# stormalex/minimap2_chaindp

Hardware: AMD Instinct MI355X
Metric: chained anchors/sec (whole node) (higher is better)
Workload: dtype int32

## Files before the change

### minimap2_chaindp_amd/chaindp.py

```python
import collections
import ctypes as C
import os

import numpy as np

from .params import ChainParams, PostOpt

_HERE = os.path.dirname(os.path.abspath(__file__))
LIB_PATH = os.environ.get("CHAINDP_LIB") or os.path.join(_HERE, "csrc", "libchaindp_hip.so")

SEED_DTYPE = np.dtype([("x", "<u8"), ("y", "<u8"), ("p", "<i4"), ("f", "<i4")])

ABI_SYMBOLS = (
    "chaindp_device_count", "chaindp_create", "chaindp_destroy", "chaindp_last_error", "chaindp_chain_batch",
    "chaindp_upload", "chaindp_run", "chaindp_sync", "chaindp_download", "chaindp_compact",
    "chaindp_upload_gather", "chaindp_compact_offsets", "chaindp_download_seeds", "chaindp_host_alloc",
    "chaindp_host_free", "chaindp_run_device", "chaindp_set_profiling", "chaindp_get_kernel_ms",
    "chaindp_get_stats", "chaindp_set_ring", "chaindp_run_full", "chaindp_set_variant", "chaindp_upload_gather_ex", "chaindp_scatter_seeds", "chaindp_backtrack",
    "chaindp_index_create", "chaindp_index_destroy", "chaindp_collect_seeds", "chaindp_download_mini_pos", "chaindp_download_anchors", "chaindp_collect_seeds_gather", "chaindp_scatter_mini_pos",
    "chaindp_gen_regs", "chaindp_est_err",
    "chaindp_pipe_create", "chaindp_pipe_destroy", "chaindp_pipe_submit", "chaindp_pipe_wait", "chaindp_pipe_release",
    "chaindp_pipe_last_error", "chaindp_map_batch",
    "chaindp_chain_post", "chaindp_map_reads", "chaindp_post_logf_selftest", "chaindp_post_logf_patches",
)

REG_DTYPE = np.dtype([(k, "<i4") for k in ("id", "cnt", "rid", "score", "qs", "qe", "rs", "re", "parent", "subsc", "as", "mlen", "blen", "n_sub", "score0")]
                     + [("bits", "<u4"), ("hash", "<u4"), ("div", "<f4"), ("reserved", "<u4", (2,))])


class ChainDPError(RuntimeError):
    pass


_lib = None


def lib():
    global _lib
    if _lib is None:
        if not os.path.exists(LIB_PATH):
            raise ChainDPError(f"{LIB_PATH} is missing: build it with __graft_entry__.build() "
                               "(make -C minimap2_chaindp_amd/csrc); there is no fallback path")
        L = C.CDLL(LIB_PATH)
        P = C.POINTER(ChainParams)
        vp, i64, i32 = C.c_void_p, C.c_int64, C.c_int
        L.chaindp_device_count.restype = i32
        L.chaindp_create.restype = vp
        L.chaindp_create.argtypes = [i32, i64, i64]
        L.chaindp_destroy.argtypes = [vp]
        L.chaindp_last_error.restype = C.c_char_p
        L.chaindp_last_error.argtypes = [vp]
        L.chaindp_chain_batch.argtypes = [vp, P, i64, vp, vp, vp, vp, vp, vp]
        L.chaindp_upload.argtypes = [vp, i64, vp, vp, vp]
        L.chaindp_run.argtypes = [vp, P]
        L.chaindp_run_full.argtypes = [vp, P]
        L.chaindp_sync.argtypes = [vp]
        L.chaindp_download.argtypes = [vp, vp, vp, vp]
        L.chaindp_compact.argtypes = [vp, P, vp, vp]
        L.chaindp_upload_gather.argtypes = [vp, i64, vp, vp, vp]
        L.chaindp_compact_offsets.argtypes = [vp, P, vp]
        L.chaindp_download_seeds.argtypes = [vp, i64, i64, vp]
        L.chaindp_host_alloc.restype = vp
        L.chaindp_host_alloc.argtypes = [C.c_size_t]
        L.chaindp_host_free.argtypes = [vp]
        L.chaindp_run_device.argtypes = [vp, P, i64, i64, vp, vp, vp, vp, vp, vp, vp]
        L.chaindp_set_profiling.argtypes = [vp, i32]
        L.chaindp_get_kernel_ms.argtypes = [vp, vp, vp, i32]
        L.chaindp_get_stats.argtypes = [vp, vp]
        L.chaindp_set_ring.argtypes = [vp, i32]
        L.chaindp_set_variant.argtypes = [vp, i32]
        L.chaindp_backtrack.argtypes = [vp, P, i32, vp, vp, vp, vp]
        L.chaindp_gen_regs.argtypes = [vp, vp, vp, vp]
        L.chaindp_est_err.argtypes = [vp, vp, vp, vp, vp, i32, vp, vp, vp]
        L.chaindp_index_create.restype = vp
        L.chaindp_index_create.argtypes = [i32, vp, C.c_size_t, vp, C.c_size_t, vp, C.c_size_t, vp, C.c_size_t]
        L.chaindp_index_destroy.restype = None
        L.chaindp_index_destroy.argtypes = [vp]
        L.chaindp_collect_seeds.argtypes = [vp, vp, i32, i32, i64, vp, vp, vp, vp, vp, vp, vp, vp]
        L.chaindp_download_mini_pos.argtypes = [vp, vp]
        L.chaindp_collect_seeds_gather.argtypes = [vp, vp, i32, i32, i64, vp, vp, vp, vp, vp, vp, vp, vp]
        L.chaindp_scatter_mini_pos.argtypes = [vp, i64, vp]
        L.chaindp_upload_gather_ex.argtypes = [vp, i64, vp, vp, vp, i32]
        L.chaindp_scatter_seeds.argtypes = [vp, i64, vp]
        L.chaindp_device_count.argtypes = []
        L.chaindp_download_anchors.argtypes = [vp, vp]
        L.chaindp_map_batch.argtypes = [vp, vp, i32, i32, P, i32, i64, vp, vp, vp, vp, vp, vp, vp, i64, vp, vp]
        PO = C.POINTER(PostOpt)
        L.chaindp_chain_post.argtypes = [vp, PO, vp, vp, vp, i32, vp, vp, vp, vp, i64, vp, vp]
        L.chaindp_map_reads.argtypes = [vp, vp, i32, i32, P, i32, PO, i64, vp, vp, vp, vp, vp, vp, i32, vp, vp, i64, vp, vp]
        L.chaindp_post_logf_selftest.restype = i64
        L.chaindp_post_logf_selftest.argtypes = [vp, i32]
        L.chaindp_post_logf_patches.restype = i64
        L.chaindp_post_logf_patches.argtypes = [vp, vp, i64]
        L.chaindp_pipe_create.restype = vp
        L.chaindp_pipe_create.argtypes = [i32, i32, i64, i64]
        L.chaindp_pipe_destroy.restype = None
        L.chaindp_pipe_destroy.argtypes = [vp]
        L.chaindp_pipe_submit.argtypes = [vp, P, i64, vp, vp, vp, i64]
        L.chaindp_pipe_wait.argtypes = [vp, vp]
        L.chaindp_pipe_release.argtypes = [vp]
        L.chaindp_pipe_last_error.restype = C.c_char_p
        L.chaindp_pipe_last_error.argtypes = [vp]
        _lib = L
    return _lib


def post_logf_patches():
    L = lib()
    n = int(L.chaindp_post_logf_patches(None, None, 0))
    k, v = np.zeros(max(n, 1), np.uint32), np.zeros(max(n, 1), np.float32)
    L.chaindp_post_logf_patches(_ptr(k), _ptr(v), n)
    return k[:n], v[:n]


def device_count():
    return lib().chaindp_device_count()


def _ptr(a):
    return None if a is None else a.ctypes.data


class Device:

    def __init__(self, device=0, max_anchors=1 << 24, max_reads=1 << 20, ring=None):
        self._lib = lib()
        if self._lib.chaindp_device_count() <= 0:
            raise ChainDPError("no HIP device visible: the chaining DP runs only on the GPU (no CPU fallback)")
        self._ctx = self._lib.chaindp_create(device, max_anchors, max_reads)
        if not self._ctx:
            raise ChainDPError(self._lib.chaindp_last_error(None).decode())
        self.device = device
        self.max_anchors, self.max_reads = max_anchors, max_reads
        self._n_reads = self._total = 0
        self._indexes = []
        if ring is not None:
            self._check(self._lib.chaindp_set_ring(self._ctx, ring))

    def close(self):
        if self._ctx:
            for h in self._indexes:
                self._lib.chaindp_index_destroy(h)
            self._indexes = []
            self._lib.chaindp_destroy(self._ctx)
            self._ctx = None

    def __enter__(self):
        return self

    def __exit__(self, *exc):
        self.close()

    def __del__(self):
        try:
            self.close()
        except Exception:
            pass

    def _check(self, rc):
        if rc != 0:
            raise ChainDPError(f"chaindp error {rc}: {self._lib.chaindp_last_error(self._ctx).decode()}")

    @staticmethod
    def _prep(off, anchors, n_segs):
        off = np.ascontiguousarray(off, np.int64)
        anchors = np.ascontiguousarray(anchors, np.uint64).reshape(-1, 2)
        if len(off) < 1 or off[0] != 0 or int(off[-1]) != anchors.shape[0]:
            raise ValueError("off must start at 0 and end at the number of anchors")
        ns = None if n_segs is None else np.ascontiguousarray(n_segs, np.int32)
        if ns is not None and len(ns) != len(off) - 1:
            raise ValueError("n_segs must have one entry per read")
        return off, anchors, ns

    def chain_batch(self, par, off, anchors, n_segs=None, want_v=True):
        off, anchors, ns = self._prep(off, anchors, n_segs)
        tot = anchors.shape[0]
        f, p = np.empty(tot, np.int32), np.empty(tot, np.int32)
        v = np.empty(tot, np.int32) if want_v else None
        self._check(self._lib.chaindp_chain_batch(self._ctx, C.byref(par), len(off) - 1, _ptr(off), _ptr(anchors), _ptr(ns),
                                                  _ptr(f), _ptr(p), _ptr(v)))
        self._n_reads, self._total = len(off) - 1, tot
        return f, p, v

    def upload(self, off, anchors, n_segs=None):
        off, anchors, ns = self._prep(off, anchors, n_segs)
        self._check(self._lib.chaindp_upload(self._ctx, len(off) - 1, _ptr(off), _ptr(anchors), _ptr(ns)))
        self._n_reads, self._total = len(off) - 1, anchors.shape[0]

    def run(self, par):
        self._check(self._lib.chaindp_run(self._ctx, C.byref(par)))

    def run_full(self, par):
        self._check(self._lib.chaindp_run_full(self._ctx, C.byref(par)))

    def sync(self):
        self._check(self._lib.chaindp_sync(self._ctx))

    def download(self, want_v=True):
        f, p = np.empty(self._total, np.int32), np.empty(self._total, np.int32)
        v = np.empty(self._total, np.int32) if want_v else None
        self._check(self._lib.chaindp_download(self._ctx, _ptr(f), _ptr(p), _ptr(v)))
        return f, p, v

    def compact(self, par):
        soff = np.zeros(self._n_reads + 1, np.int64)
        seeds = np.zeros(max(self._total, 1), SEED_DTYPE)
        self._check(self._lib.chaindp_compact(self._ctx, C.byref(par), _ptr(soff), _ptr(seeds)))
        return soff, seeds[:int(soff[-1])]

    def backtrack(self, par, min_cnt=3):
        coff = np.zeros(self._n_reads + 1, np.int64)
        boff = np.zeros(self._n_reads + 1, np.int64)
        cap = max(self._total, 1)
        u = np.zeros(cap, np.uint64)
        b = np.zeros((cap, 2), np.uint64)
        self._check(self._lib.chaindp_backtrack(self._ctx, C.byref(par), min_cnt, _ptr(coff), _ptr(u), _ptr(boff), _ptr(b)))
        return coff, u[:int(coff[-1])], boff, b[:int(boff[-1])]

    def gen_regs(self, hash_, qlen, n_chains):
        hash_ = np.ascontiguousarray(hash_, np.uint32)
        qlen = np.ascontiguousarray(qlen, np.int32)
        regs = np.zeros(max(int(n_chains), 1), REG_DTYPE)
        self._check(self._lib.chaindp_gen_regs(self._ctx, _ptr(hash_), _ptr(qlen), _ptr(regs)))
        return regs[:int(n_chains)]

    def est_err(self, regs_off, regs, qlen, ref_len, mini_pos_off=None, mini_pos=None):
        regs_off = np.ascontiguousarray(regs_off, np.int64)
        regs = np.ascontiguousarray(regs, REG_DTYPE).copy()
        qlen = np.ascontiguousarray(qlen, np.int32)
        ref_len = np.ascontiguousarray(ref_len, np.int32)
        mt = np.zeros((max(len(regs), 1), 2), np.int32)
        mpo = None if mini_pos_off is None else np.ascontiguousarray(mini_pos_off, np.int64)
        mp = None if mini_pos is None else np.ascontiguousarray(mini_pos, np.uint64)
        self._check(self._lib.chaindp_est_err(self._ctx, _ptr(regs_off), _ptr(regs) if len(regs) else None, _ptr(qlen), _ptr(ref_len) if len(ref_len) else None,
                                              len(ref_len), None if mpo is None else _ptr(mpo), None if mp is None or not len(mp) else _ptr(mp), _ptr(mt)))
        return regs, mt[:len(regs), 0].copy(), mt[:len(regs), 1].copy()

    def load_index(self, img):
        blobs = [np.ascontiguousarray(b, np.uint8) for b in img]
        h = self._lib.chaindp_index_create(self.device, *sum(([_ptr(b) if b.size else None, int(b.size)] for b in blobs), []))
        if not h:
            raise ChainDPError((self._lib.chaindp_last_error(None) or b"").decode())
        self._indexes.append(h)
        return h

    def collect_seeds(self, index, flag, max_occ, mini_off, mini, bid, qlen, n_segs=None):
        mini_off = np.ascontiguousarray(mini_off, np.int64)
        n_reads = len(mini_off) - 1
        mini = np.ascontiguousarray(mini, np.uint64).reshape(-1, 2)
        bid = np.ascontiguousarray(bid, np.uint32); qlen = np.ascontiguousarray(qlen, np.int32)
        off = np.zeros(n_reads + 1, np.int64); mpo = np.zeros(n_reads + 1, np.int64); rep = np.zeros(max(n_reads, 1), np.int32)
        ns = None if n_segs is None else np.ascontiguousarray(n_segs, np.int32)
        self._check(self._lib.chaindp_collect_seeds(self._ctx, index, int(flag), int(max_occ), n_reads, _ptr(mini_off), _ptr(mini), _ptr(bid),
                                                    _ptr(qlen), _ptr(ns), _ptr(off), _ptr(rep), _ptr(mpo)))
        self._n_reads, self._total = n_reads, int(off[-1])
        a = np.zeros((max(self._total, 1), 2), np.uint64)
        self._check(self._lib.chaindp_download_anchors(self._ctx, _ptr(a)))
        mp = np.zeros(max(int(mpo[-1]), 1), np.uint64)
        self._check(self._lib.chaindp_download_mini_pos(self._ctx, _ptr(mp)))
        return off, a[:self._total], rep[:n_reads], mpo, mp[:int(mpo[-1])]

    def map_batch(self, index, flag, max_occ, par, min_cnt, mini_off, mini, bid, qlen, hash_, regs_cap=None):
        mini_off = np.ascontiguousarray(mini_off, np.int64)
        n_reads = len(mini_off) - 1
        mini = np.ascontiguousarray(mini, np.uint64).reshape(-1, 2)
        bid = np.ascontiguousarray(bid, np.uint32); qlen = np.ascontiguousarray(qlen, np.int32); hash_ = np.ascontiguousarray(hash_, np.uint32)
        cap = int(regs_cap) if regs_cap is not None else max(len(mini) // 4, 1024)
        roff = np.zeros(n_reads + 1, np.int64); rep = np.zeros(max(n_reads, 1), np.int32)
        regs = np.zeros(max(cap, 1), REG_DTYPE)
        na = C.c_int64(0)
        rc = self._lib.chaindp_map_batch(self._ctx, index, int(flag), int(max_occ), C.byref(par), int(min_cnt), n_reads, _ptr(mini_off), _ptr(mini),
                                         _ptr(bid), _ptr(qlen), _ptr(hash_), _ptr(roff), _ptr(regs), cap, _ptr(rep), C.byref(na))
        if rc == -2 and int(roff[-1]) > cap:
            regs = self.gen_regs(hash_, qlen, int(roff[-1]))
        else:
            self._check(rc)
        self._n_reads, self._total = n_reads, int(na.value)
        return roff, regs[:int(roff[-1])], rep[:n_reads], int(na.value)

    def chain_post(self, opt, ref_len, qlen=None, rep_len=None, mini_pos_off=None, mini_pos=None, regs_cap=None, want_anchors=False):
        n_reads = self._n_reads
        ref_len = np.ascontiguousarray(ref_len, np.int32)
        ql = None if qlen is None else np.ascontiguousarray(qlen, np.int32)
        rl = None if rep_len is None else np.ascontiguousarray(rep_len, np.int32)
        mpo = None if mini_pos_off is None else np.ascontiguousarray(mini_pos_off, np.int64)
        mp = None if mini_pos is None else np.ascontiguousarray(mini_pos, np.uint64)
        cap = int(regs_cap) if regs_cap is not None else max(self._total, 1)
        roff = np.zeros(n_reads + 1, np.int64)
        regs = np.zeros(max(cap, 1), REG_DTYPE)
        aoff = np.zeros(n_reads + 1, np.int64) if want_anchors else None
        a = np.zeros((max(self._total, 1), 2), np.uint64) if want_anchors else None
        self._check(self._lib.chaindp_chain_post(self._ctx, C.byref(opt), _ptr(ql), _ptr(rl), _ptr(ref_len) if len(ref_len) else None, len(ref_len),
                                                 _ptr(mpo), None if mp is None or not len(mp) else _ptr(mp), _ptr(roff), _ptr(regs), cap,
                                                 _ptr(aoff), _ptr(a)))
        regs = regs[:int(roff[-1])]
        return (roff, regs, aoff, a[:int(aoff[-1])]) if want_anchors else (roff, regs)

    def map_reads(self, index, flag, max_occ, par, min_cnt, opt, mini_off, mini, bid, qlen, hash_, ref_len, regs_cap=None):
        mini_off = np.ascontiguousarray(mini_off, np.int64)
        n_reads = len(mini_off) - 1
        mini = np.ascontiguousarray(mini, np.uint64).reshape(-1, 2)
        bid = np.ascontiguousarray(bid, np.uint32); qlen = np.ascontiguousarray(qlen, np.int32); hash_ = np.ascontiguousarray(hash_, np.uint32)
        ref_len = np.ascontiguousarray(ref_len, np.int32)
        cap = int(regs_cap) if regs_cap is not None else max(len(mini) // 4, 1024)
        roff = np.zeros(n_reads + 1, np.int64); rep = np.zeros(max(n_reads, 1), np.int32)
        regs = np.zeros(max(cap, 1), REG_DTYPE)
        na = C.c_int64(0)
        rc = self._lib.chaindp_map_reads(self._ctx, index, int(flag), int(max_occ), C.byref(par), int(min_cnt), C.byref(opt), n_reads, _ptr(mini_off),
                                         _ptr(mini), _ptr(bid), _ptr(qlen), _ptr(hash_), _ptr(ref_len) if len(ref_len) else None, len(ref_len),
                                         _ptr(roff), _ptr(regs), cap, _ptr(rep), C.byref(na))
        self._n_reads, self._total = n_reads, int(na.value)
        if rc == -2 and int(roff[-1]) > cap:
            roff, regs = self.chain_post(opt, ref_len, regs_cap=int(roff[-1]))
        else:
            self._check(rc)
        return roff, regs[:int(roff[-1])], rep[:n_reads], int(na.value)

    def post_logf_selftest(self, kmax=1 << 24):
        n = self._lib.chaindp_post_logf_selftest(self._ctx, int(kmax))
        if n < 0:
            self._check(int(n))
        return int(n)

    def run_device(self, par, n_reads, total, d_off, d_a, d_n_segs, d_f, d_p, d_v, stream=0):
        self._check(self._lib.chaindp_run_device(self._ctx, C.byref(par), n_reads, total, d_off, d_a, d_n_segs or None,
                                                 d_f, d_p, d_v, stream or None))

    def set_ring(self, ring):
        self._check(self._lib.chaindp_set_ring(self._ctx, ring))

    def set_variant(self, force_general):
        self._check(self._lib.chaindp_set_variant(self._ctx, int(force_general)))

    def set_profiling(self, on=True):
        self._check(self._lib.chaindp_set_profiling(self._ctx, int(bool(on))))

    def kernel_ms(self, reset=False):
        ms = (C.c_double * 4)()
        n = (C.c_int64 * 4)()
        self._check(self._lib.chaindp_get_kernel_ms(self._ctx, ms, n, int(reset)))
        return {k: (ms[i], n[i]) for i, k in enumerate(("prepass", "chain_dp", "compact", "backtrack"))}

    def leftover_units(self):
        self._lib.chaindp_debug_leftover.restype = C.c_int64
        self._lib.chaindp_debug_leftover.argtypes = [C.c_void_p]
        return int(self._lib.chaindp_debug_leftover(self._ctx))

    def deep_units(self):
        self._lib.chaindp_debug_deep_units.restype = C.c_int64
        self._lib.chaindp_debug_deep_units.argtypes = [C.c_void_p]
        return int(self._lib.chaindp_debug_deep_units(self._ctx))

    def set_quad(self, on=True):
        self._lib.chaindp_debug_set_quad.restype = C.c_int
        self._lib.chaindp_debug_set_quad.argtypes = [C.c_void_p, C.c_int]
        self._check(self._lib.chaindp_debug_set_quad(self._ctx, int(bool(on))))

    def quad_took(self):
        self._lib.chaindp_debug_quad_took.restype = C.c_int
        self._lib.chaindp_debug_quad_took.argtypes = [C.c_void_p]
        return int(self._lib.chaindp_debug_quad_took(self._ctx)) == 1

    def set_twin_handover(self, mode=0):
        self._lib.chaindp_debug_set_twin_handover.restype = C.c_int
        self._lib.chaindp_debug_set_twin_handover.argtypes = [C.c_void_p, C.c_int]
        self._check(self._lib.chaindp_debug_set_twin_handover(self._ctx, int(mode)))

    def set_deep_handover(self, on=True):
        self._lib.chaindp_debug_set_deep_handover.restype = C.c_int
        self._lib.chaindp_debug_set_deep_handover.argtypes = [C.c_void_p, C.c_int]
        self._check(self._lib.chaindp_debug_set_deep_handover(self._ctx, on if on in (2, 3, 4) else int(bool(on))))

    def stats(self):
        st = (C.c_int64 * 4)()
        self._check(self._lib.chaindp_get_stats(self._ctx, st))
        return dict(units=st[0], singletons=st[1], anchors=st[2], reads=st[3])


class PinnedArray:

    def __init__(self, shape, dtype):
        self._lib = lib()
        dtype = np.dtype(dtype)
        n = int(np.prod(shape)) * dtype.itemsize
        self._ptr = self._lib.chaindp_host_alloc(max(n, 1))
        if not self._ptr:
            raise ChainDPError("chaindp_host_alloc failed (no GPU runtime or out of pinned memory)")
        self.array = np.ctypeslib.as_array((C.c_uint8 * max(n, 1)).from_address(self._ptr))[:n].view(dtype).reshape(shape)

    def free(self):
        if self._ptr:
            self.array = None
            self._lib.chaindp_host_free(self._ptr)
            self._ptr = None

    def __del__(self):
        try:
            self.free()
        except Exception:
            pass


class _PipeResult(C.Structure):
    _fields_ = [("tag", C.c_int64), ("n_reads", C.c_int64), ("n_anchors", C.c_int64), ("n_seeds", C.c_int64),
                ("seeds_off", C.c_void_p), ("seeds", C.c_void_p)]


class Pipe:

    def __init__(self, device=0, depth=3, max_anchors=1 << 24, max_reads=1 << 20):
        self._lib = lib()
        if self._lib.chaindp_device_count() <= 0:
            raise ChainDPError("no HIP device visible: the chaining DP runs only on the GPU (no CPU fallback)")
        self._p = self._lib.chaindp_pipe_create(device, depth, max_anchors, max_reads)
        if not self._p:
            raise ChainDPError((self._lib.chaindp_pipe_last_error(None) or b"").decode())
        self.depth = depth
        self._keep = collections.deque()

    def close(self):
        if self._p:
            self._lib.chaindp_pipe_destroy(self._p)
            self._p = None

    def __enter__(self):
        return self

    def __exit__(self, *exc):
        self.close()

    def _check(self, rc):
        if rc != 0:
            raise ChainDPError(f"chaindp pipe error {rc}: {self._lib.chaindp_pipe_last_error(self._p).decode()}")

    def submit(self, par, off, anchors, n_segs=None, tag=0):
        off, anchors, ns = Device._prep(off, anchors, n_segs)
        rc = self._lib.chaindp_pipe_submit(self._p, C.byref(par), len(off) - 1, _ptr(off), _ptr(anchors), _ptr(ns), tag)
        if rc == -5:
            return False
        self._check(rc)
        self._keep.append((off, anchors, ns))
        return True

    def wait(self, copy=True):
        r = _PipeResult()
        self._check(self._lib.chaindp_pipe_wait(self._p, C.byref(r)))
        soff = np.ctypeslib.as_array((C.c_int64 * (r.n_reads + 1)).from_address(r.seeds_off))
        seeds = np.ctypeslib.as_array((C.c_uint8 * max(r.n_seeds * 24, 1)).from_address(r.seeds))[:r.n_seeds * 24].view(SEED_DTYPE)
        if copy:
            soff, seeds = soff.copy(), seeds.copy()
        if self._keep:
            self._keep.popleft()
        return r.tag, soff, seeds

    def release(self):
        self._check(self._lib.chaindp_pipe_release(self._p))
```

### minimap2_chaindp_amd/csrc/chaindp_abi.cpp

```cpp
#include <hip/hip_runtime.h>
#include <stdint.h>
#include <stdio.h>
#include <stdlib.h>
#include <string.h>
#include <math.h>
#include <mutex>
#include <string>
#include <vector>
#include "../../include/chaindp.h"
#include "chaindp_kernels.h"

using chaindp::Params;
using chaindp::Unit;

static thread_local std::string g_create_error;

struct EventSet { hipEvent_t e[3]; int n; int slot0; };

struct chaindp_ctx {
	int device = -1;
	hipStream_t stream = nullptr;
	int64_t cap_anchors = 0, cap_reads = 0;
	int ring = 128;
	int64_t n_reads = 0, total = 0, n_seeds = 0;
	bool has_n_segs = false, ran = false, compact_ready = false;
	bool singles_pending = false;
	chaindp_params_t ran_par{};
	int64_t *d_off = nullptr;
	void *d_a = nullptr;
	int32_t *d_n_segs = nullptr;
	int32_t *d_f = nullptr, *d_p = nullptr, *d_v = nullptr;
	unsigned long long *d_tg = nullptr;
	uint32_t epoch = 0;
	unsigned long long *d_sumq = nullptr;
	Unit *d_units = nullptr;
	chaindp::UnitAux *d_unit_aux = nullptr;
	Unit *d_left = nullptr;
	unsigned long long *d_left_cnt = nullptr;
	Unit *d_deep = nullptr;
	int deep_route = 0;
	int deep_eager = 0;
	bool deep_handover = true;
	bool use_quad = false;
	int twin_force_left = 0;
	int variant = 0;
	unsigned long long *d_counters = nullptr;
	chaindp::PrepassScratch pre = {nullptr, nullptr, nullptr, nullptr, nullptr};
	chaindp::CompactScratch cmp = {nullptr, nullptr, nullptr, nullptr, nullptr, nullptr};
	chaindp::BottomScratch bot = {};
	bool bot_ready = false, seed_ready = false;
	std::vector<void*> bot_allocs;
	uint16_t *d_lut = nullptr;
	void **d_ptrs = nullptr;
	size_t ptr_cap = 0;
	size_t lut_bytes = 0;
	bool use_lut = true;
	int32_t *d_first_child = nullptr;
	unsigned int *d_twin_queue = nullptr;
	int64_t *d_seeds_off = nullptr;
	void *d_seeds = nullptr;
	chaindp::SeedScratch seed = {nullptr, nullptr, nullptr, nullptr, nullptr, nullptr, nullptr};
	void *d_mini = nullptr;
	int64_t *d_mini_off = nullptr, *d_mp_off = nullptr;
	uint32_t *d_bid = nullptr;
	int32_t *d_qlen = nullptr, *d_rep_len = nullptr;
	unsigned long long *d_mini_pos = nullptr;
	int64_t seed_cap_mini = 0, n_mini_pos = 0;
	int seed_max_n = -1, seed_max_n2 = -1;
	int seed_lab_cap = 0;
	void *d_regs = nullptr, *d_reg_counts = nullptr, *d_ref_len = nullptr, *d_mp_up = nullptr;
	size_t regs_cap = 0, reg_counts_cap = 0, ref_len_cap = 0, mp_up_cap = 0;
	uint32_t *d_rhash = nullptr;
	int32_t *d_rqlen = nullptr;
	int64_t *d_regs_off = nullptr, *d_mp_off_up = nullptr;
	unsigned long long *d_sum_k = nullptr;
	int64_t bot_n_reads = -1, bot_n_chains = 0, bot_n_b = 0;
	bool mp_resident = false;
	bool regs_resident = false;
	void *d_post_stage = nullptr, *d_post_out = nullptr, *d_post_sq = nullptr, *d_post_scratch = nullptr;
	size_t post_stage_cap = 0, post_out_cap = 0, post_sq_cap = 0, post_scratch_cap = 0;
	unsigned long long *d_post_off = nullptr, *d_post_tile = nullptr;
	int32_t *d_post_qlen = nullptr, *d_post_rep = nullptr, *d_post_err = nullptr;
	uint32_t *d_logf_k = nullptr;
	float *d_logf_v = nullptr;
	int n_logf = -1;
	bool prof = false;
	std::vector<EventSet> pending;
	double ms[4] = {0, 0, 0, 0};
	int64_t launches[4] = {0, 0, 0, 0};
	int64_t stats[4] = {0, 0, 0, 0};
	std::string err;
};

#define HIP_TRY(ctx, call)                                                                         \
	do {                                                                                           \
		hipError_t e_ = (call);                                                                    \
		if (e_ != hipSuccess) {                                                                    \
			(ctx)->err = std::string(#call) + ": " + hipGetErrorString(e_);                        \
			return CHAINDP_ERR_HIP;                                                                \
		}                                                                                          \
	} while (0)

static Params to_params(const chaindp_params_t *p)
{
	Params q;
	q.max_dist_x = p->max_dist_x; q.max_dist_y = p->max_dist_y; q.bw = p->bw; q.max_skip = p->max_skip;
	q.min_sc = p->min_sc; q.is_cdna = p->is_cdna; q.n_segs = p->n_segs;
	return q;
}

static int check_params(chaindp_ctx *ctx, const chaindp_params_t *par)
{
	if (!par) { ctx->err = "params is NULL"; return CHAINDP_ERR_ARG; }
	if (par->max_dist_x < 0 || par->max_dist_y < 0 || par->bw < 0) {
		ctx->err = "max_dist_x, max_dist_y and bw must be >= 0";
		return CHAINDP_ERR_ARG;
	}
	return CHAINDP_OK;
}

extern "C" int chaindp_device_count(void)
{
	int n = 0;
	if (hipGetDeviceCount(&n) != hipSuccess) return 0;
	return n;
}

extern "C" const char *chaindp_last_error(const chaindp_ctx_t *ctx)
{
	return ctx ? ctx->err.c_str() : g_create_error.c_str();
}

extern "C" void chaindp_destroy(chaindp_ctx_t *ctx)
{
	if (!ctx) return;
	if (ctx->device >= 0) (void)hipSetDevice(ctx->device);
	if (ctx->stream) (void)hipStreamSynchronize(ctx->stream);
	for (auto &es : ctx->pending) for (int k = 0; k < es.n; ++k) (void)hipEventDestroy(es.e[k]);
	void *bufs[] = {ctx->d_twin_queue, ctx->d_off, ctx->d_a, ctx->d_n_segs, ctx->d_f, ctx->d_p, ctx->d_v, ctx->d_tg, ctx->d_sumq, ctx->d_units,
	                ctx->d_counters, ctx->d_unit_aux, ctx->d_left, ctx->d_left_cnt, ctx->d_deep, ctx->pre.start_mask, ctx->pre.single_mask, ctx->pre.emit_mask, ctx->pre.block_cnt, ctx->pre.tile_tmp, ctx->pre.units_tmp, ctx->pre.hist, ctx->pre.block_reads, ctx->d_lut, ctx->d_ptrs, ctx->cmp.flags, ctx->cmp.block_cnt, ctx->cmp.tile_tmp, ctx->cmp.n_seeds, ctx->cmp.sub, ctx->d_first_child, ctx->d_seeds_off, ctx->d_seeds};
	for (void *b : bufs) if (b) (void)hipFree(b);
	for (void *b : ctx->bot_allocs) if (b) (void)hipFree(b);
	void *sbufs[] = {ctx->seed.kept, ctx->seed.used, ctx->seed.src, ctx->seed.mstate, ctx->seed.tile_tmp, ctx->seed.totals, ctx->seed.stacks,
	                 ctx->d_mini, ctx->d_mini_off, ctx->d_mp_off, ctx->d_bid, ctx->d_qlen, ctx->d_rep_len, ctx->d_mini_pos};
	for (void *b : sbufs) if (b) (void)hipFree(b);
	if (ctx->stream) (void)hipStreamDestroy(ctx->stream);
	delete ctx;
}

extern "C" chaindp_ctx_t *chaindp_create(int device, int64_t max_anchors, int64_t max_reads)
{
	int n_dev = 0;
	if (hipGetDeviceCount(&n_dev) != hipSuccess || n_dev <= 0) { g_create_error = "no HIP device visible"; return nullptr; }
	if (device < 0 || device >= n_dev || max_anchors < 0 || max_reads < 0 || max_anchors > 0x7fffffff || max_reads > 0x7fffffff) {
		g_create_error = "bad device index or capacity (at most 2^31-1 anchors and reads per batch)";
		return nullptr;
	}
	chaindp_ctx *ctx = new chaindp_ctx();
	ctx->device = device;
	ctx->cap_anchors = max_anchors > 0 ? max_anchors : 1;
	ctx->cap_reads = max_reads > 0 ? max_reads : 1;
	const size_t na = (size_t)ctx->cap_anchors, nr = (size_t)ctx->cap_reads;
	hipError_t e = hipSetDevice(device);
	if (e == hipSuccess) e = hipStreamCreateWithFlags(&ctx->stream, hipStreamNonBlocking);
	if (e == hipSuccess) e = hipMalloc((void**)&ctx->d_off, (nr + 1) * 8);
	if (e == hipSuccess) e = hipMalloc(&ctx->d_a, na * 16);
	if (e == hipSuccess) e = hipMalloc((void**)&ctx->d_n_segs, nr * 4);
	if (e == hipSuccess) e = hipMalloc((void**)&ctx->d_f, na * 4);
	if (e == hipSuccess) e = hipMalloc((void**)&ctx->d_twin_queue, 8 * 64 * sizeof(unsigned int));
	if (e == hipSuccess) e = hipMalloc((void**)&ctx->d_p, na * 4);
	if (e == hipSuccess) e = hipMalloc((void**)&ctx->d_v, na * 4);
	if (e == hipSuccess) e = hipMalloc((void**)&ctx->d_tg, na * 8);
	if (e == hipSuccess) e = hipMemset(ctx->d_tg, 0, na * 8);
	if (e == hipSuccess) e = hipMalloc((void**)&ctx->d_sumq, nr * 8);
	if (e == hipSuccess) e = hipMalloc((void**)&ctx->d_units, (na / 2 + 1) * sizeof(Unit));
	if (e == hipSuccess) e = hipMalloc((void**)&ctx->d_unit_aux, (na / 2 + 1) * sizeof(chaindp::UnitAux));
	if (e == hipSuccess) e = hipMalloc((void**)&ctx->d_counters, 2 * sizeof(unsigned long long));
	if (e == hipSuccess) e = hipMalloc((void**)&ctx->d_left, (na / 2 + 1) * sizeof(Unit));
	if (e == hipSuccess) e = hipMalloc((void**)&ctx->d_left_cnt, 4 * sizeof(unsigned long long));
	if (e == hipSuccess) e = hipMalloc((void**)&ctx->d_deep, (na / 64 + 2) * sizeof(Unit));
	size_t flags_bytes0 = 0, cblocks_bytes0 = 0;
	chaindp::compact_scratch_bytes(ctx->cap_anchors, &flags_bytes0, &cblocks_bytes0);
	if (e == hipSuccess) e = hipMalloc((void**)&ctx->d_first_child, na * 4);
	if (e == hipSuccess) e = hipMalloc((void**)&ctx->cmp.flags, flags_bytes0);
	size_t mask_bytes = 0, blocks_bytes = 0;
	chaindp::prepass_scratch_bytes(ctx->cap_anchors, &mask_bytes, &blocks_bytes);
	if (e == hipSuccess) e = hipMalloc((void**)&ctx->pre.start_mask, mask_bytes);
	if (e == hipSuccess) e = hipMalloc((void**)&ctx->pre.single_mask, mask_bytes);
	if (e == hipSuccess) e = hipMalloc((void**)&ctx->pre.emit_mask, mask_bytes);
	ctx->cmp.single_mask = ctx->pre.single_mask; ctx->cmp.emit_mask = ctx->pre.emit_mask;
	if (e == hipSuccess) e = hipMalloc((void**)&ctx->pre.block_cnt, blocks_bytes);
	if (e == hipSuccess) e = hipMalloc((void**)&ctx->pre.tile_tmp, blocks_bytes);
	if (e == hipSuccess) e = hipMalloc((void**)&ctx->pre.units_tmp, (na / 2 + 1) * sizeof(Unit));
	if (e == hipSuccess) e = hipMalloc((void**)&ctx->pre.hist, (2 * 128 + 2) * sizeof(unsigned int));
	ctx->pre.key_range = ctx->pre.hist ? ctx->pre.hist + 2 * 128 : nullptr;
	if (e == hipSuccess) e = hipMalloc((void**)&ctx->pre.block_reads, blocks_bytes);
	ctx->cmp.block_reads = ctx->pre.block_reads;
	ctx->use_quad = getenv("CHAINDP_QUAD") != nullptr;
	ctx->deep_handover = getenv("CHAINDP_NO_DEEP_HANDOVER") == nullptr;
	if (const char *v = getenv("CHAINDP_TWIN_FORCE_LEFT")) ctx->twin_force_left = atoi(v) == 2 ? 2 : 1;
	if (e != hipSuccess) {
		g_create_error = std::string("chaindp_create: ") + hipGetErrorString(e);
		chaindp_destroy(ctx);
		return nullptr;
	}
	return ctx;
}

extern "C" int chaindp_set_ring(chaindp_ctx_t *ctx, int ring)
{
	if (!ctx) return CHAINDP_ERR_ARG;
	if (ring != 128 && ring != 256 && ring != 512) { ctx->err = "ring must be 128, 256 or 512"; return CHAINDP_ERR_ARG; }
	ctx->ring = ring;
	return CHAINDP_OK;
}

extern "C" int chaindp_set_variant(chaindp_ctx_t *ctx, int force_general)
{
	if (!ctx) return CHAINDP_ERR_ARG;
	if (force_general < 0 || force_general > 2) { ctx->err = "variant must be 0 (two units per wave + the rest), 1 (general) or 2 (one unit per wave)"; return CHAINDP_ERR_ARG; }
	ctx->use_lut = force_general != 1;
	ctx->variant = force_general;
	return CHAINDP_OK;
}

extern "C" int chaindp_set_profiling(chaindp_ctx_t *ctx, int on)
{
	if (!ctx) return CHAINDP_ERR_ARG;
	ctx->prof = on != 0;
	return CHAINDP_OK;
}

static int run_on_stream(chaindp_ctx *ctx, const chaindp_params_t *par, int64_t n_reads, int64_t total,
                         const int64_t *d_off, const void *d_a, const int32_t *d_n_segs,
                         int32_t *d_f, int32_t *d_p, int32_t *d_v, hipStream_t st)
{
	int rc = check_params(ctx, par);
	if (rc) return rc;
	if (n_reads < 0 || total < 0) { ctx->err = "negative batch size"; return CHAINDP_ERR_ARG; }
	if (n_reads > ctx->cap_reads || total > ctx->cap_anchors) {
		ctx->err = "batch exceeds the capacity the context was created with";
		return CHAINDP_ERR_CAPACITY;
	}
	HIP_TRY(ctx, hipSetDevice(ctx->device));
	const Params q = to_params(par);
	EventSet es; es.n = 0; es.slot0 = 0;
	if (ctx->prof) {
		for (int k = 0; k < 3; ++k) HIP_TRY(ctx, hipEventCreate(&es.e[k]));
		es.n = 3;
	}
	if (ctx->prof) HIP_TRY(ctx, hipEventRecord(es.e[0], st));
	HIP_TRY(ctx, chaindp::launch_prepass(st, q, n_reads, total, d_off, d_a, ctx->d_sumq, ctx->d_units, ctx->d_counters, ctx->pre, ctx->d_unit_aux, d_n_segs, ctx->d_left_cnt));
	if (ctx->prof) HIP_TRY(ctx, hipEventRecord(es.e[1], st));
	uint16_t *lut = nullptr;
	int lut_stride = 0;
	if (ctx->use_lut && !q.is_cdna && q.bw <= CHAINDP_LUT_MAX_BW && n_reads > 0) {
		lut_stride = (q.bw + 1 + 7) & ~7;
		const size_t need = (size_t)n_reads * lut_stride * sizeof(uint16_t);
		if (need > ctx->lut_bytes) {
			HIP_TRY(ctx, hipStreamSynchronize(st));
			if (ctx->d_lut) HIP_TRY(ctx, hipFree(ctx->d_lut));
			ctx->d_lut = nullptr; ctx->lut_bytes = 0;
			HIP_TRY(ctx, hipMalloc((void**)&ctx->d_lut, need));
			ctx->lut_bytes = need;
		}
		lut = ctx->d_lut;
		HIP_TRY(ctx, chaindp::launch_lut(st, q, n_reads, d_off, ctx->d_sumq, lut_stride, lut));
	}
	if (++ctx->epoch == 0) {
		HIP_TRY(ctx, hipMemsetAsync(ctx->d_tg, 0, (size_t)ctx->cap_anchors * 8, st));
		ctx->epoch = 1;
	}
	Unit *const deep = ctx->deep_handover ? ctx->d_deep : nullptr;
	unsigned int *const deep_cnt = (unsigned int*)(ctx->d_left_cnt + 1);
	if (ctx->variant == 0 && lut) {
		unsigned int *const route = (unsigned int*)(ctx->d_left_cnt + 3);
		Params qt = q;
		if (d_n_segs) qt.n_segs = 1;
		if (ctx->use_quad)
			HIP_TRY(ctx, chaindp::launch_chain_quad(st, qt, total / 2, d_a, lut, lut_stride, ctx->d_units, ctx->d_unit_aux, ctx->d_counters, ctx->pre.key_range,
			                                        d_f, d_p, d_v, ctx->d_first_child, ctx->cmp.flags, ctx->d_left, (unsigned int*)ctx->d_left_cnt,
			                                        (unsigned int*)ctx->d_left_cnt + 1, route, ctx->twin_force_left, total));
		HIP_TRY(ctx, chaindp::launch_chain_twin(st, qt, total / 2, d_off, d_a, ctx->d_sumq, lut, lut_stride, ctx->d_units, ctx->d_counters,
		                                        d_f, d_p, d_v, ctx->d_first_child, ctx->cmp.flags, ctx->d_left, (unsigned int*)ctx->d_left_cnt,
		                                        ctx->twin_force_left, total, ctx->d_unit_aux, route, ctx->d_twin_queue));
		const int64_t left_grid = total / 2 < 32768 ? total / 2 : 32768;
		HIP_TRY(ctx, chaindp::launch_chain(st, ctx->ring, q, left_grid, d_off, d_a, d_n_segs, ctx->d_sumq, lut, lut_stride, ctx->d_left,
		                                   ctx->d_left_cnt, d_f, d_p, d_v, ctx->d_tg, ctx->epoch, ctx->d_first_child, ctx->cmp.flags,
		                                   ctx->d_units, ctx->d_counters, deep, deep_cnt, ctx->pre.hist + CHAINDP_LONG_UNIT_CLASS, ctx->deep_eager, ctx->deep_route));
	} else
		HIP_TRY(ctx, chaindp::launch_chain(st, ctx->ring, q, total / 2, d_off, d_a, d_n_segs, ctx->d_sumq, lut, lut_stride, ctx->d_units,
		                                   ctx->d_counters, d_f, d_p, d_v, ctx->d_tg, ctx->epoch, ctx->d_first_child, ctx->cmp.flags,
		                                   nullptr, nullptr, deep, deep_cnt, ctx->pre.hist + CHAINDP_LONG_UNIT_CLASS, ctx->deep_eager, ctx->deep_route));
	if (deep && lut) {
		HIP_TRY(ctx, chaindp::launch_chain_dense(st, q, total / 64 + 1, d_off, d_a, lut, lut_stride, ctx->d_deep, ctx->d_left_cnt + 1,
		                                         d_f, d_p, d_v, ctx->d_first_child, ctx->cmp.flags, ctx->pre.hist + CHAINDP_LONG_UNIT_CLASS, ctx->deep_route,
		                                           (unsigned int*)(ctx->d_left_cnt + 3) + 1));
		HIP_TRY(ctx, chaindp::launch_chain_dense16(st, q, total / 64 + 1, d_off, d_a, lut, lut_stride, ctx->d_deep, ctx->d_left_cnt + 1,
		                                           d_f, d_p, d_v, ctx->d_first_child, ctx->cmp.flags, ctx->pre.hist + CHAINDP_LONG_UNIT_CLASS, ctx->deep_route,
		                                           (unsigned int*)(ctx->d_left_cnt + 3) + 1));
		HIP_TRY(ctx, chaindp::launch_chain_dense1(st, q, total / 64 + 1, d_off, d_a, lut, lut_stride, ctx->d_deep, ctx->d_left_cnt + 1,
		                                          ctx->pre.hist + CHAINDP_LONG_UNIT_CLASS, ctx->deep_route, (unsigned int*)(ctx->d_left_cnt + 2), d_f, d_p, d_v, ctx->d_first_child, ctx->cmp.flags));
	}
	if (ctx->prof) { HIP_TRY(ctx, hipEventRecord(es.e[2], st)); ctx->pending.push_back(es); }
	ctx->stats[2] = total; ctx->stats[3] = n_reads;
	return CHAINDP_OK;
}

extern "C" int chaindp_upload(chaindp_ctx_t *ctx, int64_t n_reads, const int64_t *off, const chaindp_anchor_t *a,
                              const int32_t *n_segs_per_read)
{
	if (!ctx) return CHAINDP_ERR_ARG;
	if (n_reads < 0 || !off || (n_reads > 0 && off[0] != 0)) { ctx->err = "bad offsets"; return CHAINDP_ERR_ARG; }
	const int64_t total = n_reads > 0 ? off[n_reads] : 0;
	if (total < 0 || (total > 0 && !a)) { ctx->err = "bad anchors"; return CHAINDP_ERR_ARG; }
	if (n_reads > ctx->cap_reads || total > ctx->cap_anchors) {
		ctx->err = "batch exceeds the capacity the context was created with";
		return CHAINDP_ERR_CAPACITY;
	}
	HIP_TRY(ctx, hipSetDevice(ctx->device));
	HIP_TRY(ctx, hipMemcpyAsync(ctx->d_off, off, (size_t)(n_reads + 1) * 8, hipMemcpyHostToDevice, ctx->stream));
	if (total) HIP_TRY(ctx, hipMemcpyAsync(ctx->d_a, a, (size_t)total * 16, hipMemcpyHostToDevice, ctx->stream));
	ctx->has_n_segs = n_segs_per_read != nullptr;
	if (n_segs_per_read && n_reads)
		HIP_TRY(ctx, hipMemcpyAsync(ctx->d_n_segs, n_segs_per_read, (size_t)n_reads * 4, hipMemcpyHostToDevice, ctx->stream));
	HIP_TRY(ctx, hipStreamSynchronize(ctx->stream));
	ctx->n_reads = n_reads; ctx->total = total; ctx->ran = false; ctx->bot_n_reads = -1; ctx->mp_resident = false;
	return CHAINDP_OK;
}

extern "C" int chaindp_run(chaindp_ctx_t *ctx, const chaindp_params_t *par)
{
	if (!ctx) return CHAINDP_ERR_ARG;
	int rc = run_on_stream(ctx, par, ctx->n_reads, ctx->total, ctx->d_off, ctx->d_a, ctx->has_n_segs ? ctx->d_n_segs : nullptr,
	                       ctx->d_f, ctx->d_p, ctx->d_v, ctx->stream);
	if (rc == CHAINDP_OK) { ctx->ran = true; ctx->singles_pending = true; ctx->ran_par = *par; }
	return rc;
}

extern "C" int chaindp_run_device(chaindp_ctx_t *ctx, const chaindp_params_t *par, int64_t n_reads, int64_t total_anchors,
                                  const void *d_off, const void *d_a, const void *d_n_segs,
                                  void *d_f, void *d_p, void *d_v, void *stream)
{
	if (!ctx) return CHAINDP_ERR_ARG;
	if (!d_off || (total_anchors > 0 && (!d_a || !d_f || !d_p || !d_v))) { ctx->err = "NULL device pointer"; return CHAINDP_ERR_ARG; }
	hipStream_t st = stream ? (hipStream_t)stream : ctx->stream;
	const int rc = run_on_stream(ctx, par, n_reads, total_anchors, (const int64_t*)d_off, d_a, (const int32_t*)d_n_segs,
	                             (int32_t*)d_f, (int32_t*)d_p, (int32_t*)d_v, st);
	if (rc != CHAINDP_OK) return rc;
	HIP_TRY(ctx, chaindp::launch_fill_singles(st, to_params(par), total_anchors, d_a, ctx->pre, (int32_t*)d_f, (int32_t*)d_p, (int32_t*)d_v, ctx->cmp.flags));
	return CHAINDP_OK;
}

extern "C" int chaindp_sync(chaindp_ctx_t *ctx)
{
	if (!ctx) return CHAINDP_ERR_ARG;
	HIP_TRY(ctx, hipSetDevice(ctx->device));
	HIP_TRY(ctx, hipStreamSynchronize(ctx->stream));
	return CHAINDP_OK;
}

extern "C" int chaindp_download(chaindp_ctx_t *ctx, int32_t *f, int32_t *p, int32_t *v)
{
	if (!ctx) return CHAINDP_ERR_ARG;
	if (!ctx->ran) { ctx->err = "chaindp_download before chaindp_run"; return CHAINDP_ERR_ARG; }
	HIP_TRY(ctx, hipSetDevice(ctx->device));
	const size_t bytes = (size_t)ctx->total * 4;
	if (ctx->singles_pending) {
		HIP_TRY(ctx, chaindp::launch_fill_singles(ctx->stream, to_params(&ctx->ran_par), ctx->total, ctx->d_a, ctx->pre, ctx->d_f, ctx->d_p, ctx->d_v, ctx->cmp.flags));
		ctx->singles_pending = false;
	}
	if (bytes) {
		if (f) HIP_TRY(ctx, hipMemcpyAsync(f, ctx->d_f, bytes, hipMemcpyDeviceToHost, ctx->stream));
		if (p) HIP_TRY(ctx, hipMemcpyAsync(p, ctx->d_p, bytes, hipMemcpyDeviceToHost, ctx->stream));
		if (v) HIP_TRY(ctx, hipMemcpyAsync(v, ctx->d_v, bytes, hipMemcpyDeviceToHost, ctx->stream));
	}
	HIP_TRY(ctx, hipStreamSynchronize(ctx->stream));
	return CHAINDP_OK;
}

extern "C" int chaindp_chain_batch(chaindp_ctx_t *ctx, const chaindp_params_t *par, int64_t n_reads, const int64_t *off,
                                   const chaindp_anchor_t *a, const int32_t *n_segs_per_read,
                                   int32_t *f, int32_t *p, int32_t *v)
{
	if (!ctx) return CHAINDP_ERR_ARG;
	int rc = check_params(ctx, par);
	if (rc) return rc;
	if ((rc = chaindp_upload(ctx, n_reads, off, a, n_segs_per_read)) != CHAINDP_OK) return rc;
	if ((rc = chaindp_run(ctx, par)) != CHAINDP_OK) return rc;
	return chaindp_download(ctx, f, p, v);
}

static int compact_launch(chaindp_ctx *ctx, const chaindp_params_t *par)
{
	int rc = check_params(ctx, par);
	if (rc) return rc;
	if (!ctx->ran) { ctx->err = "compaction before chaindp_run"; return CHAINDP_ERR_ARG; }
	HIP_TRY(ctx, hipSetDevice(ctx->device));
	if (!ctx->compact_ready) {
		const size_t na = (size_t)ctx->cap_anchors, nr = (size_t)ctx->cap_reads;
		size_t flags_bytes = 0, blocks_bytes = 0;
		chaindp::compact_scratch_bytes(ctx->cap_anchors, &flags_bytes, &blocks_bytes);
		void *nb[6] = {nullptr, nullptr, nullptr, nullptr, nullptr, nullptr};
		const size_t sz[6] = {(nr + 1) * 8, ctx->d_seeds ? 0 : na * sizeof(chaindp_seed_t) + 16, blocks_bytes, blocks_bytes, 8, blocks_bytes * 32};
		hipError_t e = hipSuccess;
		for (int k = 0; k < 6 && e == hipSuccess; ++k) if (sz[k]) e = hipMalloc(&nb[k], sz[k]);
		if (e != hipSuccess) {
			for (void *b : nb) if (b) (void)hipFree(b);
			ctx->err = std::string("compaction buffers: ") + hipGetErrorString(e);
			return CHAINDP_ERR_HIP;
		}
		ctx->d_seeds_off = (int64_t*)nb[0];
		if (nb[1]) ctx->d_seeds = nb[1];
		ctx->cmp.block_cnt = (unsigned long long*)nb[2]; ctx->cmp.tile_tmp = (unsigned long long*)nb[3];
		ctx->cmp.n_seeds = (unsigned long long*)nb[4]; ctx->cmp.sub = (uint32_t*)nb[5];
		ctx->compact_ready = true;
	}
	EventSet es; es.n = 0; es.slot0 = 2;
	if (ctx->prof) {
		for (int k = 0; k < 2; ++k) HIP_TRY(ctx, hipEventCreate(&es.e[k]));
		es.n = 2;
		HIP_TRY(ctx, hipEventRecord(es.e[0], ctx->stream));
	}
	HIP_TRY(ctx, chaindp::launch_compact(ctx->stream, to_params(par), ctx->n_reads, ctx->total, ctx->d_off, ctx->d_a, ctx->d_f, ctx->d_p,
	                                     ctx->d_v, ctx->d_first_child, ctx->d_seeds_off, ctx->d_seeds, ctx->cmp));
	if (ctx->prof) { HIP_TRY(ctx, hipEventRecord(es.e[1], ctx->stream)); ctx->pending.push_back(es); }
	return CHAINDP_OK;
}

static int compact_on_device(chaindp_ctx *ctx, const chaindp_params_t *par, int64_t *seeds_off)
{
	if (!seeds_off) { ctx->err = "NULL output"; return CHAINDP_ERR_ARG; }
	int rc = compact_launch(ctx, par);
	if (rc) return rc;
	HIP_TRY(ctx, hipMemcpyAsync(seeds_off, ctx->d_seeds_off, (size_t)(ctx->n_reads + 1) * 8, hipMemcpyDeviceToHost, ctx->stream));
	HIP_TRY(ctx, hipStreamSynchronize(ctx->stream));
	ctx->n_seeds = seeds_off[ctx->n_reads];
	return CHAINDP_OK;
}

template <typename T>
static hipError_t bot_alloc(chaindp_ctx *ctx, T *&p, size_t bytes)
{
	void *q = nullptr;
	hipError_t e = hipMalloc(&q, bytes ? bytes : 8);
	if (e == hipSuccess) { ctx->bot_allocs.push_back(q); p = (T*)q; }
	return e;
}

extern "C" int chaindp_backtrack(chaindp_ctx_t *ctx, const chaindp_params_t *par, int min_cnt,
                                 int64_t *chains_off, uint64_t *u, int64_t *b_off, chaindp_anchor_t *b)
{
	if (!ctx) return CHAINDP_ERR_ARG;
	int rc = check_params(ctx, par);
	if (rc) return rc;
	if (!ctx->ran || !ctx->d_seeds) { ctx->err = "chaindp_backtrack needs a completed run and compaction"; return CHAINDP_ERR_ARG; }
	if (!chains_off || !b_off) { ctx->err = "NULL output"; return CHAINDP_ERR_ARG; }
	ctx->regs_resident = false;
	HIP_TRY(ctx, hipSetDevice(ctx->device));
	unsigned long long n_seeds = 0;
	HIP_TRY(ctx, hipMemcpyAsync(&n_seeds, ctx->cmp.n_seeds, 8, hipMemcpyDeviceToHost, ctx->stream));
	HIP_TRY(ctx, hipStreamSynchronize(ctx->stream));
	const int64_t m = ctx->total > 0 && ctx->n_reads > 0 ? (int64_t)(uint32_t)n_seeds : 0;
	ctx->n_seeds = m;
	if (!ctx->bot_ready) {
		const size_t M = (size_t)ctx->cap_anchors, R = (size_t)ctx->cap_reads, NB = M / 1024 + 2;
		chaindp::BottomScratch &s = ctx->bot;
		const size_t first = ctx->bot_allocs.size();
		hipError_t e = hipSuccess;
#define BOT_ALLOC(field, bytes) if (e == hipSuccess) e = bot_alloc(ctx, s.field, (bytes))
		BOT_ALLOC(has, M);
		BOT_ALLOC(owner, M * 4); BOT_ALLOC(end_rec, M * 4); BOT_ALLOC(ccnt, M * 4); BOT_ALLOC(kpos, M * 4); BOT_ALLOC(bpos, M * 4);
		BOT_ALLOC(c_src, M * 4); BOT_ALLOC(c_dst, M * 4);
		BOT_ALLOC(key, M * 8); BOT_ALLOC(skey, M * 8); BOT_ALLOC(cu, M * 8); BOT_ALLOC(u_tmp, M * 8); BOT_ALLOC(u_out, M * 8);
		BOT_ALLOC(b_tmp, M * 16); BOT_ALLOC(b_out, M * 16); BOT_ALLOC(w, M * 16);
		BOT_ALLOC(stacks, (M / 64 + 2 * R + 4) * 12);
		BOT_ALLOC(block_cnt, (NB > R + 2 ? NB : R + 2) * 8); BOT_ALLOC(tile_tmp, (NB > R + 2 ? NB : R + 2) * 8);
		BOT_ALLOC(read_tot, (R + 2) * 8); BOT_ALLOC(total, 8);
		BOT_ALLOC(ends_off, (R + 2) * 8); BOT_ALLOC(chains_off, (R + 2) * 8); BOT_ALLOC(b_off, (R + 2) * 8);
#undef BOT_ALLOC
		if (e != hipSuccess) {
			for (size_t k = first; k < ctx->bot_allocs.size(); ++k) if (ctx->bot_allocs[k]) (void)hipFree(ctx->bot_allocs[k]);
			ctx->bot_allocs.resize(first);
			ctx->bot = chaindp::BottomScratch{};
			ctx->err = std::string("backtrack buffers: ") + hipGetErrorString(e);
			return CHAINDP_ERR_HIP;
		}
		ctx->bot_ready = true;
	}
	EventSet es; es.n = 0; es.slot0 = 3;
	if (ctx->prof) {
		for (int k = 0; k < 2; ++k) HIP_TRY(ctx, hipEventCreate(&es.e[k]));
		es.n = 2;
		HIP_TRY(ctx, hipEventRecord(es.e[0], ctx->stream));
	}
	HIP_TRY(ctx, chaindp::launch_backtrack(ctx->stream, min_cnt, par->min_sc, ctx->n_reads, ctx->cap_anchors, ctx->d_seeds_off, ctx->d_seeds,
	                                       ctx->cmp.n_seeds, ctx->bot, m));
	if (ctx->prof) { HIP_TRY(ctx, hipEventRecord(es.e[1], ctx->stream)); ctx->pending.push_back(es); }
	const size_t ob = (size_t)(ctx->n_reads > 0 ? ctx->n_reads + 1 : 1) * 8;
	HIP_TRY(ctx, hipMemcpyAsync(chains_off, ctx->bot.chains_off, ob, hipMemcpyDeviceToHost, ctx->stream));
	HIP_TRY(ctx, hipMemcpyAsync(b_off, ctx->bot.b_off, ob, hipMemcpyDeviceToHost, ctx->stream));
	HIP_TRY(ctx, hipStreamSynchronize(ctx->stream));
	const int64_t n_c = ctx->n_reads > 0 ? chains_off[ctx->n_reads] : 0, n_b = ctx->n_reads > 0 ? b_off[ctx->n_reads] : 0;
	ctx->bot_n_reads = ctx->n_reads; ctx->bot_n_chains = n_c; ctx->bot_n_b = n_b;
	if (u && n_c > 0) HIP_TRY(ctx, hipMemcpyAsync(u, ctx->bot.u_out, (size_t)n_c * 8, hipMemcpyDeviceToHost, ctx->stream));
	if (b && n_b > 0) HIP_TRY(ctx, hipMemcpyAsync(b, ctx->bot.b_out, (size_t)n_b * 16, hipMemcpyDeviceToHost, ctx->stream));
	HIP_TRY(ctx, hipStreamSynchronize(ctx->stream));
	return CHAINDP_OK;
}

static hipError_t regs_grow(chaindp_ctx *ctx, void *&p, size_t &cap, size_t need)
{
	if (need <= cap && p) return hipSuccess;
	void *q = nullptr;
	hipError_t e = hipMalloc(&q, need ? need + need / 4 : 8);
	if (e != hipSuccess) return e;
	for (void *&old : ctx->bot_allocs) if (old == p && p) { (void)hipFree(p); old = nullptr; }
	ctx->bot_allocs.push_back(q);
	p = q; cap = need + need / 4;
	return hipSuccess;
}

static int regs_per_read_buffers(chaindp_ctx *ctx)
{
	if (ctx->d_rhash) return CHAINDP_OK;
	const size_t R = (size_t)ctx->cap_reads + 2;
	HIP_TRY(ctx, bot_alloc(ctx, ctx->d_rhash, R * 4)); HIP_TRY(ctx, bot_alloc(ctx, ctx->d_rqlen, R * 4));
	HIP_TRY(ctx, bot_alloc(ctx, ctx->d_regs_off, R * 8)); HIP_TRY(ctx, bot_alloc(ctx, ctx->d_mp_off_up, R * 8));
	HIP_TRY(ctx, bot_alloc(ctx, ctx->d_sum_k, R * 8));
	return CHAINDP_OK;
}

static int gen_regs_impl(chaindp_ctx *ctx, const uint32_t *hash, const int32_t *qlen, chaindp_reg_t *regs, bool download)
{
	if (!ctx) return CHAINDP_ERR_ARG;
	if (ctx->bot_n_reads < 0 || ctx->bot_n_reads != ctx->n_reads || !ctx->bot.has) { ctx->err = "chaindp_gen_regs needs the chains of a chaindp_backtrack on this batch"; return CHAINDP_ERR_ARG; }
	const int64_t R = ctx->bot_n_reads, n_c = ctx->bot_n_chains;
	if (R > 0 && (!hash || !qlen)) { ctx->err = "NULL hash or qlen"; return CHAINDP_ERR_ARG; }
	if (download && n_c > 0 && !regs) { ctx->err = "NULL output"; return CHAINDP_ERR_ARG; }
	ctx->regs_resident = false;
	if (R == 0 || n_c == 0) { ctx->regs_resident = true; return CHAINDP_OK; }
	HIP_TRY(ctx, hipSetDevice(ctx->device));
	int rc = regs_per_read_buffers(ctx);
	if (rc) return rc;
	HIP_TRY(ctx, regs_grow(ctx, ctx->d_regs, ctx->regs_cap, (size_t)n_c * sizeof(chaindp_reg_t)));
	hipStream_t st = ctx->stream;
	HIP_TRY(ctx, hipMemcpyAsync(ctx->d_rhash, hash, (size_t)R * 4, hipMemcpyHostToDevice, st));
	HIP_TRY(ctx, hipMemcpyAsync(ctx->d_rqlen, qlen, (size_t)R * 4, hipMemcpyHostToDevice, st));
	HIP_TRY(ctx, chaindp::launch_gen_regs(st, R, ctx->bot.chains_off, ctx->bot.b_off, ctx->bot.u_out, ctx->bot.b_out, ctx->d_rhash, ctx->d_rqlen,
	                                      ctx->bot.w, ctx->bot.stacks, ctx->d_regs));
	if (download) HIP_TRY(ctx, hipMemcpyAsync(regs, ctx->d_regs, (size_t)n_c * sizeof(chaindp_reg_t), hipMemcpyDeviceToHost, st));
	HIP_TRY(ctx, hipStreamSynchronize(st));
	ctx->regs_resident = true;
	return CHAINDP_OK;
}

extern "C" int chaindp_gen_regs(chaindp_ctx_t *ctx, const uint32_t *hash, const int32_t *qlen, chaindp_reg_t *regs)
{
	return gen_regs_impl(ctx, hash, qlen, regs, true);
}

extern "C" int chaindp_est_err(chaindp_ctx_t *ctx, const int64_t *regs_off, chaindp_reg_t *regs, const int32_t *qlen,
                               const int32_t *ref_len, int32_t n_ref, const int64_t *mini_pos_off, const uint64_t *mini_pos,
                               int32_t *match_tot)
{
	if (!ctx) return CHAINDP_ERR_ARG;
	if (ctx->bot_n_reads < 0 || ctx->bot_n_reads != ctx->n_reads || !ctx->bot.has) { ctx->err = "chaindp_est_err needs the chains of a chaindp_backtrack on this batch"; return CHAINDP_ERR_ARG; }
	const int64_t R = ctx->bot_n_reads;
	if (R == 0) return CHAINDP_OK;
	if (!regs_off || !qlen || (n_ref > 0 && !ref_len) || n_ref < 0) { ctx->err = "NULL argument"; return CHAINDP_ERR_ARG; }
	if (regs_off[0] != 0) { ctx->err = "regs_off must start at 0"; return CHAINDP_ERR_ARG; }
	for (int64_t r = 0; r < R; ++r) if (regs_off[r + 1] < regs_off[r]) { ctx->err = "regs_off must not decrease"; return CHAINDP_ERR_ARG; }
	const int64_t n_regs = regs_off[R];
	if (n_regs == 0) return CHAINDP_OK;
	if (!regs) { ctx->err = "NULL regs"; return CHAINDP_ERR_ARG; }
	const bool resident = mini_pos == nullptr && mini_pos_off == nullptr;
	if (resident && (!ctx->mp_resident || !ctx->d_mp_off)) { ctx->err = "no resident mini_pos: pass the arrays, or collect the seeds with chaindp_collect_seeds"; return CHAINDP_ERR_ARG; }
	if (!resident && !mini_pos_off) { ctx->err = "mini_pos without offsets"; return CHAINDP_ERR_ARG; }
	for (int64_t g = 0; g < n_regs; ++g) if (regs[g].cnt < 0 || regs[g].as < 0) { ctx->err = "hit with a negative count or offset"; return CHAINDP_ERR_ARG; }
	HIP_TRY(ctx, hipSetDevice(ctx->device));
	int rc = regs_per_read_buffers(ctx);
	if (rc) return rc;
	hipStream_t st = ctx->stream;
	ctx->regs_resident = false;
	{
		std::vector<int64_t> boff((size_t)R + 1);
		HIP_TRY(ctx, hipMemcpyAsync(boff.data(), ctx->bot.b_off, (size_t)(R + 1) * 8, hipMemcpyDeviceToHost, st));
		HIP_TRY(ctx, hipStreamSynchronize(st));
		for (int64_t r = 0; r < R; ++r)
			for (int64_t g = regs_off[r]; g < regs_off[r + 1]; ++g)
				if ((int64_t)regs[g].as + regs[g].cnt > boff[r + 1] - boff[r]) { ctx->err = "hit reaches beyond its read's chain anchors"; return CHAINDP_ERR_ARG; }
	}
	HIP_TRY(ctx, regs_grow(ctx, ctx->d_regs, ctx->regs_cap, (size_t)n_regs * sizeof(chaindp_reg_t)));
	HIP_TRY(ctx, regs_grow(ctx, ctx->d_reg_counts, ctx->reg_counts_cap, (size_t)n_regs * 8));
	HIP_TRY(ctx, regs_grow(ctx, ctx->d_ref_len, ctx->ref_len_cap, (size_t)(n_ref > 0 ? n_ref : 1) * 4));
	const int64_t *d_mpo = ctx->d_mp_off;
	const unsigned long long *d_mp = ctx->d_mini_pos;
	if (!resident) {
		const int64_t n_mp = mini_pos_off[R];
		if (n_mp < 0 || (n_mp > 0 && !mini_pos)) { ctx->err = "mini_pos announced but absent"; return CHAINDP_ERR_ARG; }
		HIP_TRY(ctx, regs_grow(ctx, ctx->d_mp_up, ctx->mp_up_cap, (size_t)(n_mp > 0 ? n_mp : 1) * 8));
		HIP_TRY(ctx, hipMemcpyAsync(ctx->d_mp_off_up, mini_pos_off, (size_t)(R + 1) * 8, hipMemcpyHostToDevice, st));
		if (n_mp > 0) HIP_TRY(ctx, hipMemcpyAsync(ctx->d_mp_up, mini_pos, (size_t)n_mp * 8, hipMemcpyHostToDevice, st));
		d_mpo = ctx->d_mp_off_up; d_mp = (const unsigned long long*)ctx->d_mp_up;
	}
	HIP_TRY(ctx, hipMemcpyAsync(ctx->d_regs_off, regs_off, (size_t)(R + 1) * 8, hipMemcpyHostToDevice, st));
	HIP_TRY(ctx, hipMemcpyAsync(ctx->d_rqlen, qlen, (size_t)R * 4, hipMemcpyHostToDevice, st));
	if (n_ref > 0) HIP_TRY(ctx, hipMemcpyAsync(ctx->d_ref_len, ref_len, (size_t)n_ref * 4, hipMemcpyHostToDevice, st));
	HIP_TRY(ctx, hipMemcpyAsync(ctx->d_regs, regs, (size_t)n_regs * sizeof(chaindp_reg_t), hipMemcpyHostToDevice, st));
	HIP_TRY(ctx, chaindp::launch_est_err(st, R, n_regs, ctx->d_regs_off, ctx->bot.b_off, ctx->bot.b_out, ctx->d_rqlen, (const int32_t*)ctx->d_ref_len, n_ref,
	                                     d_mpo, d_mp, ctx->d_sum_k, ctx->d_regs, (int32_t*)ctx->d_reg_counts));
	HIP_TRY(ctx, hipMemcpyAsync(regs, ctx->d_regs, (size_t)n_regs * sizeof(chaindp_reg_t), hipMemcpyDeviceToHost, st));
	if (match_tot) HIP_TRY(ctx, hipMemcpyAsync(match_tot, ctx->d_reg_counts, (size_t)n_regs * 8, hipMemcpyDeviceToHost, st));
	HIP_TRY(ctx, hipStreamSynchronize(st));
	return CHAINDP_OK;
}

extern "C" int64_t chaindp_debug_leftover(chaindp_ctx_t *ctx)
{
	if (!ctx || !ctx->d_left_cnt) return -1;
	unsigned long long c = 0, cnt = 0;
	if (hipSetDevice(ctx->device) != hipSuccess || hipStreamSynchronize(ctx->stream) != hipSuccess ||
	    hipMemcpy(&c, ctx->d_left_cnt, sizeof(c), hipMemcpyDeviceToHost) != hipSuccess ||
	    hipMemcpy(&cnt, ctx->d_counters, sizeof(cnt), hipMemcpyDeviceToHost) != hipSuccess) return -1;
	return (uint32_t)c == 0xffffffffu ? (int64_t)(uint32_t)cnt : (int64_t)(uint32_t)c;
}

extern "C" int chaindp_debug_set_quad(chaindp_ctx_t *ctx, int on)
{
	if (!ctx) return CHAINDP_ERR_ARG;
	ctx->use_quad = on != 0;
	return CHAINDP_OK;
}

extern "C" int chaindp_debug_quad_took(chaindp_ctx_t *ctx)
{
	if (!ctx || !ctx->d_left_cnt) return -1;
	unsigned long long r = 0;
	if (hipSetDevice(ctx->device) != hipSuccess || hipStreamSynchronize(ctx->stream) != hipSuccess ||
	    hipMemcpy(&r, ctx->d_left_cnt + 3, sizeof(r), hipMemcpyDeviceToHost) != hipSuccess) return -1;
	return (uint32_t)r != 0;
}

extern "C" int chaindp_debug_set_twin_handover(chaindp_ctx_t *ctx, int mode)
{
	if (!ctx || mode < 0 || mode > 2) return CHAINDP_ERR_ARG;
	ctx->twin_force_left = mode;
	return CHAINDP_OK;
}

extern "C" int chaindp_debug_set_deep_handover(chaindp_ctx_t *ctx, int on)
{
	if (!ctx) return CHAINDP_ERR_ARG;
	ctx->deep_handover = on != 0;
	ctx->deep_eager = on >= 2;
	ctx->deep_route = on == 2 ? 1 : on == 3 ? 2 : on == 4 ? 3 : 0;
	return CHAINDP_OK;
}

extern "C" int64_t chaindp_debug_deep_units(chaindp_ctx_t *ctx)
{
	if (!ctx || !ctx->d_left_cnt) return -1;
	unsigned long long c = 0;
	if (hipSetDevice(ctx->device) != hipSuccess || hipStreamSynchronize(ctx->stream) != hipSuccess ||
	    hipMemcpy(&c, ctx->d_left_cnt + 1, sizeof(c), hipMemcpyDeviceToHost) != hipSuccess) return -1;
	return (int64_t)(uint32_t)c;
}

extern "C" int chaindp_debug_poison(chaindp_ctx_t *ctx, int which, int byte, size_t bytes)
{
	if (!ctx || which < 0 || (size_t)which >= ctx->bot_allocs.size()) return CHAINDP_ERR_ARG;
	HIP_TRY(ctx, hipSetDevice(ctx->device));
	HIP_TRY(ctx, hipMemset(ctx->bot_allocs[which], byte, bytes));
	return CHAINDP_OK;
}

extern "C" int chaindp_debug_bottom(chaindp_ctx_t *ctx, int which, void *dst, size_t bytes)
{
	if (!ctx || !ctx->bot.has) return CHAINDP_ERR_ARG;
	const void *src = nullptr;
	switch (which) {
	case 0: src = ctx->bot.has; break;
	case 1: src = ctx->bot.owner; break;
	case 2: src = ctx->bot.skey; break;
	case 3: src = ctx->bot.ccnt; break;
	case 4: src = ctx->bot.key; break;
	case 5: src = ctx->bot.end_rec; break;
	case 6: src = ctx->bot.ends_off; break;
	default: return CHAINDP_ERR_ARG;
	}
	HIP_TRY(ctx, hipSetDevice(ctx->device));
	HIP_TRY(ctx, hipMemcpy(dst, src, bytes, hipMemcpyDeviceToHost));
	return CHAINDP_OK;
}

extern "C" int chaindp_run_full(chaindp_ctx_t *ctx, const chaindp_params_t *par)
{
	if (!ctx) return CHAINDP_ERR_ARG;
	int rc = chaindp_run(ctx, par);
	if (rc) return rc;
	return compact_launch(ctx, par);
}

extern "C" int chaindp_compact_offsets(chaindp_ctx_t *ctx, const chaindp_params_t *par, int64_t *seeds_off)
{
	if (!ctx) return CHAINDP_ERR_ARG;
	return compact_on_device(ctx, par, seeds_off);
}

extern "C" int chaindp_download_seeds(chaindp_ctx_t *ctx, int64_t first_seed, int64_t n_seeds, chaindp_seed_t *dst)
{
	if (!ctx) return CHAINDP_ERR_ARG;
	if (first_seed < 0 || n_seeds < 0 || first_seed + n_seeds > ctx->n_seeds || (n_seeds > 0 && !dst)) {
		ctx->err = "seed range outside the last compaction";
		return CHAINDP_ERR_ARG;
	}
	if (n_seeds == 0) return CHAINDP_OK;
	HIP_TRY(ctx, hipSetDevice(ctx->device));
	HIP_TRY(ctx, hipMemcpyAsync(dst, (const chaindp_seed_t*)ctx->d_seeds + first_seed, (size_t)n_seeds * sizeof(chaindp_seed_t),
	                            hipMemcpyDeviceToHost, ctx->stream));
	return CHAINDP_OK;
}

extern "C" int chaindp_compact(chaindp_ctx_t *ctx, const chaindp_params_t *par, int64_t *seeds_off, chaindp_seed_t *seeds)
{
	if (!ctx) return CHAINDP_ERR_ARG;
	if (ctx->total > 0 && !seeds) { ctx->err = "NULL output"; return CHAINDP_ERR_ARG; }
	int rc = compact_on_device(ctx, par, seeds_off);
	if (rc) return rc;
	if ((rc = chaindp_download_seeds(ctx, 0, ctx->n_seeds, seeds)) != CHAINDP_OK) return rc;
	return chaindp_sync(ctx);
}

static int stage_pointers(chaindp_ctx *ctx, const void *const *ptrs, int64_t n)
{
	if ((size_t)n > ctx->ptr_cap) {
		HIP_TRY(ctx, hipStreamSynchronize(ctx->stream));
		if (ctx->d_ptrs) HIP_TRY(ctx, hipFree(ctx->d_ptrs));
		ctx->d_ptrs = nullptr; ctx->ptr_cap = 0;
		const size_t cap = (size_t)n + (size_t)n / 2 + 64;
		HIP_TRY(ctx, hipMalloc((void**)&ctx->d_ptrs, cap * sizeof(void*)));
		ctx->ptr_cap = cap;
	}
	if (n) HIP_TRY(ctx, hipMemcpyAsync(ctx->d_ptrs, ptrs, (size_t)n * sizeof(void*), hipMemcpyHostToDevice, ctx->stream));
	return CHAINDP_OK;
}

extern "C" int chaindp_upload_gather_ex(chaindp_ctx_t *ctx, int64_t n_reads, const int64_t *off,
                                        const chaindp_anchor_t *const *read_anchors, const int32_t *n_segs_per_read, int pinned)
{
	if (!ctx) return CHAINDP_ERR_ARG;
	if (!pinned) return chaindp_upload_gather(ctx, n_reads, off, read_anchors, n_segs_per_read);
	if (n_reads < 0 || !off || (n_reads > 0 && (off[0] != 0 || !read_anchors))) { ctx->err = "bad offsets"; return CHAINDP_ERR_ARG; }
	const int64_t total = n_reads > 0 ? off[n_reads] : 0;
	if (n_reads > ctx->cap_reads || total > ctx->cap_anchors) {
		ctx->err = "batch exceeds the capacity the context was created with";
		return CHAINDP_ERR_CAPACITY;
	}
	for (int64_t r = 0; r < n_reads; ++r)
		if (off[r + 1] < off[r] || (off[r + 1] > off[r] && !read_anchors[r])) { ctx->err = "bad read in gather list"; return CHAINDP_ERR_ARG; }
	HIP_TRY(ctx, hipSetDevice(ctx->device));
	HIP_TRY(ctx, hipMemcpyAsync(ctx->d_off, off, (size_t)(n_reads + 1) * 8, hipMemcpyHostToDevice, ctx->stream));
	int rc = stage_pointers(ctx, (const void *const *)read_anchors, n_reads);
	if (rc) return rc;
	HIP_TRY(ctx, chaindp::launch_gather_reads(ctx->stream, n_reads, ctx->d_off, (const void *const *)ctx->d_ptrs, ctx->d_a));
	ctx->has_n_segs = n_segs_per_read != nullptr;
	if (n_segs_per_read && n_reads)
		HIP_TRY(ctx, hipMemcpyAsync(ctx->d_n_segs, n_segs_per_read, (size_t)n_reads * 4, hipMemcpyHostToDevice, ctx->stream));
	HIP_TRY(ctx, hipStreamSynchronize(ctx->stream));
	ctx->n_reads = n_reads; ctx->total = total; ctx->ran = false; ctx->bot_n_reads = -1; ctx->mp_resident = false;
	return CHAINDP_OK;
}

extern "C" int chaindp_scatter_seeds(chaindp_ctx_t *ctx, int64_t n_reads, chaindp_seed_t *const *dst)
{
	if (!ctx) return CHAINDP_ERR_ARG;
	if (n_reads != ctx->n_reads || (n_reads > 0 && !dst) || !ctx->d_seeds) { ctx->err = "scatter does not match the last compaction"; return CHAINDP_ERR_ARG; }
	for (int64_t r = 0; r < n_reads; ++r) if ((uintptr_t)dst[r] & 15u) { ctx->err = "scatter destinations must be 16-byte aligned"; return CHAINDP_ERR_ARG; }
	HIP_TRY(ctx, hipSetDevice(ctx->device));
	int rc = stage_pointers(ctx, (const void *const *)dst, n_reads);
	if (rc) return rc;
	HIP_TRY(ctx, chaindp::launch_scatter_seeds(ctx->stream, n_reads, ctx->d_seeds_off, (void *const *)ctx->d_ptrs, ctx->d_seeds));
	return CHAINDP_OK;
}

extern "C" int chaindp_upload_gather(chaindp_ctx_t *ctx, int64_t n_reads, const int64_t *off,
                                     const chaindp_anchor_t *const *read_anchors, const int32_t *n_segs_per_read)
{
	if (!ctx) return CHAINDP_ERR_ARG;
	if (n_reads < 0 || !off || (n_reads > 0 && (off[0] != 0 || !read_anchors))) { ctx->err = "bad offsets"; return CHAINDP_ERR_ARG; }
	const int64_t total = n_reads > 0 ? off[n_reads] : 0;
	if (n_reads > ctx->cap_reads || total > ctx->cap_anchors) {
		ctx->err = "batch exceeds the capacity the context was created with";
		return CHAINDP_ERR_CAPACITY;
	}
	HIP_TRY(ctx, hipSetDevice(ctx->device));
	HIP_TRY(ctx, hipMemcpyAsync(ctx->d_off, off, (size_t)(n_reads + 1) * 8, hipMemcpyHostToDevice, ctx->stream));
	for (int64_t r = 0; r < n_reads; ++r) {
		const int64_t n = off[r + 1] - off[r];
		if (n < 0 || (n > 0 && !read_anchors[r])) { ctx->err = "bad read in gather list"; return CHAINDP_ERR_ARG; }
		if (n) HIP_TRY(ctx, hipMemcpyAsync((chaindp_anchor_t*)ctx->d_a + off[r], read_anchors[r], (size_t)n * 16, hipMemcpyHostToDevice, ctx->stream));
	}
	ctx->has_n_segs = n_segs_per_read != nullptr;
	if (n_segs_per_read && n_reads)
		HIP_TRY(ctx, hipMemcpyAsync(ctx->d_n_segs, n_segs_per_read, (size_t)n_reads * 4, hipMemcpyHostToDevice, ctx->stream));
	HIP_TRY(ctx, hipStreamSynchronize(ctx->stream));
	ctx->n_reads = n_reads; ctx->total = total; ctx->ran = false; ctx->bot_n_reads = -1; ctx->mp_resident = false;
	return CHAINDP_OK;
}

extern "C" void *chaindp_host_alloc(size_t bytes)
{
	void *p = nullptr;
	if (hipHostMalloc(&p, bytes ? bytes : 1, hipHostMallocDefault) != hipSuccess) return nullptr;
	return p;
}

extern "C" void chaindp_host_free(void *p)
{
	if (p) (void)hipHostFree(p);
}

extern "C" int chaindp_get_kernel_ms(chaindp_ctx_t *ctx, double ms[4], int64_t launches[4], int reset)
{
	if (!ctx) return CHAINDP_ERR_ARG;
	HIP_TRY(ctx, hipSetDevice(ctx->device));
	for (auto &es : ctx->pending) {
		HIP_TRY(ctx, hipEventSynchronize(es.e[es.n - 1]));
		for (int k = 0; k + 1 < es.n; ++k) {
			float t = 0;
			HIP_TRY(ctx, hipEventElapsedTime(&t, es.e[k], es.e[k + 1]));
			ctx->ms[es.slot0 + k] += (double)t;
			ctx->launches[es.slot0 + k] += 1;
		}
		for (int k = 0; k < es.n; ++k) (void)hipEventDestroy(es.e[k]);
	}
	ctx->pending.clear();
	for (int k = 0; k < 4; ++k) { if (ms) ms[k] = ctx->ms[k]; if (launches) launches[k] = ctx->launches[k]; }
	if (reset) for (int k = 0; k < 4; ++k) { ctx->ms[k] = 0; ctx->launches[k] = 0; }
	return CHAINDP_OK;
}

extern "C" int chaindp_get_stats(chaindp_ctx_t *ctx, int64_t st[4])
{
	if (!ctx || !st) return CHAINDP_ERR_ARG;
	HIP_TRY(ctx, hipSetDevice(ctx->device));
	unsigned long long c = 0;
	HIP_TRY(ctx, hipStreamSynchronize(ctx->stream));
	HIP_TRY(ctx, hipMemcpy(&c, ctx->d_counters, sizeof(c), hipMemcpyDeviceToHost));
	ctx->stats[0] = (int64_t)(c & 0xffffffffull); ctx->stats[1] = (int64_t)(c >> 32);
	for (int k = 0; k < 4; ++k) st[k] = ctx->stats[k];
	return CHAINDP_OK;
}


struct chaindp_index {
	int device = -1;
	uint8_t *blob[4] = {nullptr, nullptr, nullptr, nullptr};
	size_t bytes[4] = {0, 0, 0, 0};
	int b_bits = 0;
};

extern "C" chaindp_index_t *chaindp_index_create(int device, const void *B, size_t nB, const void *H, size_t nH,
                                                 const void *V, size_t nV, const void *P, size_t nP)
{
	g_create_error.clear();
	if (!B || nB < 16 || !H || !V) { g_create_error = "chaindp_index_create: the image needs its B, H and V blobs"; return nullptr; }
	if (hipSetDevice(device) != hipSuccess) { g_create_error = "chaindp_index_create: no such HIP device (there is no CPU fallback)"; return nullptr; }
	chaindp_index *ix = new chaindp_index();
	ix->device = device;
	const void *src[4] = {B, H, V, P};
	const size_t nb[4] = {nB, nH, nV, nP};
	for (int k = 0; k < 4; ++k) {
		ix->bytes[k] = nb[k];
		const size_t alloc = (nb[k] + 63) & ~(size_t)63;
		if (hipMalloc((void**)&ix->blob[k], alloc ? alloc : 64) != hipSuccess ||
		    hipMemset(ix->blob[k], 0, alloc ? alloc : 64) != hipSuccess ||
		    (nb[k] && hipMemcpy(ix->blob[k], src[k], nb[k], hipMemcpyHostToDevice) != hipSuccess)) {
			g_create_error = "chaindp_index_create: out of device memory";
			chaindp_index_destroy(ix);
			return nullptr;
		}
	}
	size_t entries = nB / 16;
	while ((size_t)2 << ix->b_bits <= entries) ++ix->b_bits;
	return ix;
}

extern "C" void chaindp_index_destroy(chaindp_index_t *ix)
{
	if (!ix) return;
	if (ix->device >= 0) (void)hipSetDevice(ix->device);
	for (int k = 0; k < 4; ++k) if (ix->blob[k]) (void)hipFree(ix->blob[k]);
	delete ix;
}

static int seed_reserve(chaindp_ctx *ctx, int64_t n_mini)
{
	if (!ctx->seed_ready) {
		const size_t nr = (size_t)ctx->cap_reads;
		void **slot[7] = {(void**)&ctx->d_mini_off, (void**)&ctx->d_mp_off, (void**)&ctx->d_bid, (void**)&ctx->d_qlen, (void**)&ctx->d_rep_len,
		                  (void**)&ctx->seed.totals, (void**)&ctx->seed.stacks};
		const size_t stack_bytes = ((size_t)ctx->cap_anchors / 64 + 2 * nr + 4) * 12, tied_bytes = ((size_t)ctx->cap_anchors / 64 + nr + 8) * 4;
		const size_t sz[7] = {(nr + 1) * 8, (nr + 1) * 8, (nr + 1) * 4, (nr + 1) * 4, (nr + 1) * 4, 32, stack_bytes + tied_bytes};
		void *nb[7] = {nullptr, nullptr, nullptr, nullptr, nullptr, nullptr, nullptr};
		hipError_t e = hipSuccess;
		for (int k = 0; k < 7 && e == hipSuccess; ++k) e = hipMalloc(&nb[k], sz[k]);
		if (e != hipSuccess) {
			for (void *q : nb) if (q) (void)hipFree(q);
			ctx->err = std::string("seed collection buffers: ") + hipGetErrorString(e);
			return CHAINDP_ERR_HIP;
		}
		for (int k = 0; k < 7; ++k) *slot[k] = nb[k];
		ctx->seed.tied = (uint32_t*)((char*)ctx->seed.stacks + stack_bytes);
		ctx->seed_ready = true;
	}
	if (n_mini > ctx->seed_cap_mini) {
		HIP_TRY(ctx, hipStreamSynchronize(ctx->stream));
		void **grow[] = {(void**)&ctx->seed.kept, (void**)&ctx->seed.used, (void**)&ctx->seed.src, (void**)&ctx->seed.mstate,
		                 (void**)&ctx->seed.tile_tmp, (void**)&ctx->d_mini, (void**)&ctx->d_mini_pos};
		for (void **g : grow) if (*g) { HIP_TRY(ctx, hipFree(*g)); *g = nullptr; }
		ctx->seed_cap_mini = 0;
		const size_t n = (size_t)n_mini + (size_t)n_mini / 4 + 1024;
		HIP_TRY(ctx, hipMalloc((void**)&ctx->seed.kept, n * 8));
		HIP_TRY(ctx, hipMalloc((void**)&ctx->seed.used, n * 8));
		HIP_TRY(ctx, hipMalloc((void**)&ctx->seed.src, n * 8));
		HIP_TRY(ctx, hipMalloc((void**)&ctx->seed.mstate, n * 8));
		HIP_TRY(ctx, hipMalloc((void**)&ctx->seed.tile_tmp, (n / 1024 + 2) * 8));
		HIP_TRY(ctx, hipMalloc((void**)&ctx->d_mini, n * 16));
		HIP_TRY(ctx, hipMalloc((void**)&ctx->d_mini_pos, n * 8));
		ctx->seed_cap_mini = (int64_t)n;
	}
	return CHAINDP_OK;
}

static int collect_seeds_impl(chaindp_ctx *ctx, const chaindp_index_t *ix, int flag, int max_occ, int64_t n_reads,
                              const int64_t *mini_off, const chaindp_anchor_t *mini, const chaindp_anchor_t *const *read_mini,
                              const uint32_t *bid, const int32_t *qlen,
                              const int32_t *n_segs_per_read, int64_t *off, int32_t *rep_len, int64_t *mini_pos_off)
{
	if (!ctx) return CHAINDP_ERR_ARG;
	if (!ix || ix->device != ctx->device) { ctx->err = "index image missing or on another device"; return CHAINDP_ERR_ARG; }
	if (n_reads < 0 || !mini_off || (n_reads > 0 && (mini_off[0] != 0 || !bid || !qlen))) { ctx->err = "bad minimizer offsets"; return CHAINDP_ERR_ARG; }
	const int64_t n_mini = n_reads > 0 ? mini_off[n_reads] : 0;
	if (n_mini < 0 || (n_mini > 0 && !mini && !read_mini)) { ctx->err = "bad minimizers"; return CHAINDP_ERR_ARG; }
	if (n_reads > ctx->cap_reads) { ctx->err = "batch exceeds the capacity the context was created with"; return CHAINDP_ERR_CAPACITY; }
	HIP_TRY(ctx, hipSetDevice(ctx->device));
	int rc = seed_reserve(ctx, n_mini);
	if (rc) return rc;
	hipStream_t st = ctx->stream;
	HIP_TRY(ctx, hipMemcpyAsync(ctx->d_mini_off, mini_off, (size_t)(n_reads + 1) * 8, hipMemcpyHostToDevice, st));
	if (n_mini && read_mini) {
		rc = stage_pointers(ctx, (const void *const *)read_mini, n_reads);
		if (rc) return rc;
		HIP_TRY(ctx, chaindp::launch_gather_reads(st, n_reads, ctx->d_mini_off, (const void *const *)ctx->d_ptrs, ctx->d_mini));
	} else if (n_mini) HIP_TRY(ctx, hipMemcpyAsync(ctx->d_mini, mini, (size_t)n_mini * 16, hipMemcpyHostToDevice, st));
	if (n_reads) {
		HIP_TRY(ctx, hipMemcpyAsync(ctx->d_bid, bid, (size_t)n_reads * 4, hipMemcpyHostToDevice, st));
		HIP_TRY(ctx, hipMemcpyAsync(ctx->d_qlen, qlen, (size_t)n_reads * 4, hipMemcpyHostToDevice, st));
	}
	ctx->has_n_segs = n_segs_per_read != nullptr;
	if (n_segs_per_read && n_reads) HIP_TRY(ctx, hipMemcpyAsync(ctx->d_n_segs, n_segs_per_read, (size_t)n_reads * 4, hipMemcpyHostToDevice, st));
	chaindp::SeedIndex dix;
	dix.B = ix->blob[0]; dix.H = ix->blob[1]; dix.V = ix->blob[2]; dix.P = ix->blob[3];
	dix.nB = ix->bytes[0]; dix.nH = ix->bytes[1]; dix.nV = ix->bytes[2]; dix.nP = ix->bytes[3];
	dix.b_bits = ix->b_bits;
	HIP_TRY(ctx, chaindp::launch_seed_collect(st, dix, flag, max_occ, n_reads, n_mini, ctx->d_mini_off, ctx->d_mini, ctx->d_bid, ctx->seed,
	                                          ctx->d_off, ctx->d_mp_off, ctx->d_rep_len));
	unsigned long long totals[2] = {0, 0};
	HIP_TRY(ctx, hipMemcpyAsync(totals, ctx->seed.totals, 16, hipMemcpyDeviceToHost, st));
	HIP_TRY(ctx, hipStreamSynchronize(st));
	if ((int64_t)totals[0] > ctx->cap_anchors) {
		ctx->n_reads = 0; ctx->total = 0; ctx->ran = false; ctx->bot_n_reads = -1; ctx->mp_resident = false;
		ctx->err = "the batch's seeds exceed the anchor capacity the context was created with";
		return CHAINDP_ERR_CAPACITY;
	}
	if (!ctx->d_seeds) HIP_TRY(ctx, hipMalloc(&ctx->d_seeds, (size_t)ctx->cap_anchors * sizeof(chaindp_seed_t) + 16));
	if (ctx->seed_max_n < 0) {
		int lds_limit = 0;
		HIP_TRY(ctx, hipDeviceGetAttribute(&lds_limit, hipDeviceAttributeMaxSharedMemoryPerBlock, ctx->device));
		int m = 8192, m2 = 65024, cap = (lds_limit - 8192) & ~15;
		if (const char *v = getenv("CHAINDP_SEED_MAX_N")) { m = atoi(v) < m ? atoi(v) : m; if (const char *c = strchr(v, ',')) m2 = atoi(c + 1); }
		if (const char *v = getenv("CHAINDP_SEED_LAB_CAP")) cap = atoi(v) < cap ? atoi(v) & ~15 : cap;
		if (m < 64) m = 64;
		if (cap < 256) cap = 256;
		while (m > 0 && chaindp::seed_sort_lds_bytes(m, 32, 8) > (size_t)lds_limit) m -= 512;
		while (m2 > m && chaindp::seed_sort_lds_bytes(m2, 4, 2) > (size_t)lds_limit) m2 -= 64;
		ctx->seed_lab_cap = cap;
		ctx->seed_max_n = m; ctx->seed_max_n2 = m2;
	}
	HIP_TRY(ctx, chaindp::launch_seed_expand_sort(st, dix, flag, n_reads, n_mini, ctx->d_mini_off, ctx->d_mini, ctx->d_bid, ctx->d_qlen, ctx->seed,
	                                              ctx->d_seeds, ctx->d_a, ctx->d_off, ctx->d_mini_pos, ctx->seed_max_n, ctx->seed_max_n2,
	                                              ctx->seed_lab_cap, (int64_t)totals[0]));
	if (off) HIP_TRY(ctx, hipMemcpyAsync(off, ctx->d_off, (size_t)(n_reads + 1) * 8, hipMemcpyDeviceToHost, st));
	if (mini_pos_off) HIP_TRY(ctx, hipMemcpyAsync(mini_pos_off, ctx->d_mp_off, (size_t)(n_reads + 1) * 8, hipMemcpyDeviceToHost, st));
	if (rep_len && n_reads) HIP_TRY(ctx, hipMemcpyAsync(rep_len, ctx->d_rep_len, (size_t)n_reads * 4, hipMemcpyDeviceToHost, st));
	HIP_TRY(ctx, hipStreamSynchronize(st));
	ctx->n_reads = n_reads; ctx->total = (int64_t)totals[0]; ctx->n_mini_pos = (int64_t)totals[1]; ctx->ran = false; ctx->bot_n_reads = -1; ctx->mp_resident = true;
	return CHAINDP_OK;
}

extern "C" int chaindp_collect_seeds(chaindp_ctx_t *ctx, const chaindp_index_t *ix, int flag, int max_occ, int64_t n_reads,
                                     const int64_t *mini_off, const chaindp_anchor_t *mini, const uint32_t *bid, const int32_t *qlen,
                                     const int32_t *n_segs_per_read, int64_t *off, int32_t *rep_len, int64_t *mini_pos_off)
{
	return collect_seeds_impl(ctx, ix, flag, max_occ, n_reads, mini_off, mini, nullptr, bid, qlen, n_segs_per_read, off, rep_len, mini_pos_off);
}

extern "C" int chaindp_collect_seeds_gather(chaindp_ctx_t *ctx, const chaindp_index_t *ix, int flag, int max_occ, int64_t n_reads,
                                            const int64_t *mini_off, const chaindp_anchor_t *const *read_mini, const uint32_t *bid,
                                            const int32_t *qlen, const int32_t *n_segs_per_read, int64_t *off, int32_t *rep_len,
                                            int64_t *mini_pos_off)
{
	if (ctx && n_reads > 0 && !read_mini) { ctx->err = "bad minimizers"; return CHAINDP_ERR_ARG; }
	return collect_seeds_impl(ctx, ix, flag, max_occ, n_reads, mini_off, nullptr, read_mini, bid, qlen, n_segs_per_read, off, rep_len, mini_pos_off);
}

extern "C" int chaindp_map_batch(chaindp_ctx_t *ctx, const chaindp_index_t *ix, int flag, int max_occ, const chaindp_params_t *par, int min_cnt,
                                 int64_t n_reads, const int64_t *mini_off, const chaindp_anchor_t *mini, const uint32_t *bid, const int32_t *qlen,
                                 const uint32_t *hash, int64_t *regs_off, chaindp_reg_t *regs, int64_t regs_cap, int32_t *rep_len, int64_t *n_anchors)
{
	if (!ctx) return CHAINDP_ERR_ARG;
	int rc = check_params(ctx, par);
	if (rc) return rc;
	if (!regs_off || regs_cap < 0 || (regs_cap > 0 && !regs) || (n_reads > 0 && !hash)) { ctx->err = "NULL output or hash"; return CHAINDP_ERR_ARG; }
	if ((rc = collect_seeds_impl(ctx, ix, flag, max_occ, n_reads, mini_off, mini, nullptr, bid, qlen, nullptr, nullptr, rep_len, nullptr)) != CHAINDP_OK) return rc;
	if (n_anchors) *n_anchors = ctx->total;
	if ((rc = chaindp_run_full(ctx, par)) != CHAINDP_OK) return rc;
	std::vector<int64_t> b_off((size_t)(n_reads > 0 ? n_reads + 1 : 1));
	if ((rc = chaindp_backtrack(ctx, par, min_cnt, regs_off, nullptr, b_off.data(), nullptr)) != CHAINDP_OK) return rc;
	const int64_t n_c = n_reads > 0 ? regs_off[n_reads] : 0;
	if (n_c > regs_cap) { ctx->err = "more hits than regs has room for (regs_off is valid; chaindp_gen_regs with a larger buffer returns them)"; return CHAINDP_ERR_CAPACITY; }
	return chaindp_gen_regs(ctx, hash, qlen, regs);
}

extern "C" int chaindp_scatter_mini_pos(chaindp_ctx_t *ctx, int64_t n_reads, uint64_t *const *dst)
{
	if (!ctx) return CHAINDP_ERR_ARG;
	if (n_reads != ctx->n_reads || (n_reads > 0 && !dst) || !ctx->d_mp_off) { ctx->err = "scatter does not match the last seed collection"; return CHAINDP_ERR_ARG; }
	for (int64_t r = 0; r < n_reads; ++r) if ((uintptr_t)dst[r] & 15u) { ctx->err = "scatter destinations must be 16-byte aligned"; return CHAINDP_ERR_ARG; }
	HIP_TRY(ctx, hipSetDevice(ctx->device));
	int rc = stage_pointers(ctx, (const void *const *)dst, n_reads);
	if (rc) return rc;
	HIP_TRY(ctx, chaindp::launch_scatter_words(ctx->stream, n_reads, ctx->d_mp_off, (void *const *)ctx->d_ptrs, ctx->d_mini_pos));
	return CHAINDP_OK;
}

extern "C" int chaindp_download_mini_pos(chaindp_ctx_t *ctx, uint64_t *mini_pos)
{
	if (!ctx || (ctx->n_mini_pos > 0 && !mini_pos)) return CHAINDP_ERR_ARG;
	HIP_TRY(ctx, hipSetDevice(ctx->device));
	if (ctx->n_mini_pos) HIP_TRY(ctx, hipMemcpyAsync(mini_pos, ctx->d_mini_pos, (size_t)ctx->n_mini_pos * 8, hipMemcpyDeviceToHost, ctx->stream));
	HIP_TRY(ctx, hipStreamSynchronize(ctx->stream));
	return CHAINDP_OK;
}

extern "C" int chaindp_download_anchors(chaindp_ctx_t *ctx, chaindp_anchor_t *a)
{
	if (!ctx || (ctx->total > 0 && !a)) return CHAINDP_ERR_ARG;
	HIP_TRY(ctx, hipSetDevice(ctx->device));
	if (ctx->total) HIP_TRY(ctx, hipMemcpyAsync(a, ctx->d_a, (size_t)ctx->total * 16, hipMemcpyDeviceToHost, ctx->stream));
	HIP_TRY(ctx, hipStreamSynchronize(ctx->stream));
	return CHAINDP_OK;
}


struct PipeSlot {
	chaindp_ctx *ctx = nullptr;
	int64_t *h_seeds_off = nullptr;
	chaindp_seed_t *h_seeds = nullptr;
	unsigned long long *h_n_seeds = nullptr;
	hipEvent_t done = nullptr;
	hipEvent_t up = nullptr;
	int64_t tag = 0, n_reads = 0, total = 0;
	int state = 0;
};

struct chaindp_pipe {
	int device = -1, depth = 0;
	hipStream_t s_up = nullptr, s_down = nullptr;
	std::vector<PipeSlot> slots;
	int head = 0, tail = 0, inflight = 0;
	std::string err;
};

extern "C" const char *chaindp_pipe_last_error(const chaindp_pipe_t *pipe)
{
	return pipe ? pipe->err.c_str() : g_create_error.c_str();
}

extern "C" void chaindp_pipe_destroy(chaindp_pipe_t *pipe)
{
	if (!pipe) return;
	if (pipe->device >= 0) (void)hipSetDevice(pipe->device);
	for (auto &sl : pipe->slots) {
		if (sl.ctx && sl.ctx->stream) (void)hipStreamSynchronize(sl.ctx->stream);
		if (sl.done) (void)hipEventDestroy(sl.done);
		if (sl.up) (void)hipEventDestroy(sl.up);
		if (sl.h_seeds_off) (void)hipHostFree(sl.h_seeds_off);
		if (sl.h_seeds) (void)hipHostFree(sl.h_seeds);
		if (sl.h_n_seeds) (void)hipHostFree(sl.h_n_seeds);
		if (sl.ctx) chaindp_destroy(sl.ctx);
	}
	if (pipe->s_up) { (void)hipStreamSynchronize(pipe->s_up); (void)hipStreamDestroy(pipe->s_up); }
	if (pipe->s_down) { (void)hipStreamSynchronize(pipe->s_down); (void)hipStreamDestroy(pipe->s_down); }
	delete pipe;
}

extern "C" chaindp_pipe_t *chaindp_pipe_create(int device, int depth, int64_t max_anchors, int64_t max_reads)
{
	g_create_error.clear();
	if (depth < 1 || depth > 8) { g_create_error = "chaindp_pipe_create: depth must be 1..8"; return nullptr; }
	chaindp_pipe *pipe = new chaindp_pipe();
	pipe->device = device; pipe->depth = depth;
	pipe->slots.resize((size_t)depth);
	if (hipSetDevice(device) != hipSuccess || hipStreamCreateWithFlags(&pipe->s_up, hipStreamNonBlocking) != hipSuccess ||
	    hipStreamCreateWithFlags(&pipe->s_down, hipStreamNonBlocking) != hipSuccess) {
		g_create_error = "chaindp_pipe_create: no usable HIP device (there is no CPU fallback)";
		chaindp_pipe_destroy(pipe);
		return nullptr;
	}
	for (auto &sl : pipe->slots) {
		sl.ctx = chaindp_create(device, max_anchors, max_reads);
		if (!sl.ctx) { chaindp_pipe_destroy(pipe); return nullptr; }
		const size_t na = (size_t)sl.ctx->cap_anchors, nr = (size_t)sl.ctx->cap_reads;
		hipError_t e = hipHostMalloc((void**)&sl.h_seeds_off, (nr + 1) * 8, hipHostMallocDefault);
		if (e == hipSuccess) e = hipHostMalloc((void**)&sl.h_seeds, na * sizeof(chaindp_seed_t) + 16, hipHostMallocDefault);
		if (e == hipSuccess) e = hipHostMalloc((void**)&sl.h_n_seeds, 64, hipHostMallocDefault);
		if (e == hipSuccess) e = hipEventCreateWithFlags(&sl.done, hipEventDisableTiming);
		if (e == hipSuccess) e = hipEventCreateWithFlags(&sl.up, hipEventDisableTiming);
		if (e != hipSuccess) {
			g_create_error = std::string("chaindp_pipe_create: ") + hipGetErrorString(e);
			chaindp_pipe_destroy(pipe);
			return nullptr;
		}
	}
	return pipe;
}

#define PIPE_TRY(pipe, call)                                                                       \
	do {                                                                                           \
		hipError_t e_ = (call);                                                                    \
		if (e_ != hipSuccess) {                                                                    \
			(pipe)->err = std::string(#call) + ": " + hipGetErrorString(e_);                       \
			return CHAINDP_ERR_HIP;                                                                \
		}                                                                                          \
	} while (0)

extern "C" int chaindp_pipe_submit(chaindp_pipe_t *pipe, const chaindp_params_t *par, int64_t n_reads, const int64_t *off,
                                   const chaindp_anchor_t *a, const int32_t *n_segs_per_read, int64_t tag)
{
	if (!pipe) return CHAINDP_ERR_ARG;
	if (pipe->inflight == pipe->depth) { pipe->err = "every slot of the pipe is in flight: wait for the oldest batch first"; return CHAINDP_ERR_BUSY; }
	PipeSlot &sl = pipe->slots[(size_t)pipe->head];
	chaindp_ctx *ctx = sl.ctx;
	int rc = check_params(ctx, par);
	if (rc) { pipe->err = ctx->err; return rc; }
	if (n_reads < 0 || !off || (n_reads > 0 && off[0] != 0)) { pipe->err = "bad offsets"; return CHAINDP_ERR_ARG; }
	const int64_t total = n_reads > 0 ? off[n_reads] : 0;
	if (total < 0 || (total > 0 && !a)) { pipe->err = "bad anchors"; return CHAINDP_ERR_ARG; }
	if (n_reads > ctx->cap_reads || total > ctx->cap_anchors) { pipe->err = "batch exceeds the capacity the pipe was created with"; return CHAINDP_ERR_CAPACITY; }
	PIPE_TRY(pipe, hipSetDevice(pipe->device));
	hipStream_t st = ctx->stream;
	PIPE_TRY(pipe, hipMemcpyAsync(ctx->d_off, off, (size_t)(n_reads + 1) * 8, hipMemcpyHostToDevice, pipe->s_up));
	if (total) PIPE_TRY(pipe, hipMemcpyAsync(ctx->d_a, a, (size_t)total * 16, hipMemcpyHostToDevice, pipe->s_up));
	ctx->has_n_segs = n_segs_per_read != nullptr;
	if (n_segs_per_read && n_reads) PIPE_TRY(pipe, hipMemcpyAsync(ctx->d_n_segs, n_segs_per_read, (size_t)n_reads * 4, hipMemcpyHostToDevice, pipe->s_up));
	PIPE_TRY(pipe, hipEventRecord(sl.up, pipe->s_up));
	PIPE_TRY(pipe, hipStreamWaitEvent(st, sl.up, 0));
	ctx->n_reads = n_reads; ctx->total = total; ctx->ran = false; ctx->bot_n_reads = -1; ctx->mp_resident = false;
	rc = chaindp_run_full(ctx, par);
	if (rc) { pipe->err = ctx->err; return rc; }
	PIPE_TRY(pipe, hipMemcpyAsync(sl.h_seeds_off, ctx->d_seeds_off, (size_t)(n_reads + 1) * 8, hipMemcpyDeviceToHost, st));
	PIPE_TRY(pipe, hipMemcpyAsync(sl.h_n_seeds, ctx->cmp.n_seeds, 8, hipMemcpyDeviceToHost, st));
	PIPE_TRY(pipe, hipEventRecord(sl.done, st));
	sl.tag = tag; sl.n_reads = n_reads; sl.total = total; sl.state = 1;
	pipe->head = (pipe->head + 1) % pipe->depth;
	++pipe->inflight;
	return CHAINDP_OK;
}

extern "C" int chaindp_pipe_wait(chaindp_pipe_t *pipe, chaindp_pipe_result_t *res)
{
	if (!pipe || !res) return CHAINDP_ERR_ARG;
	PipeSlot &sl = pipe->slots[(size_t)pipe->tail];
	if (pipe->inflight == 0 || sl.state != 1) { pipe->err = sl.state == 2 ? "release the batch waited for first" : "nothing in flight"; return CHAINDP_ERR_BUSY; }
	PIPE_TRY(pipe, hipSetDevice(pipe->device));
	PIPE_TRY(pipe, hipEventSynchronize(sl.done));
	const int64_t m = sl.total > 0 && sl.n_reads > 0 ? (int64_t)(uint32_t)*sl.h_n_seeds : 0;
	sl.ctx->n_seeds = m;
	if (m > 0) {
		static const int copy_blocks = getenv("CHAINDP_PIPE_COPY_BLOCKS") ? atoi(getenv("CHAINDP_PIPE_COPY_BLOCKS")) : 64;
		if (copy_blocks > 0) PIPE_TRY(pipe, chaindp::launch_copy_out(pipe->s_down, sl.h_seeds, sl.ctx->d_seeds, (size_t)m * sizeof(chaindp_seed_t), copy_blocks));
		else PIPE_TRY(pipe, hipMemcpyAsync(sl.h_seeds, sl.ctx->d_seeds, (size_t)m * sizeof(chaindp_seed_t), hipMemcpyDeviceToHost, pipe->s_down));
		PIPE_TRY(pipe, hipStreamSynchronize(pipe->s_down));
	}
	if (sl.n_reads == 0) sl.h_seeds_off[0] = 0;
	res->tag = sl.tag; res->n_reads = sl.n_reads; res->n_anchors = sl.total; res->n_seeds = m;
	res->seeds_off = sl.h_seeds_off; res->seeds = sl.h_seeds;
	sl.state = 2;
	return CHAINDP_OK;
}

extern "C" int chaindp_pipe_release(chaindp_pipe_t *pipe)
{
	if (!pipe) return CHAINDP_ERR_ARG;
	PipeSlot &sl = pipe->slots[(size_t)pipe->tail];
	if (sl.state != 2) { pipe->err = "no waited batch to release"; return CHAINDP_ERR_ARG; }
	sl.state = 0;
	pipe->tail = (pipe->tail + 1) % pipe->depth;
	--pipe->inflight;
	return CHAINDP_OK;
}


static std::once_flag g_logf_once;
static std::vector<uint32_t> g_logf_k;
static std::vector<float> g_logf_v;
static float (*volatile g_host_logf)(float) = logf;
static double (*volatile g_host_log)(double) = log;

static void build_logf_patches()
{
	std::call_once(g_logf_once, [] {
		float (*lf)(float) = g_host_logf;
		double (*ld)(double) = g_host_log;
		for (uint32_t k = 1; k <= (uint32_t)POST_LOGF_MAX; ++k) {
			const float h = lf((float)k), c = (float)ld((double)k);
			if (memcmp(&h, &c, 4) != 0) { g_logf_k.push_back(k); g_logf_v.push_back(h); }
		}
	});
}

extern "C" int64_t chaindp_post_logf_patches(uint32_t *k, float *v, int64_t cap)
{
	build_logf_patches();
	const int64_t n = (int64_t)g_logf_k.size();
	for (int64_t i = 0; i < n && i < cap; ++i) { if (k) k[i] = g_logf_k[(size_t)i]; if (v) v[i] = g_logf_v[(size_t)i]; }
	return n;
}

static int post_logf_upload(chaindp_ctx *ctx)
{
	if (ctx->n_logf >= 0) return CHAINDP_OK;
	build_logf_patches();
	const size_t n = g_logf_k.size();
	HIP_TRY(ctx, bot_alloc(ctx, ctx->d_logf_k, (n ? n : 1) * 4));
	HIP_TRY(ctx, bot_alloc(ctx, ctx->d_logf_v, (n ? n : 1) * 4));
	if (n) {
		HIP_TRY(ctx, hipMemcpy(ctx->d_logf_k, g_logf_k.data(), n * 4, hipMemcpyHostToDevice));
		HIP_TRY(ctx, hipMemcpy(ctx->d_logf_v, g_logf_v.data(), n * 4, hipMemcpyHostToDevice));
	}
	ctx->n_logf = (int)n;
	return CHAINDP_OK;
}

extern "C" int64_t chaindp_post_logf_selftest(chaindp_ctx_t *ctx, int32_t kmax)
{
	if (!ctx) return CHAINDP_ERR_ARG;
	if (kmax < 1 || kmax > POST_LOGF_MAX) { ctx->err = "kmax must lie in [1, 2^24]"; return CHAINDP_ERR_ARG; }
	HIP_TRY(ctx, hipSetDevice(ctx->device));
	int rc = post_logf_upload(ctx);
	if (rc) return rc;
	float *d_out = nullptr;
	HIP_TRY(ctx, hipMalloc(&d_out, (size_t)kmax * 8));
	int32_t *d_term = (int32_t*)(d_out + kmax);
	std::vector<float> dev((size_t)kmax);
	std::vector<int32_t> term((size_t)kmax);
	hipError_t e = chaindp::launch_post_logf_probe(ctx->stream, kmax, ctx->d_logf_k, ctx->d_logf_v, ctx->n_logf, d_out, d_term);
	if (e == hipSuccess) e = hipMemcpyAsync(dev.data(), d_out, (size_t)kmax * 4, hipMemcpyDeviceToHost, ctx->stream);
	if (e == hipSuccess) e = hipMemcpyAsync(term.data(), d_term, (size_t)kmax * 4, hipMemcpyDeviceToHost, ctx->stream);
	if (e == hipSuccess) e = hipStreamSynchronize(ctx->stream);
	(void)hipFree(d_out);
	if (e != hipSuccess) { ctx->err = std::string("logf self-test: ") + hipGetErrorString(e); return CHAINDP_ERR_HIP; }
	float (*lf)(float) = g_host_logf;
	int64_t bad = 0;
	for (int32_t k = 1; k <= kmax; ++k) {
		const float h = lf((float)k);
		const int t = (int)(4.343f * h + .499f);
		bad += memcmp(&h, &dev[(size_t)k - 1], 4) != 0 || t != term[(size_t)k - 1];
	}
	return bad;
}

static chaindp::PostOpt to_post_opt(const chaindp_post_opt_t *o)
{
	chaindp::PostOpt p;
	p.flag = o->flag; p.mask_level = o->mask_level; p.pri_ratio = o->pri_ratio; p.best_n = o->best_n; p.min_diff = o->min_diff;
	p.sub_diff = o->sub_diff; p.max_join_long = o->max_join_long; p.max_join_short = o->max_join_short;
	p.min_join_flank_sc = o->min_join_flank_sc; p.min_cnt = o->min_cnt; p.min_chain_score = o->min_chain_score; p.match_sc = o->match_sc;
	p.is_sr = o->is_sr;
	return p;
}

extern "C" int chaindp_chain_post(chaindp_ctx_t *ctx, const chaindp_post_opt_t *opt, const int32_t *qlen, const int32_t *rep_len,
                                  const int32_t *ref_len, int32_t n_ref, const int64_t *mini_pos_off, const uint64_t *mini_pos,
                                  int64_t *regs_off, chaindp_reg_t *regs, int64_t regs_cap, int64_t *a_off, chaindp_anchor_t *a)
{
	if (!ctx) return CHAINDP_ERR_ARG;
	if (!opt || !regs_off || regs_cap < 0 || (regs_cap > 0 && !regs) || n_ref < 0 || (n_ref > 0 && !ref_len) || (a && !a_off)) {
		ctx->err = "NULL argument"; return CHAINDP_ERR_ARG;
	}
	if (ctx->bot_n_reads < 0 || ctx->bot_n_reads != ctx->n_reads || !ctx->bot.has || !ctx->regs_resident) {
		ctx->err = "chaindp_chain_post needs the hits of a chaindp_gen_regs on this batch (a chaindp_est_err since has replaced them)";
		return CHAINDP_ERR_ARG;
	}
	const int64_t R = ctx->bot_n_reads, n_c = ctx->bot_n_chains, n_b = ctx->bot_n_b;
	const bool do_mapq = !(opt->flag & CHAINDP_F_CIGAR), do_err = !opt->is_sr;
	hipStream_t st = ctx->stream;
	HIP_TRY(ctx, hipSetDevice(ctx->device));
	if (ctx->ran_par.n_segs > 1 && !ctx->has_n_segs) { ctx->err = "chaindp_chain_post takes single-segment reads only (n_segs > 1)"; return CHAINDP_ERR_ARG; }
	if (ctx->has_n_segs && R > 0) {
		std::vector<int32_t> ns((size_t)R);
		HIP_TRY(ctx, hipMemcpyAsync(ns.data(), ctx->d_n_segs, (size_t)R * 4, hipMemcpyDeviceToHost, st));
		HIP_TRY(ctx, hipStreamSynchronize(st));
		for (int32_t v : ns) if (v > 1) { ctx->err = "chaindp_chain_post takes single-segment reads only (n_segs > 1)"; return CHAINDP_ERR_ARG; }
	}
	if (R == 0) { regs_off[0] = 0; if (a_off) a_off[0] = 0; return CHAINDP_OK; }
	if (n_c == 0) {
		for (int64_t r = 0; r <= R; ++r) regs_off[r] = 0;
		if (a_off) for (int64_t r = 0; r <= R; ++r) a_off[r] = 0;
		return CHAINDP_OK;
	}
	const bool mp_given = mini_pos != nullptr || mini_pos_off != nullptr;
	if (do_err && !mp_given && (!ctx->mp_resident || !ctx->d_mp_off)) { ctx->err = "no resident mini_pos: pass the arrays, or collect the seeds with chaindp_collect_seeds"; return CHAINDP_ERR_ARG; }
	if (do_err && mp_given && !mini_pos_off) { ctx->err = "mini_pos without offsets"; return CHAINDP_ERR_ARG; }
	if (do_mapq && !rep_len && !ctx->mp_resident) { ctx->err = "no resident rep_len: pass it, or collect the seeds with chaindp_collect_seeds"; return CHAINDP_ERR_ARG; }
	int rc = regs_per_read_buffers(ctx);
	if (rc) return rc;
	if ((rc = post_logf_upload(ctx)) != CHAINDP_OK) return rc;
	const size_t RB = (size_t)ctx->cap_reads + 2;
	if (!ctx->d_post_off) {
		HIP_TRY(ctx, bot_alloc(ctx, ctx->d_post_off, RB * 8)); HIP_TRY(ctx, bot_alloc(ctx, ctx->d_post_tile, (RB / 1024 + 2) * 8));
		HIP_TRY(ctx, bot_alloc(ctx, ctx->d_post_qlen, RB * 4)); HIP_TRY(ctx, bot_alloc(ctx, ctx->d_post_rep, RB * 4));
		HIP_TRY(ctx, bot_alloc(ctx, ctx->d_post_err, 4));
	}
	HIP_TRY(ctx, regs_grow(ctx, ctx->d_post_stage, ctx->post_stage_cap, (size_t)n_c * sizeof(chaindp_reg_t)));
	HIP_TRY(ctx, regs_grow(ctx, ctx->d_post_out, ctx->post_out_cap, (size_t)n_c * sizeof(chaindp_reg_t)));
	HIP_TRY(ctx, regs_grow(ctx, ctx->d_post_sq, ctx->post_sq_cap, (size_t)(n_b > 0 ? n_b : 1) * 16));
	HIP_TRY(ctx, regs_grow(ctx, ctx->d_post_scratch, ctx->post_scratch_cap, (size_t)n_c * POST_SCRATCH_INTS * 4));
	const int32_t *d_qlen = ctx->d_rqlen;
	if (qlen) { HIP_TRY(ctx, hipMemcpyAsync(ctx->d_post_qlen, qlen, (size_t)R * 4, hipMemcpyHostToDevice, st)); d_qlen = ctx->d_post_qlen; }
	const int32_t *d_rep = ctx->d_rep_len;
	if (rep_len) { HIP_TRY(ctx, hipMemcpyAsync(ctx->d_post_rep, rep_len, (size_t)R * 4, hipMemcpyHostToDevice, st)); d_rep = ctx->d_post_rep; }
	HIP_TRY(ctx, hipMemsetAsync(ctx->d_post_err, 0, 4, st));
	const chaindp::PostOpt po = to_post_opt(opt);
	HIP_TRY(ctx, chaindp::launch_post_read(st, R, ctx->bot.chains_off, ctx->bot.b_off, ctx->bot.b_out, ctx->d_regs, d_qlen, po,
	                                       (int32_t*)ctx->d_post_scratch, ctx->d_post_stage, ctx->d_post_sq, ctx->d_post_off));
	HIP_TRY(ctx, chaindp::launch_scan_u64(st, R, ctx->d_post_off, ctx->d_post_tile, ctx->d_post_off + R));
	HIP_TRY(ctx, chaindp::launch_post_scatter(st, R, ctx->bot.chains_off, ctx->d_post_off, ctx->d_post_stage, ctx->d_post_out));
	HIP_TRY(ctx, hipMemcpyAsync(regs_off, ctx->d_post_off, (size_t)(R + 1) * 8, hipMemcpyDeviceToHost, st));
	HIP_TRY(ctx, hipStreamSynchronize(st));
	const int64_t n_out = regs_off[R];
	if (n_out > regs_cap) { ctx->err = "more hits than regs has room for (regs_off is valid)"; return CHAINDP_ERR_CAPACITY; }
	if (do_err && n_out > 0) {
		const int64_t *d_mpo = ctx->d_mp_off;
		const unsigned long long *d_mp = ctx->d_mini_pos;
		if (mp_given) {
			const int64_t n_mp = mini_pos_off[R];
			if (n_mp < 0 || (n_mp > 0 && !mini_pos)) { ctx->err = "mini_pos announced but absent"; return CHAINDP_ERR_ARG; }
			HIP_TRY(ctx, regs_grow(ctx, ctx->d_mp_up, ctx->mp_up_cap, (size_t)(n_mp > 0 ? n_mp : 1) * 8));
			HIP_TRY(ctx, hipMemcpyAsync(ctx->d_mp_off_up, mini_pos_off, (size_t)(R + 1) * 8, hipMemcpyHostToDevice, st));
			if (n_mp > 0) HIP_TRY(ctx, hipMemcpyAsync(ctx->d_mp_up, mini_pos, (size_t)n_mp * 8, hipMemcpyHostToDevice, st));
			d_mpo = ctx->d_mp_off_up; d_mp = (const unsigned long long*)ctx->d_mp_up;
		}
		HIP_TRY(ctx, regs_grow(ctx, ctx->d_ref_len, ctx->ref_len_cap, (size_t)(n_ref > 0 ? n_ref : 1) * 4));
		if (n_ref > 0) HIP_TRY(ctx, hipMemcpyAsync(ctx->d_ref_len, ref_len, (size_t)n_ref * 4, hipMemcpyHostToDevice, st));
		HIP_TRY(ctx, chaindp::launch_est_err(st, R, n_out, (const int64_t*)ctx->d_post_off, ctx->bot.b_off, ctx->d_post_sq, d_qlen,
		                                     (const int32_t*)ctx->d_ref_len, n_ref, d_mpo, d_mp, ctx->d_sum_k, ctx->d_post_out, nullptr));
	}
	if (do_mapq && n_out > 0)
		HIP_TRY(ctx, chaindp::launch_post_mapq(st, R, ctx->d_post_off, d_rep, opt->min_chain_score, ctx->d_logf_k, ctx->d_logf_v, ctx->n_logf,
		                                       ctx->d_post_out, ctx->d_post_err));
	int32_t err = 0;
	if (n_out > 0) HIP_TRY(ctx, hipMemcpyAsync(regs, ctx->d_post_out, (size_t)n_out * sizeof(chaindp_reg_t), hipMemcpyDeviceToHost, st));
	if (a_off) HIP_TRY(ctx, hipMemcpyAsync(a_off, ctx->bot.b_off, (size_t)(R + 1) * 8, hipMemcpyDeviceToHost, st));
	if (a && n_b > 0) HIP_TRY(ctx, hipMemcpyAsync(a, ctx->d_post_sq, (size_t)n_b * 16, hipMemcpyDeviceToHost, st));
	HIP_TRY(ctx, hipMemcpyAsync(&err, ctx->d_post_err, 4, hipMemcpyDeviceToHost, st));
	HIP_TRY(ctx, hipStreamSynchronize(st));
	if (err) { ctx->err = "a score or n_sub + 1 above 2^24: beyond the logf patch list"; return CHAINDP_ERR_CAPACITY; }
	return CHAINDP_OK;
}

extern "C" int chaindp_map_reads(chaindp_ctx_t *ctx, const chaindp_index_t *ix, int flag, int max_occ, const chaindp_params_t *par, int min_cnt,
                                 const chaindp_post_opt_t *opt, int64_t n_reads, const int64_t *mini_off, const chaindp_anchor_t *mini, const uint32_t *bid,
                                 const int32_t *qlen, const uint32_t *hash, const int32_t *ref_len, int32_t n_ref, int64_t *regs_off, chaindp_reg_t *regs,
                                 int64_t regs_cap, int32_t *rep_len, int64_t *n_anchors)
{
	if (!ctx) return CHAINDP_ERR_ARG;
	int rc = check_params(ctx, par);
	if (rc) return rc;
	if (!opt || !regs_off || regs_cap < 0 || (regs_cap > 0 && !regs) || (n_reads > 0 && !hash)) { ctx->err = "NULL output, hash or opt"; return CHAINDP_ERR_ARG; }
	if (par->n_segs > 1) { ctx->err = "chaindp_map_reads takes single-segment reads only (n_segs > 1)"; return CHAINDP_ERR_ARG; }
	if ((rc = collect_seeds_impl(ctx, ix, flag, max_occ, n_reads, mini_off, mini, nullptr, bid, qlen, nullptr, nullptr, rep_len, nullptr)) != CHAINDP_OK) return rc;
	if (n_anchors) *n_anchors = ctx->total;
	if ((rc = chaindp_run_full(ctx, par)) != CHAINDP_OK) return rc;
	std::vector<int64_t> c_off((size_t)(n_reads > 0 ? n_reads + 1 : 1)), b_off(c_off.size());
	if ((rc = chaindp_backtrack(ctx, par, min_cnt, c_off.data(), nullptr, b_off.data(), nullptr)) != CHAINDP_OK) return rc;
	if ((rc = gen_regs_impl(ctx, hash, qlen, nullptr, false)) != CHAINDP_OK) return rc;
	return chaindp_chain_post(ctx, opt, nullptr, nullptr, ref_len, n_ref, nullptr, nullptr, regs_off, regs, regs_cap, nullptr, nullptr);
}
```

### minimap2_chaindp_amd/csrc/chaindp_kernels.h

```cpp
#ifndef CHAINDP_KERNELS_H
#define CHAINDP_KERNELS_H

#include <hip/hip_runtime.h>
#include <stdint.h>

namespace chaindp {

struct Params {
	int32_t max_dist_x, max_dist_y, bw, max_skip, min_sc, is_cdna, n_segs;
};

struct Unit {
	int64_t start;
	int32_t read;
	int32_t len;
};

struct UnitAux {
	int32_t rel0;
	uint32_t lutkey;
	uint32_t flags;
	uint32_t pad;
};

#define CHAINDP_BLOCK_ANCHORS 1024

struct PrepassScratch {
	uint64_t *start_mask;
	uint64_t *single_mask;
	uint64_t *emit_mask;
	unsigned long long *block_cnt;
	unsigned long long *tile_tmp;
	Unit *units_tmp;
	unsigned int *hist;
	int2 *block_reads;
	unsigned int *key_range;
};
size_t prepass_scratch_bytes(int64_t max_anchors, size_t *mask_bytes, size_t *blocks_bytes);

hipError_t launch_prepass(hipStream_t st, const Params &par, int64_t n_reads, int64_t total, const int64_t *d_off, const void *d_a,
                          unsigned long long *d_sumq, Unit *d_units, unsigned long long *d_counters, PrepassScratch sc,
                          UnitAux *d_unit_aux = nullptr, const int32_t *d_n_segs = nullptr,
                          unsigned long long *d_left_cnt = nullptr);
hipError_t launch_fill_singles(hipStream_t st, const Params &par, int64_t total, const void *d_a, PrepassScratch sc,
                               int32_t *d_f, int32_t *d_p, int32_t *d_v, uint8_t *d_flags);

#define CHAINDP_LUT_MAX_BW 4095
hipError_t launch_lut(hipStream_t st, const Params &par, int64_t n_reads, const int64_t *d_off,
                      unsigned long long *d_sumq, int lut_stride, uint16_t *d_lut);
size_t chain_lds_bytes(int ring, int lut_stride);

hipError_t launch_chain(hipStream_t st, int ring, const Params &par, int64_t max_units, const int64_t *d_off, const void *d_a,
                        const int32_t *d_n_segs, const unsigned long long *d_sumq, const uint16_t *d_lut, int lut_stride,
                        const Unit *d_units, const unsigned long long *d_counters,
                        int32_t *d_f, int32_t *d_p, int32_t *d_v, unsigned long long *d_tg, uint32_t epoch, int32_t *d_first_child, uint8_t *d_flags,
                        const Unit *d_units_all = nullptr, const unsigned long long *d_counters_all = nullptr,
                        Unit *d_deep = nullptr, unsigned int *d_deep_cnt = nullptr, const unsigned int *d_long_units = nullptr,
                        int deep_eager = 0,
                        int deep_route = 0);
#define CHAINDP_LONG_UNIT_CLASS 65
#define CHAINDP_DENSE_MAX_LONG 4096u
#define CHAINDP_DENSE_BITCAP 65536
#define CHAINDP_DENSE_RING 512
#define CHAINDP_DENSE_UNITS 2048u
hipError_t launch_chain_dense(hipStream_t st, const Params &par, int64_t max_units, const int64_t *d_off, const void *d_a,
                              const uint16_t *d_lut, int lut_stride, const Unit *d_deep, const unsigned long long *d_deep_cnt,
                              int32_t *d_f, int32_t *d_p, int32_t *d_v, int32_t *d_first_child, uint8_t *d_flags,
                              const unsigned int *d_long_units, int deep_route, unsigned int *d_queue);
hipError_t launch_chain_dense16(hipStream_t st, const Params &par, int64_t max_units, const int64_t *d_off, const void *d_a,
                              const uint16_t *d_lut, int lut_stride, const Unit *d_deep, const unsigned long long *d_deep_cnt,
                              int32_t *d_f, int32_t *d_p, int32_t *d_v, int32_t *d_first_child, uint8_t *d_flags,
                              const unsigned int *d_long_units, int deep_route, unsigned int *d_queue);
hipError_t launch_chain_dense1(hipStream_t st, const Params &par, int64_t max_units, const int64_t *d_off, const void *d_a,
                               const uint16_t *d_lut, int lut_stride, const Unit *d_deep, const unsigned long long *d_deep_cnt,
                               const unsigned int *d_long_units, int deep_route, unsigned int *d_queues,
                               int32_t *d_f, int32_t *d_p, int32_t *d_v, int32_t *d_first_child, uint8_t *d_flags);

hipError_t launch_chain_twin(hipStream_t st, const Params &par, int64_t max_units, const int64_t *d_off, const void *d_a,
                             const unsigned long long *d_sumq, const uint16_t *d_lut, int lut_stride, const Unit *d_units,
                             const unsigned long long *d_counters, int32_t *d_f, int32_t *d_p, int32_t *d_v,
                             int32_t *d_first_child, uint8_t *d_flags, Unit *d_left, unsigned int *d_left_cnt, int force_left, int64_t total,
                             const UnitAux *d_unit_aux, const unsigned int *d_route = nullptr, unsigned int *d_queue = nullptr   );
size_t twin_lds_bytes();

hipError_t launch_chain_quad(hipStream_t st, const Params &par, int64_t max_units, const void *d_a, const uint16_t *d_lut, int lut_stride,
                             const Unit *d_units, const UnitAux *d_unit_aux, const unsigned long long *d_counters, const unsigned int *d_key_range,
                             int32_t *d_f, int32_t *d_p, int32_t *d_v, int32_t *d_first_child, uint8_t *d_flags, Unit *d_left,
                             unsigned int *d_left_cnt, unsigned int *d_queue, unsigned int *d_route, int force_left, int64_t total);
size_t quad_lds_bytes();

hipError_t launch_scan_u64(hipStream_t st, int64_t n, unsigned long long *d_data, unsigned long long *d_tile_tmp,
                           unsigned long long *d_total);

struct CompactScratch {
	uint8_t *flags;
	unsigned long long *block_cnt;
	unsigned long long *tile_tmp;
	unsigned long long *n_seeds;
	const int2 *block_reads;
	const uint64_t *single_mask, *emit_mask;
	uint32_t *sub;
};
size_t compact_scratch_bytes(int64_t max_anchors, size_t *flags_bytes, size_t *blocks_bytes);
hipError_t launch_compact(hipStream_t st, const Params &par, int64_t n_reads, int64_t total, const int64_t *d_off,
                          const void *d_a, const int32_t *d_f, const int32_t *d_p, const int32_t *d_v,
                          int32_t *d_first_child, int64_t *d_seeds_off, void *d_seeds,
                          CompactScratch sc);

struct BottomScratch {
	uint8_t *has;
	int32_t *owner, *end_rec, *ccnt, *kpos, *bpos, *c_src, *c_dst;
	unsigned long long *key, *skey, *cu, *u_tmp, *u_out;
	void *b_tmp, *b_out, *w;
	void *stacks;
	unsigned long long *block_cnt, *tile_tmp, *read_tot, *total;
	int64_t *ends_off, *chains_off, *b_off;
};
hipError_t launch_backtrack(hipStream_t st, int min_cnt, int min_sc, int64_t n_reads, int64_t m_cap, const int64_t *d_soff, const void *d_seeds,
                            const unsigned long long *d_n_seeds, BottomScratch sc, int64_t n_seeds_host);

hipError_t launch_gen_regs(hipStream_t st, int64_t n_reads, const int64_t *d_chains_off, const int64_t *d_b_off, const unsigned long long *d_u,
                           const void *d_b, const uint32_t *d_hash, const int32_t *d_qlen, void *d_z, void *d_stacks, void *d_regs);
hipError_t launch_est_err(hipStream_t st, int64_t n_reads, int64_t n_regs, const int64_t *d_regs_off, const int64_t *d_b_off, const void *d_b,
                          const int32_t *d_qlen, const int32_t *d_ref_len, int32_t n_ref, const int64_t *d_mp_off, const unsigned long long *d_mini_pos,
                          unsigned long long *d_sum_k, void *d_regs, int32_t *d_counts);

#define POST_LDS_CAP 256
#define POST_LOGF_MAX (1 << 24)
#define POST_F_SPLICE 0x080
#define POST_F_NO_LJOIN 0x400
#define POST_F_SR 0x1000
#define POST_F_ALL_CHAINS 0x800000
#define POST_SCRATCH_INTS 20
struct PostOpt {
	int32_t flag;
	float mask_level, pri_ratio;
	int32_t best_n, min_diff, sub_diff, max_join_long, max_join_short, min_join_flank_sc, min_cnt, min_chain_score, match_sc, is_sr;
};
hipError_t launch_post_read(hipStream_t st, int64_t n_reads, const int64_t *d_chains_off, const int64_t *d_b_off, const void *d_b, const void *d_regs,
                            const int32_t *d_qlen, const PostOpt &o, int32_t *d_scratch, void *d_stage, void *d_sq, unsigned long long *d_n_out);
hipError_t launch_post_scatter(hipStream_t st, int64_t n_reads, const int64_t *d_chains_off, const unsigned long long *d_out_off, const void *d_stage,
                               void *d_out);
hipError_t launch_post_mapq(hipStream_t st, int64_t n_reads, const unsigned long long *d_out_off, const int32_t *d_rep_len, int min_chain_sc,
                            const uint32_t *d_pk, const float *d_pv, int n_patch, void *d_out, int32_t *d_err);
hipError_t launch_post_logf_probe(hipStream_t st, int kmax, const uint32_t *d_pk, const float *d_pv, int n_patch, float *d_out, int32_t *d_term);

struct SeedIndex {
	const uint8_t *B, *H, *V, *P;
	uint64_t nB, nH, nV, nP;
	int b_bits;
};
struct SeedScratch {
	unsigned long long *kept, *used;
	unsigned long long *src, *mstate;
	unsigned long long *tile_tmp;
	unsigned long long *totals;
	void *stacks;
	uint32_t *tied;
};
hipError_t launch_seed_collect(hipStream_t st, const SeedIndex &ix, int flag, int max_occ, int64_t n_reads, int64_t n_mini,
                               const int64_t *d_mini_off, const void *d_mini, const uint32_t *d_bid, SeedScratch sc,
                               int64_t *d_off, int64_t *d_mp_off, int32_t *d_rep_len);
hipError_t launch_seed_expand_sort(hipStream_t st, const SeedIndex &ix, int flag, int64_t n_reads, int64_t n_mini,
                                   const int64_t *d_mini_off, const void *d_mini, const uint32_t *d_bid, const int32_t *d_qlen, SeedScratch sc,
                                   void *d_unsorted, void *d_a, const int64_t *d_off, unsigned long long *d_mini_pos, int max_n, int max_n2,
                                   int lab_cap, int64_t total);
size_t seed_sort_lds_bytes(int max_n, int workers, int coop);

hipError_t launch_gather_reads(hipStream_t st, int64_t n_reads, const int64_t *d_off, const void *const *d_src, void *d_a);
hipError_t launch_scatter_seeds(hipStream_t st, int64_t n_reads, const int64_t *d_seeds_off, void *const *d_dst, const void *d_seeds);
hipError_t launch_copy_out(hipStream_t st, void *h_dst, const void *d_src, size_t bytes, int blocks);
hipError_t launch_scatter_words(hipStream_t st, int64_t n_reads, const int64_t *d_woff, void *const *d_dst, const void *d_words);

hipError_t check_no_static_lds(const void *fn);

}
#endif
```

### minimap2_chaindp_amd/csrc/chaindp_lanes.h

```cpp
#ifndef CHAINDP_LANES_H
#define CHAINDP_LANES_H

#include <hip/hip_runtime.h>
#include <stdint.h>

namespace chaindp {

#if defined(__HIP_DEVICE_COMPILE__)
#define TW_LDS(T, a) ((__attribute__((address_space(3))) T*)(a))
#else
#define TW_LDS(T, a) ((T*)(uintptr_t)(a))
#endif
#if defined(__HIP_DEVICE_COMPILE__)
#define TW_CONST(T, p) ((const __attribute__((address_space(4))) T*)(uintptr_t)(p))
#else
#define TW_CONST(T, p) ((const T*)(p))
#endif
typedef uint32_t tw_u32x2 __attribute__((ext_vector_type(2)));
typedef uint32_t tw_u32x4 __attribute__((ext_vector_type(4)));

__device__ __forceinline__ tw_u32x2 tw_ld64(uint32_t a) { return *TW_LDS(const tw_u32x2, a); }
__device__ __forceinline__ int tw_ld32(uint32_t a) { return *TW_LDS(const int, a); }
__device__ __forceinline__ int tw_ld_i8(uint32_t a) { return (int)*TW_LDS(const signed char, a); }
__device__ __forceinline__ int tw_ld_u8(uint32_t a) { return (int)*TW_LDS(const unsigned char, a); }
__device__ __forceinline__ tw_u32x4 tw_ld128(uint32_t a) { return *TW_LDS(const tw_u32x4, a); }
__device__ __forceinline__ void tw_st64(uint32_t a, uint32_t x, uint32_t y) { tw_u32x2 t; t.x = x; t.y = y; *TW_LDS(tw_u32x2, a) = t; }
__device__ __forceinline__ void tw_st32(uint32_t a, int v) { *TW_LDS(int, a) = v; }
__device__ __forceinline__ void tw_st8(uint32_t a, int v) { *TW_LDS(signed char, a) = (signed char)v; }
__device__ __forceinline__ void tw_st128(uint32_t a, uint32_t x, uint32_t y, uint32_t z, uint32_t w) { tw_u32x4 t; t.x = x; t.y = y; t.z = z; t.w = w; *TW_LDS(tw_u32x4, a) = t; }

#if defined(__HIP_DEVICE_COMPILE__)
#define TW_VREG(x) asm volatile("" : "+v"(x))
#else
#define TW_VREG(x) ((void)(x))
#endif

#define TW_UNI(x) ((uint32_t)__builtin_amdgcn_readfirstlane((int)(x)))

__device__ __forceinline__ uint32_t tw_sad(uint32_t a, uint32_t b, uint32_t c)
{
	uint32_t d = 0;
#if defined(__HIP_DEVICE_COMPILE__)
	asm("v_sad_u32 %0, %1, %2, %3" : "=v"(d) : "v"(a), "v"(b), "v"(c));
#endif
	return d;
}

#define TW_ULT(a, b) __builtin_amdgcn_uicmp((unsigned)(a), (unsigned)(b), 36)
#define TW_EQ(a, b)  __builtin_amdgcn_uicmp((unsigned)(a), (unsigned)(b), 32)
#define TW_SGT(a, b) __builtin_amdgcn_sicmp((int)(a), (int)(b), 38)
#define TW_SGE(a, b) __builtin_amdgcn_sicmp((int)(a), (int)(b), 39)
#define TW_SEL(m, a, b) (__builtin_amdgcn_inverse_ballot_w64(m) ? (a) : (b))

}
#endif
```

### minimap2_chaindp_amd/csrc/chaindp_twin.hip

```cpp
#include <hip/hip_runtime.h>
#include <stdint.h>
#include <limits.h>
#include <stdio.h>
#include <stdlib.h>
#include <vector>
#include "chaindp_kernels.h"
#include "chaindp_wave.h"
#include "chaindp_lanes.h"

namespace chaindp {

#define TW_XY 0u
#define TW_PF 2048u
#define TW_V 3072u
#define TW_XQ 3584u
#define TW_XQ_HALF 512u
#define TW_LUT 4608u
#define TW_LUT_HALF 512u
#define TW_ST 5632u
#define TW_ST_HALF 56u
#define TW_MK 5744u
#define TW_MK_HALF 260u
#define TW_SP 6264u
#define TW_SP_HALF 64u
#define TW_SP_OF_XQ (TW_SP - TW_XQ / 8u)
#define TW_KEY 6392u
#define TW_LDS_BYTES 6400u
#define TW_TILE 64
#define TW_RING 64
#define TW_QCH 8

__device__ __forceinline__ int tw_excl_max32(int v)
{
	v = max(v, __builtin_amdgcn_update_dpp(0, v, DPP_ROW_SHR(1), 0xf, 0xf, true));
	v = max(v, __builtin_amdgcn_update_dpp(0, v, DPP_ROW_SHR(2), 0xf, 0xf, true));
	v = max(v, __builtin_amdgcn_update_dpp(0, v, DPP_ROW_SHR(4), 0xf, 0xf, true));
	v = max(v, __builtin_amdgcn_update_dpp(0, v, DPP_ROW_SHR(8), 0xf, 0xf, true));
	int e = __builtin_amdgcn_update_dpp(0, v, DPP_ROW_SHR(1), 0xf, 0xf, true);
#if defined(__HIP_DEVICE_COMPILE__)
	asm("s_nop 1\n\tv_max_i32_dpp %0, %1, %0 row_bcast:15 row_mask:0xa bank_mask:0xf" : "+v"(e) : "v"(v));
#endif
	return e;
}
__device__ __forceinline__ int tw_incl_min32(int v)
{
	v = min(v, dpp_or_old<DPP_ROW_SHR(1), 0xf>(INT_MAX, v));
	v = min(v, dpp_or_old<DPP_ROW_SHR(2), 0xf>(INT_MAX, v));
	v = min(v, dpp_or_old<DPP_ROW_SHR(4), 0xf>(INT_MAX, v));
	v = min(v, dpp_or_old<DPP_ROW_SHR(8), 0xf>(INT_MAX, v));
	v = min(v, dpp_or_old<DPP_ROW_BCAST15, 0xa>(INT_MAX, v));
	return v;
}

__device__ __forceinline__ int tw_below_in_half(uint64_t m, bool hi_half)
{
	const int lo = (int)__builtin_amdgcn_mbcnt_lo((uint32_t)m, 0u);
	const int hi = (int)__builtin_amdgcn_mbcnt_hi((uint32_t)(m >> 32), 0u);
	return hi_half ? hi : lo;
}

__device__ __forceinline__ uint64_t tw_smear_halves(uint64_t m)
{
	uint32_t lo = 0, hi = 0;
#if defined(__HIP_DEVICE_COMPILE__)
	asm("s_cmp_lg_u32 %2, 0\n\ts_cselect_b32 %0, -1, 0\n\ts_cmp_lg_u32 %3, 0\n\ts_cselect_b32 %1, -1, 0"
	    : "=&s"(lo), "=&s"(hi) : "s"(TW_UNI((uint32_t)m)), "s"(TW_UNI((uint32_t)(m >> 32))) : "scc");
#endif
	return (uint64_t)hi << 32 | lo;
}

__device__ __forceinline__ uint64_t tw_last_or_lane0(uint64_t m)
{
	uint32_t lo = 0, hi = 0;
#if defined(__HIP_DEVICE_COMPILE__)
	asm("s_flbit_i32_b32 %0, %2\n\ts_flbit_i32_b32 %1, %3\n\ts_lshr_b32 %0, 0x80000000, %0\n\ts_lshr_b32 %1, 0x80000000, %1"
	    : "=&s"(lo), "=&s"(hi) : "s"(TW_UNI((uint32_t)m)), "s"(TW_UNI((uint32_t)(m >> 32))));
#endif
	return (uint64_t)hi << 32 | lo;
}

__device__ __forceinline__ uint32_t tw_both_halves(uint64_t m)
{
	uint32_t t = 0;
#if defined(__HIP_DEVICE_COMPILE__)
	asm("s_cmp_lg_u32 %1, 0\n\ts_cselect_b32 %0, %2, 0" : "=s"(t) : "s"(TW_UNI((uint32_t)m)), "s"(TW_UNI((uint32_t)(m >> 32))) : "scc");
#endif
	return t;
}

__device__ __forceinline__ uint64_t tw_below_first(uint64_t m, uint64_t b)
{
	const uint32_t blo = (uint32_t)b, bhi = (uint32_t)(b >> 32);
	const uint32_t klo = blo ? (blo & (0u - blo)) - 1u : 0xffffffffu, khi = bhi ? (bhi & (0u - bhi)) - 1u : 0xffffffffu;
	return m & ((uint64_t)khi << 32 | klo);
}

#define TW_HI31 0x8000000080000000ull

struct TwinArgs {
	Params par;
	const int64_t *off;
	const ulonglong2 *a;
	const unsigned long long *sumq;
	const uint16_t *lut;
	int lut_stride;
	const Unit *units;
	const UnitAux *aux;
	const unsigned long long *counters;
	int32_t *f, *p, *v;
	int32_t *first_child;
	uint8_t *flags;
	Unit *left;
	unsigned int *left_cnt;
	unsigned int *queue;
	const unsigned int *route;
	int force_left;
	int64_t total;
	unsigned long long *stamp;
};

struct TwinCold {
	int64_t next;
	int64_t base;
	uint64_t x_carry;
	int32_t rel0, room, read, tile0;
};

struct TwinHot {
	uint32_t S;
	uint32_t m4;
	uint32_t pc, pend;
};
#define TW_CARRY 40u

#ifdef CHAINDP_TWIN_STAMPS
#define TW_STAMP(...) __VA_ARGS__
#else
#define TW_STAMP(...)
#endif
#if defined(CHAINDP_TWIN_STAMPS) && CHAINDP_TWIN_STAMPS == 2
#define TW_STAMP_A(...)
#define TW_STAMP_B(...) __VA_ARGS__
#elif defined(CHAINDP_TWIN_STAMPS) && CHAINDP_TWIN_STAMPS == 1
#define TW_STAMP_A(...) __VA_ARGS__
#define TW_STAMP_B(...)
#else
#define TW_STAMP_A(...)
#define TW_STAMP_B(...)
#endif
#if defined(CHAINDP_TWIN_STAMPS) && CHAINDP_TWIN_STAMPS == 3
#define TW_STAMP_C(...) __VA_ARGS__
#else
#define TW_STAMP_C(...)
#endif
#define TW_NOW() __builtin_amdgcn_s_memtime()

template <bool SAMEGAP>
__global__ __launch_bounds__(64) __attribute__((amdgpu_waves_per_eu(6, 6))) void k_chain_twin(TwinArgs g)
{
	const int lane = threadIdx.x;
	const bool hi_half = lane >= 32;
	const int h = lane >> 5, hl = lane & 31;

	uint32_t L16 = (uint32_t)hl << 4;
	const uint32_t mkbase = TW_MK + TW_MK_HALF * (uint32_t)h;
	const uint32_t curbase = TW_XQ + TW_XQ_HALF * (uint32_t)h;
	uint32_t c_mkbase = mkbase;
	uint32_t c_far = mkbase + 256u;
	uint32_t c_own = mkbase + ((uint32_t)hl << 2);
	uint32_t c_lut = TW_LUT + TW_LUT_HALF * (uint32_t)h;
	uint32_t c_8h = (uint32_t)h << 3;
	uint32_t c_M = (uint32_t)g.par.max_dist_x;
	uint32_t c_bw = (uint32_t)g.par.bw;
	uint32_t c_cbw = c_M - 1u > c_bw ? c_M - 1u - c_bw : 0u;
	const uint32_t mdq = (uint32_t)(g.par.max_dist_x < g.par.max_dist_y ? g.par.max_dist_x : g.par.max_dist_y);
	uint32_t c_dqoff = c_M - mdq;
	int c_ms = g.par.max_skip;
	int c_min = INT_MIN;
	int c_Mout = hl == 31 ? g.par.max_dist_x : INT_MAX;
	uint32_t c_bwl = c_bw + c_lut;
	uint32_t c_cbwl = c_cbw - c_lut;
	TW_VREG(L16); TW_VREG(c_far); TW_VREG(c_own); TW_VREG(c_lut); TW_VREG(c_M);
	if (!SAMEGAP) TW_VREG(c_dqoff);
	TW_VREG(c_ms); TW_VREG(c_min); TW_VREG(c_Mout); TW_VREG(c_bwl); TW_VREG(c_cbwl);

	const uint64_t maxx = (uint64_t)(int64_t)g.par.max_dist_x;
	if (g.route && *g.route) return;
	const int64_t n_units = (int64_t)(uint32_t)g.counters[0];
	const int64_t n_single = (int64_t)(g.counters[0] >> 32);
	const bool short_units = (g.total - n_single) <= 512 * n_units;
	if (!short_units) {
		if (blockIdx.x == 0 && lane == 0) *g.left_cnt = 0xffffffffu;
		return;
	}
	const bool params_ok = g.lut != nullptr && !g.par.is_cdna && g.par.max_dist_x >= 1 && g.par.max_dist_y >= 0 &&
	                       ((uint64_t)(int64_t)g.par.max_dist_x + 1) * 129ull < (1ull << 31) && g.par.bw + 1 <= (int)TW_LUT_HALF && g.force_left != 1;

	TwinHot u;
	u.S = 0; u.m4 = 0; u.pc = curbase; u.pend = curbase;
	uint64_t live_m = ~0ull;
	uint64_t contm = 0;
	const uint32_t st_addr = TW_ST + TW_ST_HALF * (uint32_t)h;
#define TW_COLD (*TW_LDS(TwinCold, st_addr))
	const uint32_t xcd = blockIdx.x & 7u;
	const uint32_t n_halves = 2u * gridDim.x;
#ifndef TW_END_UNITS
#define TW_END_UNITS 16u
#define TW_PIECE 1u
#endif
	const uint32_t U1 = n_units > (long long)TW_END_UNITS * n_halves ? ((uint32_t)n_units - TW_END_UNITS * n_halves) & ~(8u * TW_QCH - 1u) : 0u;
	const uint32_t G1k = U1 / (8u * TW_QCH);
	auto grab = [&](uint32_t p, uint32_t &nx, uint32_t &ne) {
		if (p < G1k) { nx = (8u * p + xcd) * TW_QCH; ne = nx + TW_QCH; }
		else { nx = U1 + TW_PIECE * (8u * (p - G1k) + xcd); ne = nx + TW_PIECE; }
	};
	if (hl == 0) {
		uint32_t nx, ne;
		grab(((blockIdx.x >> 3) << 1) | (uint32_t)h, nx, ne);
		tw_st64(st_addr, nx, ne); tw_st64(st_addr + 8u, 0u, 0u);
		tw_st64(st_addr + 16u, 0u, 0u); tw_st64(st_addr + 24u, 0u, 0u);
		tw_st64(st_addr + 32u, 0u, (uint32_t)-TW_TILE);
		tw_st64(st_addr + TW_CARRY, 0xfffffffcu, 0u); tw_st64(st_addr + TW_CARRY + 8u, 0u, 0u);
		tw_st32(TW_KEY + 4u * (uint32_t)h, -1);
	}
	wave_mem_fence();

	TW_STAMP(unsigned long long st_t0 = 0; unsigned int st_service = 0, st_n_service = 0, st_n_fast = 0, st_flush = 0, st_unit = 0, st_n_unit = 0, st_head = 0, st_take = 0, st_tail = 0;)
	uint64_t nx0_x = 0, nx0_y = 0, nx1_x = 0, nx1_y = 0;
	int32_t pfu0 = -1, pfu1 = -1;

	auto service = [&](uint64_t svc) {
#if defined(__HIP_DEVICE_COMPILE__)
		asm volatile("s_waitcnt vmcnt(0)" ::: "memory");
#endif
		wave_mem_fence();
		uint64_t retired = 0;
		for (int hs = 0; hs < 2; ++hs) {
			if (((svc >> (32 * hs)) & 1ull) == 0) continue;
			TW_STAMP_B(const unsigned long long th0 = g.stamp ? TW_NOW() : 0;)
			const uint64_t hm = hs ? 0xffffffff00000000ull : 0x00000000ffffffffull;
			const uint32_t sa = TW_ST + TW_ST_HALF * (uint32_t)hs;
			const uint32_t curb = TW_XQ + TW_XQ_HALF * (uint32_t)hs, spb = TW_SP + TW_SP_HALF * (uint32_t)hs;
			const uint32_t mkb = TW_MK + TW_MK_HALF * (uint32_t)hs, lutb = TW_LUT + TW_LUT_HALF * (uint32_t)hs;
			const tw_u32x2 cw0 = tw_ld64(sa), cw1 = tw_ld64(sa + 8u), cw2 = tw_ld64(sa + 16u), cw3 = tw_ld64(sa + 24u), cw4 = tw_ld64(sa + 32u);
			int64_t c_next = (int64_t)((uint64_t)TW_UNI(cw0.y) << 32 | TW_UNI(cw0.x));
			int64_t c_base = (int64_t)((uint64_t)TW_UNI(cw1.y) << 32 | TW_UNI(cw1.x));
			uint64_t c_xcarry = (uint64_t)TW_UNI(cw2.y) << 32 | TW_UNI(cw2.x);
			int c_rel0 = (int)TW_UNI(cw3.x), c_room = (int)TW_UNI(cw3.y), c_read = (int)TW_UNI(cw4.x), c_tile0 = (int)TW_UNI(cw4.y);
			const int cnt_prev = (int)(((uint32_t)__builtin_amdgcn_readlane((int)u.pend, 32 * hs) - curb) >> 3);
			const int slow_h = (int)TW_UNI((uint32_t)tw_ld32(sa + TW_CARRY + 12u));
			const uint32_t cur_key = TW_UNI((uint32_t)tw_ld32(TW_KEY + 4u * (uint32_t)hs));
			const int tile_prev = c_tile0, rel0_prev = c_rel0;
			const int64_t base_prev = c_base;
			bool live = true;
			const uint32_t nx0 = (uint32_t)c_next, ne0 = (uint32_t)((uint64_t)c_next >> 32);
			tw_u32x4 rec0 = {0u, 0u, 0u, 0u}, aux0 = {0u, 0u, 0u, 0u}, rec1 = {0u, 0u, 0u, 0u};
			const bool rec0_ok = nx0 < ne0 && (int64_t)nx0 < n_units;
			const bool rec1_ok = rec0_ok && nx0 + 1u < ne0 && (int64_t)nx0 + 1 < n_units;
			if (rec0_ok) { rec0 = *TW_CONST(tw_u32x4, g.units + nx0); aux0 = *TW_CONST(tw_u32x4, g.aux + nx0); }
			if (rec1_ok) rec1 = *TW_CONST(tw_u32x4, g.units + nx0 + 1u);

			auto take_tile = [&](const uint64_t an_x, const uint64_t an_y) -> int {
				const int i_lane = c_tile0 + lane;
				const bool have = i_lane < c_room;
				uint64_t xp;
				{
					uint32_t lo = (uint32_t)wave_shift_up1((int)(uint32_t)an_x, 0), hi = (uint32_t)wave_shift_up1((int)(uint32_t)(an_x >> 32), 0);
					if (lane == 0) { lo = (uint32_t)c_xcarry; hi = (uint32_t)(c_xcarry >> 32); }
					xp = (uint64_t)hi << 32 | lo;
				}
				const bool stop = !have || (i_lane > 0 && an_x - xp > maxx);
				const uint64_t stop_m = __builtin_amdgcn_ballot_w64(stop);
				const int cnt = stop_m ? __builtin_ctzll(stop_m) : TW_TILE;
				c_xcarry = readlane_u64(an_x, 63);
				u.pc = TW_SEL(hm, curb, u.pc); u.pend = TW_SEL(hm, curb + ((uint32_t)cnt << 3), u.pend);
				if (cnt == 0) return 0;
				wave_mem_fence();
				if (lane < cnt) {
					const int sp = span_of_hi((uint32_t)(an_y >> 32));
					tw_st64((((uint32_t)i_lane & 127u) << 4 | (uint32_t)hs << 3) + TW_XY, (uint32_t)an_x + 1u, (uint32_t)an_y + 1u);
					tw_st64(curb + ((uint32_t)lane << 3), (uint32_t)an_x, (uint32_t)an_y);
					tw_st8(spb + (uint32_t)lane, sp - 1);
					g.first_child[c_base + i_lane] = NO_CHILD;
				}
				wave_mem_fence();
				if (cnt == TW_TILE && c_tile0 + TW_TILE < c_room) {
					uint64_t rx = 0, ry = 0;
					if (i_lane + TW_TILE < c_room) { const ulonglong2 t = g.a[c_base + i_lane + TW_TILE]; rx = t.x; ry = t.y; }
					if (hs) { nx1_x = rx; nx1_y = ry; pfu1 = -1; } else { nx0_x = rx; nx0_y = ry; pfu0 = -1; }
				}
				return cnt;
			};

			bool goes_on = cnt_prev == TW_TILE && c_tile0 + TW_TILE < c_room;
			if (goes_on && (slow_h * 8 > c_tile0 + TW_TILE || g.force_left == 2)) {
				if (lane == 0) {
					Unit un; un.start = (int64_t)((uint64_t)c_base | (uint64_t)(uint32_t)(c_tile0 + TW_TILE) << 32); un.read = c_read; un.len = c_room;
					g.left[atomicAdd(g.left_cnt, 1u)] = un;
				}
				goes_on = false;
			}
			if (goes_on) {
				c_tile0 += TW_TILE;
				if (take_tile(hs ? nx1_x : nx0_x, hs ? nx1_y : nx0_y) == 0) goes_on = false;
			}
			TW_STAMP_B(if (g.stamp) st_take += (unsigned int)(TW_NOW() - th0);)
			TW_STAMP_A(const unsigned long long tf0 = g.stamp ? TW_NOW() : 0;)
			if (cnt_prev > 0) {
				const int i_lane = tile_prev + lane;
				const bool have = lane < cnt_prev;
				const int64_t gi = base_prev + i_lane;
				int fi = 0, p4 = -4;
				if (have) {
					const tw_u32x2 pf = tw_ld64((((uint32_t)i_lane & 63u) << 4 | (uint32_t)hs << 3) + TW_PF);
					p4 = (int)pf.x; fi = (int)pf.y + 1;
				}
				const int pi = p4 >> 2;
				int val = fi, ptr = have ? pi : -1;
				const bool ext = ptr >= 0 && ptr < tile_prev;
				int vext = 0;
				if (ext) {
					vext = tw_ld32((((uint32_t)ptr & 63u) << 3 | (uint32_t)hs << 2) + TW_V);
					val = max(val, vext & 0x7fffffff);
					ptr = -1;
				}
				const bool ext_self = ext && vext < 0;
				for (int r = 0; r < 6; ++r) {
					if (__builtin_amdgcn_ballot_w64(ptr >= tile_prev) == 0) break;
					const int src = (ptr >= tile_prev ? ptr - tile_prev : lane) << 2;
					const int pv = __builtin_amdgcn_ds_bpermute(src, val);
					const int pp = __builtin_amdgcn_ds_bpermute(src, ptr);
					if (ptr >= tile_prev) { val = max(val, pv); ptr = pp; }
				}
				const bool self = val >= g.par.min_sc || pi >= 0;
				const int srcp = (pi >= tile_prev ? pi - tile_prev : lane) << 2;
				const int pself_in = __builtin_amdgcn_ds_bpermute(srcp, self ? 1 : 0);
				const bool pred_self = ext ? ext_self : pself_in != 0;
				wave_mem_fence();
				if (have) tw_st32((((uint32_t)i_lane & 63u) << 3 | (uint32_t)hs << 2) + TW_V, val | (self ? INT_MIN : 0));
				wave_mem_fence();
				if (have) {
					g.f[gi] = fi;
					g.p[gi] = pi < 0 ? -1 : pi + rel0_prev;
					g.v[gi] = val;
					int maybe_first = 0;
					if (pi >= 0 && !pred_self) { atomicMin(&g.first_child[base_prev + pi], rel0_prev + i_lane); maybe_first = 4; }
					g.flags[gi] = (uint8_t)((self ? 2 : 0) | maybe_first | (val >= g.par.min_sc ? 8 : 0) | (fi < val ? 16 : 0));
				}
			}
			TW_STAMP_A(if (g.stamp) st_flush += (unsigned int)(TW_NOW() - tf0);)
			TW_STAMP_A(const unsigned long long tu0 = g.stamp ? TW_NOW() : 0;)
			TW_STAMP_A(if (g.stamp && !goes_on) ++st_n_unit;)
			bool have_rec = rec0_ok;
			const bool rec0_used = !goes_on;
			uint32_t cur_key_now = cur_key;
			while (!goes_on && live) {
				uint32_t nx = (uint32_t)c_next, ne = (uint32_t)((uint64_t)c_next >> 32);
				if (nx >= ne) {
					uint32_t q0 = 0;
					if (lane == 0) q0 = atomicAdd(g.queue + 64u * xcd, 1u);
					grab(TW_UNI(q0), nx, ne);
					have_rec = false;
				}
				if ((int64_t)nx >= n_units) {
					c_next = (int64_t)((uint64_t)ne << 32 | nx); live = false;
					u.pc = TW_SEL(hm, curb, u.pc); u.pend = TW_SEL(hm, curb, u.pend);
					break;
				}
				TW_STAMP_C(const unsigned long long tc0 = g.stamp ? TW_NOW() : 0;)
				if (!have_rec) { rec0 = *TW_CONST(tw_u32x4, g.units + nx); aux0 = *TW_CONST(tw_u32x4, g.aux + nx); }
				have_rec = false;
				TW_STAMP_C(if (g.stamp) { asm volatile("" :: "s"(rec0.x), "s"(aux0.x)); st_head += (unsigned int)(TW_NOW() - tc0); })
				c_next = (int64_t)((uint64_t)ne << 32 | (nx + 1u));
				Unit un;
				un.start = (int64_t)((uint64_t)rec0.y << 32 | rec0.x); un.read = (int32_t)rec0.z; un.len = (int32_t)rec0.w;
				if (!params_ok || (aux0.z & 1u) || g.par.n_segs > 1) {
					if (lane == 0) g.left[atomicAdd(g.left_cnt, 1u)] = un;
					continue;
				}
				c_base = un.start; c_rel0 = (int)aux0.x; c_room = un.len; c_read = un.read; c_tile0 = 0;
				uint64_t tl_x, tl_y;
				TW_STAMP_C(const unsigned long long tc1 = g.stamp ? TW_NOW() : 0;)
				TW_STAMP_C(if (g.stamp && (hs ? pfu1 : pfu0) == (int32_t)c_base) ++st_n_unit;)
				if ((hs ? pfu1 : pfu0) == (int32_t)c_base) { tl_x = hs ? nx1_x : nx0_x; tl_y = hs ? nx1_y : nx0_y; }
				else {
					tl_x = 0; tl_y = 0;
					if (lane < c_room) { const ulonglong2 t = g.a[c_base + lane]; tl_x = t.x; tl_y = t.y; }
				}
				if (hs) pfu1 = -1; else pfu0 = -1;
				TW_STAMP_C(if (g.stamp) { asm volatile("" :: "v"(tl_x), "v"(tl_y)); asm volatile("s_waitcnt vmcnt(0)" ::: "memory"); st_take += (unsigned int)(TW_NOW() - tc1); })
				TW_STAMP_C(const unsigned long long tc2 = g.stamp ? TW_NOW() : 0;)
				wave_mem_fence();
				if (aux0.y != cur_key_now) {
					const uint2 *src = (const uint2*)(g.lut + (int64_t)c_read * g.lut_stride);
					for (int k = lane; k * 4 <= g.par.bw; k += 64) {
						const uint2 t = src[k];
						const uint32_t w = (t.x & 0xffu) | (t.x >> 8 & 0xff00u) | (t.y << 16 & 0xff0000u) | (t.y << 8 & 0xff000000u);
						tw_st32(lutb + ((uint32_t)k << 2), (int)w);
					}
					cur_key_now = aux0.y;
					if (lane == 0) tw_st32(TW_KEY + 4u * (uint32_t)hs, (int)cur_key_now);
				}
				const uint32_t x_none = (uint32_t)__builtin_amdgcn_readlane((int)(uint32_t)tl_x, 0) - (uint32_t)maxx - 1u;
				for (int k = lane; k < 128; k += 64) tw_st64(((uint32_t)k << 4 | (uint32_t)hs << 3) + TW_XY, x_none, 0u);
				for (int k = lane; k < 65; k += 64) tw_st32(mkb + ((uint32_t)k << 2), -1);
				wave_mem_fence();
				c_xcarry = 0;
				if (lane == 0) tw_st32(sa + TW_CARRY + 12u, 0);
				if (take_tile(tl_x, tl_y) > 0) goes_on = true;
				TW_STAMP_C(if (g.stamp) { st_tail += (unsigned int)(TW_NOW() - tc2); ++st_unit; })
			}
			if (live) {
				const uint32_t cnt_now = ((uint32_t)__builtin_amdgcn_readlane((int)u.pend, 32 * hs) - curb) >> 3;
				const uint32_t nxn = (uint32_t)c_next, nen = (uint32_t)((uint64_t)c_next >> 32);
				if (!(cnt_now == TW_TILE && c_tile0 + TW_TILE < c_room) && (hs ? pfu1 : pfu0) < 0 && nxn < nen && (int64_t)nxn < n_units &&
				    ((nxn == nx0 && rec0_ok && !rec0_used) || (nxn == nx0 + 1u && rec1_ok))) {
					const tw_u32x4 rn = nxn == nx0 ? rec0 : rec1;
					const int32_t st = (int32_t)rn.x, ln = (int32_t)rn.w;
					uint64_t rx = 0, ry = 0;
					if (lane < ln) { const ulonglong2 t = g.a[(int64_t)st + lane]; rx = t.x; ry = t.y; }
					if (hs) { nx1_x = rx; nx1_y = ry; pfu1 = st; } else { nx0_x = rx; nx0_y = ry; pfu0 = st; }
				}
			}
			TW_STAMP_A(if (g.stamp) st_unit += (unsigned int)(TW_NOW() - tu0);)
			if (live) {
				const uint32_t i = (uint32_t)c_tile0;
				u.S = TW_SEL(hm, (i - 1u) << 4 | (uint32_t)hs << 3, u.S); u.m4 = TW_SEL(hm, ((i - 1u) << 2) + mkb, u.m4);
			} else retired |= hm;
			if (lane == 0) {
				tw_st64(sa, (uint32_t)c_next, (uint32_t)((uint64_t)c_next >> 32)); tw_st64(sa + 8u, (uint32_t)c_base, (uint32_t)((uint64_t)c_base >> 32));
				tw_st64(sa + 16u, (uint32_t)c_xcarry, (uint32_t)(c_xcarry >> 32)); tw_st64(sa + 24u, (uint32_t)c_rel0, (uint32_t)c_room);
				tw_st64(sa + 32u, (uint32_t)c_read, (uint32_t)c_tile0);
			}
		}
		wave_mem_fence();
		live_m &= ~retired;
		contm &= ~svc;
	};

	auto slow_tail = [&](uint64_t D, uint32_t a_cur, int nskip_after) -> uint64_t {
		const uint64_t giveup = ~D & contm;
		const int vlast = __builtin_amdgcn_ds_bpermute(((h << 5) + 31) << 2, nskip_after);
		wave_mem_fence();
		const tw_u32x2 cur = tw_ld64(a_cur);
		if (__builtin_amdgcn_inverse_ballot_w64(D)) {
			u.m4 += 4u;
			u.S = ((u.m4 - c_mkbase) << 2) | c_8h;
			u.pc += 8u;
		} else {
			if (hl == 0) {
				tw_st64(st_addr + TW_CARRY, cur.x, cur.y);
				tw_st32(st_addr + TW_CARRY + 8u, vlast);
				tw_st32(st_addr + TW_CARRY + 12u, tw_ld32(st_addr + TW_CARRY + 12u) + 1);
			}
			u.S -= 512u;
		}
		contm = ~D & ~giveup & live_m;
		if (__builtin_expect(giveup != 0, 0)) {
			if (__builtin_amdgcn_inverse_ballot_w64(giveup)) {
				wave_mem_fence();
				if (hl == 0) {
					const TwinCold c = TW_COLD;
					Unit un; un.start = (int64_t)((uint64_t)c.base | (uint64_t)(uint32_t)c.tile0 << 32); un.read = c.read; un.len = c.room;
					g.left[atomicAdd(g.left_cnt, 1u)] = un;
				}
				u.pc = curbase; u.pend = curbase;
			}
			return giveup;
		}
		return 0;
	};

	TW_STAMP(if (g.stamp) st_t0 = TW_NOW();)
	service(~0ull);
	bool force_general = false;
	while (live_m != 0) {
		wave_mem_fence();
		uint64_t svc = 0;
		if (__builtin_expect(contm == 0 && live_m == ~0ull && !force_general, 1)) {
			uint64_t B, X, tile;
			int cB;
			uint32_t a_cur;
			for (;;) {
				const uint32_t t0 = u.S - L16;
				const tw_u32x2 xy = tw_ld64((t0 & 0x7f8u) + TW_XY);
				const tw_u32x2 pf = tw_ld64((t0 & 0x3f8u) + TW_PF);
				const tw_u32x2 cur = tw_ld64(u.pc);
				const int spm1 = tw_ld_u8((u.pc >> 3) + TW_SP_OF_XQ);
				const uint32_t drm1 = cur.x - xy.x, dqm1 = cur.y - xy.y;
				const uint32_t ddl = tw_sad(drm1, dqm1, c_lut);
				const uint32_t dqs = SAMEGAP ? dqm1 : __builtin_elementwise_add_sat(dqm1, c_dqoff);
				const uint32_t m3 = max(max(drm1, dqs), ddl + c_cbwl);
				const uint64_t okm = TW_ULT(m3, c_M);
				const uint32_t dst = TW_SEL(okm, min(u.m4 - pf.x, c_far), c_far);
				tw_st32(dst, (int)u.m4);
				wave_mem_fence();
				const int tj = tw_ld32(c_own);
				const int lutv = tw_ld_i8(min(ddl, c_bwl));
#if defined(__HIP_DEVICE_COMPILE__)
				__builtin_amdgcn_sched_barrier(0);
#endif
				const int sc0 = min(min((int)dqm1, (int)drm1), spm1);
				const int sc = TW_SEL(okm, sc0 + (int)pf.y + lutv, c_min);
				const int excl = max(tw_excl_max32(sc), spm1);
				const uint64_t A = TW_SGT(sc, excl);
				B = TW_EQ(tj, u.m4) & okm & ~A;
				const uint64_t OUT = TW_SGE(drm1, c_Mout);
				cB = tw_below_in_half(B, hi_half);
				tile = 0; X = 0; a_cur = 0;
				if (__builtin_expect((TW_SGT(cB, 0) & A) != 0, 0)) { force_general = true; break; }
				const uint32_t S1 = u.S + 16u;
				a_cur = S1 & 0x3f8u;
				{
					const uint32_t wp = TW_SEL(A, u.m4 - c_own, 0xfffffffcu);
					const int wf = TW_SEL(A, sc, spm1);
					if (__builtin_amdgcn_inverse_ballot_w64(tw_last_or_lane0(A))) tw_st64(a_cur + TW_PF, wp, (uint32_t)wf);
				}
				X = (TW_SGE(cB, c_ms) & B) | OUT;
				if (__builtin_expect(tw_both_halves(X) == 0, 0)) break;
				u.m4 += 4u; u.S = S1;
				u.pc += 8u;
				tile = TW_SGE(u.pc, u.pend);
				TW_STAMP(if (g.stamp) ++st_n_fast;)
				if (__builtin_expect(tile != 0, 0)) break;
				wave_mem_fence();
			}
			if (!force_general && tile == 0) {
				svc = slow_tail(tw_smear_halves(X), a_cur + TW_PF, cB + (int)__builtin_amdgcn_inverse_ballot_w64(B));
			}
		} else {
			force_general = false;
			const uint32_t t0 = u.S - L16;
			const tw_u32x2 xy = tw_ld64((t0 & 0x7f8u) + TW_XY);
			const tw_u32x2 pf = tw_ld64((t0 & 0x3f8u) + TW_PF);
			const tw_u32x2 cur = tw_ld64(u.pc);
			const int spm1 = tw_ld_u8((u.pc >> 3) + TW_SP_OF_XQ);
			const uint64_t first = ~contm;
			const tw_u32x2 carry = tw_ld64(st_addr + TW_CARRY);
			const int maxf = TW_SEL(first, spm1, (int)carry.y);
			const uint32_t maxj4 = TW_SEL(first, 0xfffffffcu, carry.x);
			const int nskip0 = TW_SEL(first, 0, tw_ld32(st_addr + TW_CARRY + 8u));
			const uint32_t kb4 = TW_SEL(first, 0u, 128u);
			const uint32_t drm1 = cur.x - xy.x, dqm1 = cur.y - xy.y;
			const uint32_t ddl = tw_sad(drm1, dqm1, c_lut);
			const uint32_t dqs = SAMEGAP ? dqm1 : __builtin_elementwise_add_sat(dqm1, c_dqoff);
			const uint32_t m3 = max(max(drm1, dqs), ddl + c_cbwl);
			const uint64_t okm = TW_ULT(m3, c_M) & ~(contm & TW_HI31) & live_m;
			const int sc0 = min(min((int)dqm1, (int)drm1), spm1);
			const int lutv = tw_ld_i8(min(ddl, c_bwl));
			const uint32_t dst = TW_SEL(okm, min(u.m4 - pf.x, c_far), c_far);
			tw_st32(dst, (int)u.m4);
			wave_mem_fence();
			const int tj = tw_ld32(c_own + kb4);
			const int sc = TW_SEL(okm, sc0 + (int)pf.y + lutv, c_min);
			const int excl = max(tw_excl_max32(sc), maxf);
			const uint64_t A = TW_SGT(sc, excl);
			const uint64_t B = TW_EQ(tj, u.m4) & okm & ~A;
			const uint64_t OUT = TW_SGE(drm1, c_M);
			const int cB = tw_below_in_half(B, hi_half), cA = tw_below_in_half(A, hi_half);
			const int isA = (int)__builtin_amdgcn_inverse_ballot_w64(A), isB = (int)__builtin_amdgcn_inverse_ballot_w64(B);
			const uint64_t inter = TW_SGT(cB, 0) & A;
			uint64_t brk, Ap;
			int nskip_after;
			if (inter == 0) {
				nskip_after = max(nskip0 - cA - isA, 0) + cB + isB;
				brk = TW_SGT(nskip_after, c_ms) & B;
				Ap = A;
			} else {
				const int Sk = nskip0 + cB + isB - cA - isA;
				nskip_after = Sk - min(tw_incl_min32(Sk), 0);
				brk = TW_SGT(nskip_after, c_ms) & B;
				Ap = tw_below_first(A, brk);
			}
			const uint32_t a_cur = (((((u.m4 - c_mkbase) + 4u) << 2) & 0x3f8u) | c_8h) + TW_PF;
			{
				const uint32_t wp = TW_SEL(Ap, u.m4 - c_own - kb4, maxj4);
				const int wf = TW_SEL(Ap, sc, maxf);
				if (__builtin_amdgcn_inverse_ballot_w64(tw_last_or_lane0(Ap))) tw_st64(a_cur, wp, (uint32_t)wf);
			}
			const uint64_t D = tw_smear_halves(brk | (OUT & TW_HI31) | ~live_m);
			svc = slow_tail(D, a_cur, nskip_after);
		}
		svc |= tw_smear_halves(TW_SGE(u.pc, u.pend) & live_m & ~contm);
		if (__builtin_expect(svc != 0, 0)) {
			TW_STAMP(const unsigned long long ts = g.stamp ? TW_NOW() : 0;)
			service(svc & live_m);
			TW_STAMP(if (g.stamp) { st_service += (unsigned int)(TW_NOW() - ts); ++st_n_service; })
		}
	}
	TW_STAMP(if (g.stamp && lane == 0) {
		unsigned long long *o = g.stamp + 12 * (size_t)blockIdx.x;
		o[0] = TW_NOW() - st_t0; o[1] = st_service; o[2] = st_flush; o[3] = st_unit; o[4] = st_n_service; o[5] = st_n_fast; o[6] = st_n_unit; o[7] = 1; o[8] = st_head; o[9] = st_take; o[10] = st_tail;
	})
#undef TW_COLD
}

size_t twin_lds_bytes() { return TW_LDS_BYTES; }

hipError_t launch_chain_twin(hipStream_t st, const Params &par, int64_t max_units, const int64_t *d_off, const void *d_a,
                             const unsigned long long *d_sumq, const uint16_t *d_lut, int lut_stride, const Unit *d_units,
                             const unsigned long long *d_counters, int32_t *d_f, int32_t *d_p, int32_t *d_v,
                             int32_t *d_first_child, uint8_t *d_flags, Unit *d_left, unsigned int *d_left_cnt, int force_left, int64_t total,
                             const UnitAux *d_unit_aux, const unsigned int *d_route, unsigned int *d_queue)
{
	if (max_units <= 0) return hipSuccess;
	if (!d_unit_aux) return hipErrorInvalidValue;
	int dev = 0, cus = 256;
	if (hipGetDevice(&dev) == hipSuccess) (void)hipDeviceGetAttribute(&cus, hipDeviceAttributeMultiprocessorCount, dev);
	int64_t blocks = (max_units + 2 * TW_QCH - 1) / (2 * TW_QCH);
	static const int wg_per_cu = getenv("CHAINDP_TWIN_WG_PER_CU") ? atoi(getenv("CHAINDP_TWIN_WG_PER_CU")) : 24;
	const int64_t cap = (int64_t)cus * (wg_per_cu >= 1 && wg_per_cu <= 24 ? wg_per_cu : 24);
	if (blocks > cap) blocks = cap;
	if (blocks < 1) blocks = 1;
	blocks = (blocks + 7) & ~(int64_t)7;
	if (!d_queue) return hipErrorInvalidValue;
	{
		const hipError_t e = hipMemsetD32Async((hipDeviceptr_t)d_queue, (int)(2 * blocks / 8), 8 * 64, st);
		if (e != hipSuccess) return e;
	}
	TwinArgs g;
	g.par = par; g.off = d_off; g.a = (const ulonglong2*)d_a; g.sumq = d_sumq; g.lut = d_lut; g.lut_stride = lut_stride;
	g.units = d_units; g.aux = d_unit_aux; g.counters = d_counters; g.f = d_f; g.p = d_p; g.v = d_v; g.first_child = d_first_child; g.flags = d_flags;
	g.left = d_left; g.left_cnt = d_left_cnt; g.queue = d_queue; g.route = d_route; g.force_left = force_left; g.total = total;
	static unsigned long long *d_stamp = nullptr;
	const bool stamp = getenv("CHAINDP_TWIN_STAMP") != nullptr;
	if (stamp && !d_stamp && hipMalloc((void**)&d_stamp, (size_t)cap * 96) != hipSuccess) d_stamp = nullptr;
	g.stamp = stamp ? d_stamp : nullptr;
	if (g.stamp) (void)hipMemsetAsync(d_stamp, 0, (size_t)blocks * 96, st);
	{
		hipFuncAttributes fa;
		const void *fn = par.max_dist_y >= par.max_dist_x ? (const void*)k_chain_twin<true> : (const void*)k_chain_twin<false>;
		const hipError_t e = hipFuncGetAttributes(&fa, fn);
		if (e != hipSuccess) return e;
		if (fa.sharedSizeBytes != 0) return hipErrorInvalidConfiguration;
	}
	if (par.max_dist_y >= par.max_dist_x) hipLaunchKernelGGL(k_chain_twin<true>, dim3((unsigned)blocks), dim3(64), TW_LDS_BYTES, st, g);
	else hipLaunchKernelGGL(k_chain_twin<false>, dim3((unsigned)blocks), dim3(64), TW_LDS_BYTES, st, g);
	if (g.stamp) {
		std::vector<unsigned long long> hb((size_t)blocks * 12);
		if (hipStreamSynchronize(st) == hipSuccess && hipMemcpy(hb.data(), d_stamp, hb.size() * 8, hipMemcpyDeviceToHost) == hipSuccess) {
			double tot = 0, svc = 0, flush = 0, unit = 0, nsvc = 0, nfast = 0, nunit = 0, nb = 0, head = 0, take = 0, tail = 0;
			for (int64_t b = 0; b < blocks; ++b) if (hb[(size_t)b * 12 + 7]) {
				const unsigned long long *o = &hb[(size_t)b * 12];
				tot += o[0]; svc += o[1]; flush += o[2]; unit += o[3]; nsvc += o[4]; nfast += o[5]; nunit += o[6]; head += o[8]; take += o[9]; tail += o[10]; ++nb;
			}
			fprintf(stderr, "[twin stamp raw] sums over waves: head %.0f take %.0f tail %.0f unit %.0f n_unit %.0f (build 3: ticks until the record / the first tile / the rest of a unit switch; switches; first tiles requested ahead)\n", head, take, tail, unit, nunit);
			fprintf(stderr, "[twin stamp] %.0f waves, %.0f ticks each: service %.1f%% (%.0f calls, %.0f ticks each: cold state and decisions %.0f, next tile %.0f, flush %.0f, "
			                "unit switch %.0f (%.0f switches, %.0f ticks each), first anchor and cold state back %.0f), passes %.0f (%.0f ticks each, everything else included)\n",
			        nb, tot / nb, 100.0 * svc / tot, nsvc, svc / (nsvc > 0 ? nsvc : 1), head / (nsvc > 0 ? nsvc : 1), take / (nsvc > 0 ? nsvc : 1), flush / (nsvc > 0 ? nsvc : 1),
			        unit / (nsvc > 0 ? nsvc : 1), nunit, unit / (nunit > 0 ? nunit : 1), tail / (nsvc > 0 ? nsvc : 1), nfast, (tot - svc) / (nfast > 0 ? nfast : 1));
		}
	}
	return hipGetLastError();
}

}
```

Before: 20.72 billion.

## Add one-table twin kernel layout with smaller LDS for higher occupancy

Adds a one-LUT variant of the twin chaining kernel. It drops the per-half anchor queue and tile prefetch and shares one lookup table, shrinking LDS per workgroup so more workgroups fit per CU, with the waves-per-EU target raised to match. Both layouts are launched back to back. The one-table kernel runs when all units share one key range and two tables are not forced; otherwise it exits early and the two-table kernel runs. The cost is an extra kernel launch every call and uncached anchor loads on tile advance in the new path.

Result: faster. 21.39 billion (median of 6 runs) (+3.2%).

```diff
diff --git a/minimap2_chaindp_amd/chaindp.py b/minimap2_chaindp_amd/chaindp.py
--- a/minimap2_chaindp_amd/chaindp.py
+++ b/minimap2_chaindp_amd/chaindp.py
@@ -361,6 +361,16 @@
         self._lib.chaindp_debug_quad_took.argtypes = [C.c_void_p]
         return int(self._lib.chaindp_debug_quad_took(self._ctx)) == 1
 
+    def set_twin_tables(self, two=True):
+        self._lib.chaindp_debug_set_twin_tables.restype = C.c_int
+        self._lib.chaindp_debug_set_twin_tables.argtypes = [C.c_void_p, C.c_int]
+        self._check(self._lib.chaindp_debug_set_twin_tables(self._ctx, int(bool(two))))
+
+    def twin_tables(self):
+        self._lib.chaindp_debug_twin_tables.restype = C.c_int
+        self._lib.chaindp_debug_twin_tables.argtypes = [C.c_void_p]
+        return int(self._lib.chaindp_debug_twin_tables(self._ctx))
+
     def set_twin_handover(self, mode=0):
         self._lib.chaindp_debug_set_twin_handover.restype = C.c_int
         self._lib.chaindp_debug_set_twin_handover.argtypes = [C.c_void_p, C.c_int]
diff --git a/minimap2_chaindp_amd/csrc/chaindp_abi.cpp b/minimap2_chaindp_amd/csrc/chaindp_abi.cpp
--- a/minimap2_chaindp_amd/csrc/chaindp_abi.cpp
+++ b/minimap2_chaindp_amd/csrc/chaindp_abi.cpp
@@ -42,6 +42,7 @@
 	int deep_eager = 0;
 	bool deep_handover = true;
 	bool use_quad = false;
+	int twin_two_tables = 0;
 	int twin_force_left = 0;
 	int variant = 0;
 	unsigned long long *d_counters = nullptr;
@@ -283,7 +284,8 @@
 			                                        (unsigned int*)ctx->d_left_cnt + 1, route, ctx->twin_force_left, total));
 		HIP_TRY(ctx, chaindp::launch_chain_twin(st, qt, total / 2, d_off, d_a, ctx->d_sumq, lut, lut_stride, ctx->d_units, ctx->d_counters,
 		                                        d_f, d_p, d_v, ctx->d_first_child, ctx->cmp.flags, ctx->d_left, (unsigned int*)ctx->d_left_cnt,
-		                                        ctx->twin_force_left, total, ctx->d_unit_aux, route, ctx->d_twin_queue));
+		                                        ctx->twin_force_left, total, ctx->d_unit_aux, ctx->pre.key_range, route, ctx->d_twin_queue,
+		                                        ctx->twin_two_tables));
 		const int64_t left_grid = total / 2 < 32768 ? total / 2 : 32768;
 		HIP_TRY(ctx, chaindp::launch_chain(st, ctx->ring, q, left_grid, d_off, d_a, d_n_segs, ctx->d_sumq, lut, lut_stride, ctx->d_left,
 		                                   ctx->d_left_cnt, d_f, d_p, d_v, ctx->d_tg, ctx->epoch, ctx->d_first_child, ctx->cmp.flags,
@@ -639,7 +641,26 @@
 	unsigned long long r = 0;
 	if (hipSetDevice(ctx->device) != hipSuccess || hipStreamSynchronize(ctx->stream) != hipSuccess ||
 	    hipMemcpy(&r, ctx->d_left_cnt + 3, sizeof(r), hipMemcpyDeviceToHost) != hipSuccess) return -1;
-	return (uint32_t)r != 0;
+	return (uint32_t)r == 1u;
+}
+
+extern "C" int chaindp_debug_set_twin_tables(chaindp_ctx_t *ctx, int two)
+{
+	if (!ctx) return CHAINDP_ERR_ARG;
+	ctx->twin_two_tables = two != 0;
+	return CHAINDP_OK;
+}
+
+extern "C" int64_t chaindp_debug_twin_lds_bytes(int one_table) { return (int64_t)chaindp::twin_lds_bytes(one_table != 0); }
+extern "C" int chaindp_debug_twin_max_wg_per_cu(int samegap, int one_table) { return chaindp::twin_max_wg_per_cu(samegap != 0, one_table != 0); }
+
+extern "C" int chaindp_debug_twin_tables(chaindp_ctx_t *ctx)
+{
+	if (!ctx || !ctx->d_left_cnt) return -1;
+	unsigned long long r = 0;
+	if (hipSetDevice(ctx->device) != hipSuccess || hipStreamSynchronize(ctx->stream) != hipSuccess ||
+	    hipMemcpy(&r, ctx->d_left_cnt + 3, sizeof(r), hipMemcpyDeviceToHost) != hipSuccess) return -1;
+	return (uint32_t)r == 2u ? 1 : (uint32_t)r == 3u ? 2 : 0;
 }
 
 extern "C" int chaindp_debug_set_twin_handover(chaindp_ctx_t *ctx, int mode)
diff --git a/minimap2_chaindp_amd/csrc/chaindp_kernels.h b/minimap2_chaindp_amd/csrc/chaindp_kernels.h
--- a/minimap2_chaindp_amd/csrc/chaindp_kernels.h
+++ b/minimap2_chaindp_amd/csrc/chaindp_kernels.h
@@ -80,8 +80,10 @@
                              const unsigned long long *d_sumq, const uint16_t *d_lut, int lut_stride, const Unit *d_units,
                              const unsigned long long *d_counters, int32_t *d_f, int32_t *d_p, int32_t *d_v,
                              int32_t *d_first_child, uint8_t *d_flags, Unit *d_left, unsigned int *d_left_cnt, int force_left, int64_t total,
-                             const UnitAux *d_unit_aux, const unsigned int *d_route = nullptr, unsigned int *d_queue = nullptr   );
-size_t twin_lds_bytes();
+                             const UnitAux *d_unit_aux, const unsigned int *d_key_range, unsigned int *d_route,
+                             unsigned int *d_queue , int two_tables);
+size_t twin_lds_bytes(bool one_table);
+int twin_max_wg_per_cu(bool samegap, bool one_table);
 
 hipError_t launch_chain_quad(hipStream_t st, const Params &par, int64_t max_units, const void *d_a, const uint16_t *d_lut, int lut_stride,
                              const Unit *d_units, const UnitAux *d_unit_aux, const unsigned long long *d_counters, const unsigned int *d_key_range,
diff --git a/minimap2_chaindp_amd/csrc/chaindp_lanes.h b/minimap2_chaindp_amd/csrc/chaindp_lanes.h
--- a/minimap2_chaindp_amd/csrc/chaindp_lanes.h
+++ b/minimap2_chaindp_amd/csrc/chaindp_lanes.h
@@ -46,6 +46,24 @@
 	return d;
 }
 
+__device__ __forceinline__ uint32_t tw_absdiff(uint32_t a, uint32_t b)
+{
+	uint32_t d = 0;
+#if defined(__HIP_DEVICE_COMPILE__)
+	asm("v_sad_u32 %0, %1, %2, 0" : "=v"(d) : "v"(a), "v"(b));
+#endif
+	return d;
+}
+
+__device__ __forceinline__ uint32_t tw_sub_m1(uint32_t b, uint32_t a)
+{
+	uint32_t d = 0;
+#if defined(__HIP_DEVICE_COMPILE__)
+	asm("v_xad_u32 %0, %1, -1, %2" : "=v"(d) : "v"(a), "v"(b));
+#endif
+	return d;
+}
+
 #define TW_ULT(a, b) __builtin_amdgcn_uicmp((unsigned)(a), (unsigned)(b), 36)
 #define TW_EQ(a, b)  __builtin_amdgcn_uicmp((unsigned)(a), (unsigned)(b), 32)
 #define TW_SGT(a, b) __builtin_amdgcn_sicmp((int)(a), (int)(b), 38)
diff --git a/minimap2_chaindp_amd/csrc/chaindp_twin.hip b/minimap2_chaindp_amd/csrc/chaindp_twin.hip
--- a/minimap2_chaindp_amd/csrc/chaindp_twin.hip
+++ b/minimap2_chaindp_amd/csrc/chaindp_twin.hip
@@ -13,19 +13,27 @@
 #define TW_XY 0u
 #define TW_PF 2048u
 #define TW_V 3072u
-#define TW_XQ 3584u
-#define TW_XQ_HALF 512u
-#define TW_LUT 4608u
-#define TW_LUT_HALF 512u
-#define TW_ST 5632u
+#define TW_LUT_BYTES 512u
 #define TW_ST_HALF 56u
-#define TW_MK 5744u
 #define TW_MK_HALF 260u
-#define TW_SP 6264u
-#define TW_SP_HALF 64u
-#define TW_SP_OF_XQ (TW_SP - TW_XQ / 8u)
-#define TW_KEY 6392u
-#define TW_LDS_BYTES 6400u
+template <bool ONE_LUT> struct TwLayout {
+	static constexpr bool HAS_XQ = !ONE_LUT;
+	static constexpr uint32_t XQ = 3584u, XQ_HALF = 512u;
+	static constexpr uint32_t LUT = ONE_LUT ? 3584u : XQ + 2u * XQ_HALF;
+	static constexpr uint32_t LUT_HALF = ONE_LUT ? 0u : TW_LUT_BYTES;
+	static constexpr uint32_t ST = LUT + (ONE_LUT ? 1u : 2u) * TW_LUT_BYTES;
+	static constexpr uint32_t MK = ST + 2u * TW_ST_HALF;
+	static constexpr uint32_t SP = MK + 2u * TW_MK_HALF;
+	static constexpr uint32_t SP_HALF = ONE_LUT ? 0u : 64u;
+	static constexpr uint32_t SP_OF_XQ = SP - XQ / 8u;
+	static constexpr uint32_t KEY = SP + 128u;
+	static constexpr uint32_t KEY_HALF = ONE_LUT ? 0u : 4u;
+	static constexpr uint32_t BYTES = KEY + 8u;
+	static_assert(ST % 8u == 0u && MK % 4u == 0u && KEY % 4u == 0u, "cold state is read as 64-bit words, marks and keys as 32-bit");
+};
+static_assert(TwLayout<true>::BYTES == 4864u && TwLayout<true>::BYTES <= 5120u, "one table: 32 workgroups per CU");
+static_assert(TwLayout<false>::BYTES == 6400u, "two tables: 24 workgroups per CU");
+template <bool SAMEGAP, bool ONE_LUT> struct TwWaves { static constexpr int N = !ONE_LUT ? 6 : SAMEGAP ? 8 : 7; };
 #define TW_TILE 64
 #define TW_RING 64
 #define TW_QCH 8
@@ -113,7 +121,9 @@
 	Unit *left;
 	unsigned int *left_cnt;
 	unsigned int *queue;
-	const unsigned int *route;
+	const unsigned int *key_range;
+	unsigned int *route;
+	int two_tables;
 	int force_left;
 	int64_t total;
 	unsigned long long *stamp;
@@ -129,7 +139,8 @@
 struct TwinHot {
 	uint32_t S;
 	uint32_t m4;
-	uint32_t pc, pend;
+	uint32_t pc;
+	uint32_t pend;
 };
 #define TW_CARRY 40u
 
@@ -155,20 +166,21 @@
 #endif
 #define TW_NOW() __builtin_amdgcn_s_memtime()
 
-template <bool SAMEGAP>
-__global__ __launch_bounds__(64) __attribute__((amdgpu_waves_per_eu(6, 6))) void k_chain_twin(TwinArgs g)
-{
+template <bool SAMEGAP, bool ONE_LUT>
+__global__ __launch_bounds__(64) __attribute__((amdgpu_waves_per_eu(TwWaves<SAMEGAP, ONE_LUT>::N, TwWaves<SAMEGAP, ONE_LUT>::N))) void k_chain_twin(TwinArgs g)
+{
+	using L = TwLayout<ONE_LUT>;
 	const int lane = threadIdx.x;
 	const bool hi_half = lane >= 32;
 	const int h = lane >> 5, hl = lane & 31;
 
 	uint32_t L16 = (uint32_t)hl << 4;
-	const uint32_t mkbase = TW_MK + TW_MK_HALF * (uint32_t)h;
-	const uint32_t curbase = TW_XQ + TW_XQ_HALF * (uint32_t)h;
+	const uint32_t mkbase = L::MK + TW_MK_HALF * (uint32_t)h;
+	const uint32_t curbase = L::XQ + L::XQ_HALF * (uint32_t)h;
 	uint32_t c_mkbase = mkbase;
 	uint32_t c_far = mkbase + 256u;
 	uint32_t c_own = mkbase + ((uint32_t)hl << 2);
-	uint32_t c_lut = TW_LUT + TW_LUT_HALF * (uint32_t)h;
+	uint32_t c_lut = ONE_LUT ? 0u : L::LUT + L::LUT_HALF * (uint32_t)h;
 	uint32_t c_8h = (uint32_t)h << 3;
 	uint32_t c_M = (uint32_t)g.par.max_dist_x;
 	uint32_t c_bw = (uint32_t)g.par.bw;
@@ -180,12 +192,16 @@
 	int c_Mout = hl == 31 ? g.par.max_dist_x : INT_MAX;
 	uint32_t c_bwl = c_bw + c_lut;
 	uint32_t c_cbwl = c_cbw - c_lut;
-	TW_VREG(L16); TW_VREG(c_far); TW_VREG(c_own); TW_VREG(c_lut); TW_VREG(c_M);
+	constexpr uint32_t LUT_OFF = ONE_LUT ? L::LUT : 0u;
+	TW_VREG(L16); TW_VREG(c_far); TW_VREG(c_own);
+	if (!ONE_LUT) { TW_VREG(c_M); TW_VREG(c_ms); }
+	if (!ONE_LUT) TW_VREG(c_lut);
 	if (!SAMEGAP) TW_VREG(c_dqoff);
-	TW_VREG(c_ms); TW_VREG(c_min); TW_VREG(c_Mout); TW_VREG(c_bwl); TW_VREG(c_cbwl);
+	TW_VREG(c_min); TW_VREG(c_Mout); TW_VREG(c_bwl); TW_VREG(c_cbwl);
 
 	const uint64_t maxx = (uint64_t)(int64_t)g.par.max_dist_x;
-	if (g.route && *g.route) return;
+	const uint32_t route = *g.route;
+	if (ONE_LUT ? route == 1u || g.key_range[0] != g.key_range[1] || g.two_tables : route == 1u || route == 2u) return;
 	const int64_t n_units = (int64_t)(uint32_t)g.counters[0];
 	const int64_t n_single = (int64_t)(g.counters[0] >> 32);
 	const bool short_units = (g.total - n_single) <= 512 * n_units;
@@ -193,14 +209,15 @@
 		if (blockIdx.x == 0 && lane == 0) *g.left_cnt = 0xffffffffu;
 		return;
 	}
+	if (blockIdx.x == 0 && lane == 0) *g.route = ONE_LUT ? 2u : 3u;
 	const bool params_ok = g.lut != nullptr && !g.par.is_cdna && g.par.max_dist_x >= 1 && g.par.max_dist_y >= 0 &&
-	                       ((uint64_t)(int64_t)g.par.max_dist_x + 1) * 129ull < (1ull << 31) && g.par.bw + 1 <= (int)TW_LUT_HALF && g.force_left != 1;
+	                       ((uint64_t)(int64_t)g.par.max_dist_x + 1) * 129ull < (1ull << 31) && g.par.bw + 1 <= (int)TW_LUT_BYTES && g.force_left != 1;
 
 	TwinHot u;
-	u.S = 0; u.m4 = 0; u.pc = curbase; u.pend = curbase;
+	u.S = 0; u.m4 = 0; u.pc = L::HAS_XQ ? curbase : 0u; u.pend = u.pc;
 	uint64_t live_m = ~0ull;
 	uint64_t contm = 0;
-	const uint32_t st_addr = TW_ST + TW_ST_HALF * (uint32_t)h;
+	const uint32_t st_addr = L::ST + TW_ST_HALF * (uint32_t)h;
 #define TW_COLD (*TW_LDS(TwinCold, st_addr))
 	const uint32_t xcd = blockIdx.x & 7u;
 	const uint32_t n_halves = 2u * gridDim.x;
@@ -221,13 +238,15 @@
 		tw_st64(st_addr + 16u, 0u, 0u); tw_st64(st_addr + 24u, 0u, 0u);
 		tw_st64(st_addr + 32u, 0u, (uint32_t)-TW_TILE);
 		tw_st64(st_addr + TW_CARRY, 0xfffffffcu, 0u); tw_st64(st_addr + TW_CARRY + 8u, 0u, 0u);
-		tw_st32(TW_KEY + 4u * (uint32_t)h, -1);
+		tw_st32(L::KEY + 4u * (uint32_t)h, -1);
 	}
 	wave_mem_fence();
 
-	TW_STAMP(unsigned long long st_t0 = 0; unsigned int st_service = 0, st_n_service = 0, st_n_fast = 0, st_flush = 0, st_unit = 0, st_n_unit = 0, st_head = 0, st_take = 0, st_tail = 0;)
+	constexpr bool PF = !ONE_LUT;
 	uint64_t nx0_x = 0, nx0_y = 0, nx1_x = 0, nx1_y = 0;
 	int32_t pfu0 = -1, pfu1 = -1;
+
+	TW_STAMP(unsigned long long st_t0 = 0; unsigned int st_service = 0, st_n_service = 0, st_n_fast = 0, st_flush = 0, st_unit = 0, st_n_unit = 0, st_head = 0, st_take = 0, st_tail = 0;)
 
 	auto service = [&](uint64_t svc) {
 #if defined(__HIP_DEVICE_COMPILE__)
@@ -239,24 +258,29 @@
 			if (((svc >> (32 * hs)) & 1ull) == 0) continue;
 			TW_STAMP_B(const unsigned long long th0 = g.stamp ? TW_NOW() : 0;)
 			const uint64_t hm = hs ? 0xffffffff00000000ull : 0x00000000ffffffffull;
-			const uint32_t sa = TW_ST + TW_ST_HALF * (uint32_t)hs;
-			const uint32_t curb = TW_XQ + TW_XQ_HALF * (uint32_t)hs, spb = TW_SP + TW_SP_HALF * (uint32_t)hs;
-			const uint32_t mkb = TW_MK + TW_MK_HALF * (uint32_t)hs, lutb = TW_LUT + TW_LUT_HALF * (uint32_t)hs;
+			const uint32_t sa = L::ST + TW_ST_HALF * (uint32_t)hs, keya = L::KEY + L::KEY_HALF * (uint32_t)hs;
+			const uint32_t mkb = L::MK + TW_MK_HALF * (uint32_t)hs, lutb = L::LUT + L::LUT_HALF * (uint32_t)hs;
+			const uint32_t curb = L::XQ + L::XQ_HALF * (uint32_t)hs, spb = L::SP + L::SP_HALF * (uint32_t)hs;
 			const tw_u32x2 cw0 = tw_ld64(sa), cw1 = tw_ld64(sa + 8u), cw2 = tw_ld64(sa + 16u), cw3 = tw_ld64(sa + 24u), cw4 = tw_ld64(sa + 32u);
 			int64_t c_next = (int64_t)((uint64_t)TW_UNI(cw0.y) << 32 | TW_UNI(cw0.x));
 			int64_t c_base = (int64_t)((uint64_t)TW_UNI(cw1.y) << 32 | TW_UNI(cw1.x));
 			uint64_t c_xcarry = (uint64_t)TW_UNI(cw2.y) << 32 | TW_UNI(cw2.x);
 			int c_rel0 = (int)TW_UNI(cw3.x), c_room = (int)TW_UNI(cw3.y), c_read = (int)TW_UNI(cw4.x), c_tile0 = (int)TW_UNI(cw4.y);
-			const int cnt_prev = (int)(((uint32_t)__builtin_amdgcn_readlane((int)u.pend, 32 * hs) - curb) >> 3);
+			auto tile_cnt = [&]() -> int {
+				const uint32_t pe = TW_UNI(__builtin_amdgcn_readlane((int)u.pend, 32 * hs));
+				if constexpr (L::HAS_XQ) return (int)((pe - curb) >> 3);
+				else return pe < mkb ? 0 : (int)((pe - mkb) >> 2) + 1 - c_tile0;
+			};
+			const int cnt_prev = tile_cnt();
 			const int slow_h = (int)TW_UNI((uint32_t)tw_ld32(sa + TW_CARRY + 12u));
-			const uint32_t cur_key = TW_UNI((uint32_t)tw_ld32(TW_KEY + 4u * (uint32_t)hs));
+			const uint32_t cur_key = TW_UNI((uint32_t)tw_ld32(keya));
 			const int tile_prev = c_tile0, rel0_prev = c_rel0;
 			const int64_t base_prev = c_base;
 			bool live = true;
 			const uint32_t nx0 = (uint32_t)c_next, ne0 = (uint32_t)((uint64_t)c_next >> 32);
 			tw_u32x4 rec0 = {0u, 0u, 0u, 0u}, aux0 = {0u, 0u, 0u, 0u}, rec1 = {0u, 0u, 0u, 0u};
 			const bool rec0_ok = nx0 < ne0 && (int64_t)nx0 < n_units;
-			const bool rec1_ok = rec0_ok && nx0 + 1u < ne0 && (int64_t)nx0 + 1 < n_units;
+			const bool rec1_ok = PF && rec0_ok && nx0 + 1u < ne0 && (int64_t)nx0 + 1 < n_units;
 			if (rec0_ok) { rec0 = *TW_CONST(tw_u32x4, g.units + nx0); aux0 = *TW_CONST(tw_u32x4, g.aux + nx0); }
 			if (rec1_ok) rec1 = *TW_CONST(tw_u32x4, g.units + nx0 + 1u);
 
@@ -273,21 +297,26 @@
 				const uint64_t stop_m = __builtin_amdgcn_ballot_w64(stop);
 				const int cnt = stop_m ? __builtin_ctzll(stop_m) : TW_TILE;
 				c_xcarry = readlane_u64(an_x, 63);
-				u.pc = TW_SEL(hm, curb, u.pc); u.pend = TW_SEL(hm, curb + ((uint32_t)cnt << 3), u.pend);
+				if constexpr (L::HAS_XQ) { u.pc = TW_SEL(hm, curb, u.pc); u.pend = TW_SEL(hm, curb + ((uint32_t)cnt << 3), u.pend); }
+				else u.pend = TW_SEL(hm, mkb + ((uint32_t)(c_tile0 + cnt - 1) << 2), u.pend);
 				if (cnt == 0) return 0;
 				wave_mem_fence();
 				if (lane < cnt) {
 					const int sp = span_of_hi((uint32_t)(an_y >> 32));
 					tw_st64((((uint32_t)i_lane & 127u) << 4 | (uint32_t)hs << 3) + TW_XY, (uint32_t)an_x + 1u, (uint32_t)an_y + 1u);
-					tw_st64(curb + ((uint32_t)lane << 3), (uint32_t)an_x, (uint32_t)an_y);
-					tw_st8(spb + (uint32_t)lane, sp - 1);
+					if constexpr (L::HAS_XQ) {
+						tw_st64(curb + ((uint32_t)lane << 3), (uint32_t)an_x, (uint32_t)an_y);
+						tw_st8(spb + (uint32_t)lane, sp - 1);
+					} else tw_st8((((uint32_t)i_lane & 63u) << 1 | (uint32_t)hs) + L::SP, sp - 1);
 					g.first_child[c_base + i_lane] = NO_CHILD;
 				}
 				wave_mem_fence();
-				if (cnt == TW_TILE && c_tile0 + TW_TILE < c_room) {
-					uint64_t rx = 0, ry = 0;
-					if (i_lane + TW_TILE < c_room) { const ulonglong2 t = g.a[c_base + i_lane + TW_TILE]; rx = t.x; ry = t.y; }
-					if (hs) { nx1_x = rx; nx1_y = ry; pfu1 = -1; } else { nx0_x = rx; nx0_y = ry; pfu0 = -1; }
+				if constexpr (PF) {
+					if (cnt == TW_TILE && c_tile0 + TW_TILE < c_room) {
+						uint64_t rx = 0, ry = 0;
+						if (i_lane + TW_TILE < c_room) { const ulonglong2 t = g.a[c_base + i_lane + TW_TILE]; rx = t.x; ry = t.y; }
+						if (hs) { nx1_x = rx; nx1_y = ry; pfu1 = -1; } else { nx0_x = rx; nx0_y = ry; pfu0 = -1; }
+					}
 				}
 				return cnt;
 			};
@@ -302,7 +331,10 @@
 			}
 			if (goes_on) {
 				c_tile0 += TW_TILE;
-				if (take_tile(hs ? nx1_x : nx0_x, hs ? nx1_y : nx0_y) == 0) goes_on = false;
+				uint64_t nt_x = 0, nt_y = 0;
+				if constexpr (PF) { nt_x = hs ? nx1_x : nx0_x; nt_y = hs ? nx1_y : nx0_y; }
+				else if (c_tile0 + lane < c_room) { const ulonglong2 t = g.a[c_base + c_tile0 + lane]; nt_x = t.x; nt_y = t.y; }
+				if (take_tile(nt_x, nt_y) == 0) goes_on = false;
 			}
 			TW_STAMP_B(if (g.stamp) st_take += (unsigned int)(TW_NOW() - th0);)
 			TW_STAMP_A(const unsigned long long tf0 = g.stamp ? TW_NOW() : 0;)
@@ -364,7 +396,8 @@
 				}
 				if ((int64_t)nx >= n_units) {
 					c_next = (int64_t)((uint64_t)ne << 32 | nx); live = false;
-					u.pc = TW_SEL(hm, curb, u.pc); u.pend = TW_SEL(hm, curb, u.pend);
+					if constexpr (L::HAS_XQ) { u.pc = TW_SEL(hm, curb, u.pc); u.pend = TW_SEL(hm, curb, u.pend); }
+					else u.pend = TW_SEL(hm, 0u, u.pend);
 					break;
 				}
 				TW_STAMP_C(const unsigned long long tc0 = g.stamp ? TW_NOW() : 0;)
@@ -374,20 +407,17 @@
 				c_next = (int64_t)((uint64_t)ne << 32 | (nx + 1u));
 				Unit un;
 				un.start = (int64_t)((uint64_t)rec0.y << 32 | rec0.x); un.read = (int32_t)rec0.z; un.len = (int32_t)rec0.w;
-				if (!params_ok || (aux0.z & 1u) || g.par.n_segs > 1) {
+				if (!params_ok || (aux0.z & 1u) || g.par.n_segs > 1 || (ONE_LUT && cur_key_now != 0xffffffffu && aux0.y != cur_key_now)) {
 					if (lane == 0) g.left[atomicAdd(g.left_cnt, 1u)] = un;
 					continue;
 				}
 				c_base = un.start; c_rel0 = (int)aux0.x; c_room = un.len; c_read = un.read; c_tile0 = 0;
-				uint64_t tl_x, tl_y;
+				uint64_t tl_x = 0, tl_y = 0;
 				TW_STAMP_C(const unsigned long long tc1 = g.stamp ? TW_NOW() : 0;)
-				TW_STAMP_C(if (g.stamp && (hs ? pfu1 : pfu0) == (int32_t)c_base) ++st_n_unit;)
-				if ((hs ? pfu1 : pfu0) == (int32_t)c_base) { tl_x = hs ? nx1_x : nx0_x; tl_y = hs ? nx1_y : nx0_y; }
-				else {
-					tl_x = 0; tl_y = 0;
-					if (lane < c_room) { const ulonglong2 t = g.a[c_base + lane]; tl_x = t.x; tl_y = t.y; }
-				}
-				if (hs) pfu1 = -1; else pfu0 = -1;
+				TW_STAMP_C(if (g.stamp && PF && (hs ? pfu1 : pfu0) == (int32_t)c_base) ++st_n_unit;)
+				if (PF && (hs ? pfu1 : pfu0) == (int32_t)c_base) { tl_x = hs ? nx1_x : nx0_x; tl_y = hs ? nx1_y : nx0_y; }
+				else if (lane < c_room) { const ulonglong2 t = g.a[c_base + lane]; tl_x = t.x; tl_y = t.y; }
+				if constexpr (PF) { if (hs) pfu1 = -1; else pfu0 = -1; }
 				TW_STAMP_C(if (g.stamp) { asm volatile("" :: "v"(tl_x), "v"(tl_y)); asm volatile("s_waitcnt vmcnt(0)" ::: "memory"); st_take += (unsigned int)(TW_NOW() - tc1); })
 				TW_STAMP_C(const unsigned long long tc2 = g.stamp ? TW_NOW() : 0;)
 				wave_mem_fence();
@@ -399,7 +429,7 @@
 						tw_st32(lutb + ((uint32_t)k << 2), (int)w);
 					}
 					cur_key_now = aux0.y;
-					if (lane == 0) tw_st32(TW_KEY + 4u * (uint32_t)hs, (int)cur_key_now);
+					if (lane == 0) tw_st32(keya, (int)cur_key_now);
 				}
 				const uint32_t x_none = (uint32_t)__builtin_amdgcn_readlane((int)(uint32_t)tl_x, 0) - (uint32_t)maxx - 1u;
 				for (int k = lane; k < 128; k += 64) tw_st64(((uint32_t)k << 4 | (uint32_t)hs << 3) + TW_XY, x_none, 0u);
@@ -410,8 +440,8 @@
 				if (take_tile(tl_x, tl_y) > 0) goes_on = true;
 				TW_STAMP_C(if (g.stamp) { st_tail += (unsigned int)(TW_NOW() - tc2); ++st_unit; })
 			}
-			if (live) {
-				const uint32_t cnt_now = ((uint32_t)__builtin_amdgcn_readlane((int)u.pend, 32 * hs) - curb) >> 3;
+			if (PF && live) {
+				const int cnt_now = tile_cnt();
 				const uint32_t nxn = (uint32_t)c_next, nen = (uint32_t)((uint64_t)c_next >> 32);
 				if (!(cnt_now == TW_TILE && c_tile0 + TW_TILE < c_room) && (hs ? pfu1 : pfu0) < 0 && nxn < nen && (int64_t)nxn < n_units &&
 				    ((nxn == nx0 && rec0_ok && !rec0_used) || (nxn == nx0 + 1u && rec1_ok))) {
@@ -446,7 +476,7 @@
 		if (__builtin_amdgcn_inverse_ballot_w64(D)) {
 			u.m4 += 4u;
 			u.S = ((u.m4 - c_mkbase) << 2) | c_8h;
-			u.pc += 8u;
+			if constexpr (L::HAS_XQ) u.pc += 8u;
 		} else {
 			if (hl == 0) {
 				tw_st64(st_addr + TW_CARRY, cur.x, cur.y);
@@ -464,7 +494,7 @@
 					Unit un; un.start = (int64_t)((uint64_t)c.base | (uint64_t)(uint32_t)c.tile0 << 32); un.read = c.read; un.len = c.room;
 					g.left[atomicAdd(g.left_cnt, 1u)] = un;
 				}
-				u.pc = curbase; u.pend = curbase;
+				u.pc = curbase; u.pend = L::HAS_XQ ? curbase : 0u;
 			}
 			return giveup;
 		}
@@ -483,12 +513,16 @@
 			uint32_t a_cur;
 			for (;;) {
 				const uint32_t t0 = u.S - L16;
+				const uint32_t S1 = u.S + 16u;
 				const tw_u32x2 xy = tw_ld64((t0 & 0x7f8u) + TW_XY);
+				const tw_u32x2 cur = tw_ld64(L::HAS_XQ ? u.pc : (S1 & 0x7f8u) + TW_XY);
+#if defined(__HIP_DEVICE_COMPILE__)
+				__builtin_amdgcn_sched_barrier(0);
+#endif
 				const tw_u32x2 pf = tw_ld64((t0 & 0x3f8u) + TW_PF);
-				const tw_u32x2 cur = tw_ld64(u.pc);
-				const int spm1 = tw_ld_u8((u.pc >> 3) + TW_SP_OF_XQ);
-				const uint32_t drm1 = cur.x - xy.x, dqm1 = cur.y - xy.y;
-				const uint32_t ddl = tw_sad(drm1, dqm1, c_lut);
+				const int spm1 = tw_ld_u8(L::HAS_XQ ? (u.pc >> 3) + L::SP_OF_XQ : __builtin_amdgcn_ubfe(S1, 3, 7) + L::SP);
+				const uint32_t drm1 = L::HAS_XQ ? cur.x - xy.x : tw_sub_m1(cur.x, xy.x), dqm1 = L::HAS_XQ ? cur.y - xy.y : tw_sub_m1(cur.y, xy.y);
+				const uint32_t ddl = ONE_LUT ? tw_absdiff(drm1, dqm1) : tw_sad(drm1, dqm1, c_lut);
 				const uint32_t dqs = SAMEGAP ? dqm1 : __builtin_elementwise_add_sat(dqm1, c_dqoff);
 				const uint32_t m3 = max(max(drm1, dqs), ddl + c_cbwl);
 				const uint64_t okm = TW_ULT(m3, c_M);
@@ -496,7 +530,7 @@
 				tw_st32(dst, (int)u.m4);
 				wave_mem_fence();
 				const int tj = tw_ld32(c_own);
-				const int lutv = tw_ld_i8(min(ddl, c_bwl));
+				const int lutv = tw_ld_i8(min(ddl, c_bwl) + LUT_OFF);
 #if defined(__HIP_DEVICE_COMPILE__)
 				__builtin_amdgcn_sched_barrier(0);
 #endif
@@ -509,7 +543,6 @@
 				cB = tw_below_in_half(B, hi_half);
 				tile = 0; X = 0; a_cur = 0;
 				if (__builtin_expect((TW_SGT(cB, 0) & A) != 0, 0)) { force_general = true; break; }
-				const uint32_t S1 = u.S + 16u;
 				a_cur = S1 & 0x3f8u;
 				{
 					const uint32_t wp = TW_SEL(A, u.m4 - c_own, 0xfffffffcu);
@@ -519,8 +552,8 @@
 				X = (TW_SGE(cB, c_ms) & B) | OUT;
 				if (__builtin_expect(tw_both_halves(X) == 0, 0)) break;
 				u.m4 += 4u; u.S = S1;
-				u.pc += 8u;
-				tile = TW_SGE(u.pc, u.pend);
+				if constexpr (L::HAS_XQ) { u.pc += 8u; tile = TW_SGE(u.pc, u.pend); }
+				else tile = TW_SGE(u.m4, u.pend);
 				TW_STAMP(if (g.stamp) ++st_n_fast;)
 				if (__builtin_expect(tile != 0, 0)) break;
 				wave_mem_fence();
@@ -531,23 +564,24 @@
 		} else {
 			force_general = false;
 			const uint32_t t0 = u.S - L16;
+			const uint32_t xcur = ((((u.m4 - c_mkbase) + 4u) << 2) & 0x7f8u) | c_8h;
 			const tw_u32x2 xy = tw_ld64((t0 & 0x7f8u) + TW_XY);
 			const tw_u32x2 pf = tw_ld64((t0 & 0x3f8u) + TW_PF);
-			const tw_u32x2 cur = tw_ld64(u.pc);
-			const int spm1 = tw_ld_u8((u.pc >> 3) + TW_SP_OF_XQ);
+			const tw_u32x2 cur = tw_ld64(L::HAS_XQ ? u.pc : xcur + TW_XY);
+			const int spm1 = tw_ld_u8(L::HAS_XQ ? (u.pc >> 3) + L::SP_OF_XQ : ((xcur >> 3) & 0x7fu) + L::SP);
 			const uint64_t first = ~contm;
 			const tw_u32x2 carry = tw_ld64(st_addr + TW_CARRY);
 			const int maxf = TW_SEL(first, spm1, (int)carry.y);
 			const uint32_t maxj4 = TW_SEL(first, 0xfffffffcu, carry.x);
 			const int nskip0 = TW_SEL(first, 0, tw_ld32(st_addr + TW_CARRY + 8u));
 			const uint32_t kb4 = TW_SEL(first, 0u, 128u);
-			const uint32_t drm1 = cur.x - xy.x, dqm1 = cur.y - xy.y;
-			const uint32_t ddl = tw_sad(drm1, dqm1, c_lut);
+			const uint32_t drm1 = L::HAS_XQ ? cur.x - xy.x : tw_sub_m1(cur.x, xy.x), dqm1 = L::HAS_XQ ? cur.y - xy.y : tw_sub_m1(cur.y, xy.y);
+			const uint32_t ddl = ONE_LUT ? tw_absdiff(drm1, dqm1) : tw_sad(drm1, dqm1, c_lut);
 			const uint32_t dqs = SAMEGAP ? dqm1 : __builtin_elementwise_add_sat(dqm1, c_dqoff);
 			const uint32_t m3 = max(max(drm1, dqs), ddl + c_cbwl);
 			const uint64_t okm = TW_ULT(m3, c_M) & ~(contm & TW_HI31) & live_m;
 			const int sc0 = min(min((int)dqm1, (int)drm1), spm1);
-			const int lutv = tw_ld_i8(min(ddl, c_bwl));
+			const int lutv = tw_ld_i8(min(ddl, c_bwl) + LUT_OFF);
 			const uint32_t dst = TW_SEL(okm, min(u.m4 - pf.x, c_far), c_far);
 			tw_st32(dst, (int)u.m4);
 			wave_mem_fence();
@@ -572,7 +606,7 @@
 				brk = TW_SGT(nskip_after, c_ms) & B;
 				Ap = tw_below_first(A, brk);
 			}
-			const uint32_t a_cur = (((((u.m4 - c_mkbase) + 4u) << 2) & 0x3f8u) | c_8h) + TW_PF;
+			const uint32_t a_cur = (xcur & 0x3f8u) + TW_PF;
 			{
 				const uint32_t wp = TW_SEL(Ap, u.m4 - c_own - kb4, maxj4);
 				const int wf = TW_SEL(Ap, sc, maxf);
@@ -581,7 +615,7 @@
 			const uint64_t D = tw_smear_halves(brk | (OUT & TW_HI31) | ~live_m);
 			svc = slow_tail(D, a_cur, nskip_after);
 		}
-		svc |= tw_smear_halves(TW_SGE(u.pc, u.pend) & live_m & ~contm);
+		svc |= tw_smear_halves((L::HAS_XQ ? TW_SGE(u.pc, u.pend) : TW_SGE(u.m4, u.pend)) & live_m & ~contm);
 		if (__builtin_expect(svc != 0, 0)) {
 			TW_STAMP(const unsigned long long ts = g.stamp ? TW_NOW() : 0;)
 			service(svc & live_m);
@@ -595,33 +629,31 @@
 #undef TW_COLD
 }
 
-size_t twin_lds_bytes() { return TW_LDS_BYTES; }
-
-hipError_t launch_chain_twin(hipStream_t st, const Params &par, int64_t max_units, const int64_t *d_off, const void *d_a,
-                             const unsigned long long *d_sumq, const uint16_t *d_lut, int lut_stride, const Unit *d_units,
-                             const unsigned long long *d_counters, int32_t *d_f, int32_t *d_p, int32_t *d_v,
-                             int32_t *d_first_child, uint8_t *d_flags, Unit *d_left, unsigned int *d_left_cnt, int force_left, int64_t total,
-                             const UnitAux *d_unit_aux, const unsigned int *d_route, unsigned int *d_queue)
-{
-	if (max_units <= 0) return hipSuccess;
-	if (!d_unit_aux) return hipErrorInvalidValue;
-	int dev = 0, cus = 256;
-	if (hipGetDevice(&dev) == hipSuccess) (void)hipDeviceGetAttribute(&cus, hipDeviceAttributeMultiprocessorCount, dev);
+size_t twin_lds_bytes(bool one_table) { return one_table ? TwLayout<true>::BYTES : TwLayout<false>::BYTES; }
+
+int twin_max_wg_per_cu(bool samegap, bool one_table)
+{
+	const int lds_wg = one_table ? 32 : 24;
+	const int waves = one_table ? (samegap ? TwWaves<true, true>::N : TwWaves<false, true>::N)
+	                            : (samegap ? TwWaves<true, false>::N : TwWaves<false, false>::N);
+	return 4 * waves < lds_wg ? 4 * waves : lds_wg;
+}
+
+template <bool ONE_LUT>
+static hipError_t launch_twin_layout(hipStream_t st, TwinArgs g, int64_t max_units, int cus, unsigned int *d_queue)
+{
+	const bool samegap = g.par.max_dist_y >= g.par.max_dist_x;
+	const int max_wg = twin_max_wg_per_cu(samegap, ONE_LUT);
 	int64_t blocks = (max_units + 2 * TW_QCH - 1) / (2 * TW_QCH);
-	static const int wg_per_cu = getenv("CHAINDP_TWIN_WG_PER_CU") ? atoi(getenv("CHAINDP_TWIN_WG_PER_CU")) : 24;
-	const int64_t cap = (int64_t)cus * (wg_per_cu >= 1 && wg_per_cu <= 24 ? wg_per_cu : 24);
+	static const int wg_env = getenv("CHAINDP_TWIN_WG_PER_CU") ? atoi(getenv("CHAINDP_TWIN_WG_PER_CU")) : 0;
+	const int64_t cap = (int64_t)cus * (wg_env >= 1 && wg_env <= max_wg ? wg_env : max_wg);
 	if (blocks > cap) blocks = cap;
 	if (blocks < 1) blocks = 1;
 	blocks = (blocks + 7) & ~(int64_t)7;
-	if (!d_queue) return hipErrorInvalidValue;
 	{
 		const hipError_t e = hipMemsetD32Async((hipDeviceptr_t)d_queue, (int)(2 * blocks / 8), 8 * 64, st);
 		if (e != hipSuccess) return e;
 	}
-	TwinArgs g;
-	g.par = par; g.off = d_off; g.a = (const ulonglong2*)d_a; g.sumq = d_sumq; g.lut = d_lut; g.lut_stride = lut_stride;
-	g.units = d_units; g.aux = d_unit_aux; g.counters = d_counters; g.f = d_f; g.p = d_p; g.v = d_v; g.first_child = d_first_child; g.flags = d_flags;
-	g.left = d_left; g.left_cnt = d_left_cnt; g.queue = d_queue; g.route = d_route; g.force_left = force_left; g.total = total;
 	static unsigned long long *d_stamp = nullptr;
 	const bool stamp = getenv("CHAINDP_TWIN_STAMP") != nullptr;
 	if (stamp && !d_stamp && hipMalloc((void**)&d_stamp, (size_t)cap * 96) != hipSuccess) d_stamp = nullptr;
@@ -629,13 +661,13 @@
 	if (g.stamp) (void)hipMemsetAsync(d_stamp, 0, (size_t)blocks * 96, st);
 	{
 		hipFuncAttributes fa;
-		const void *fn = par.max_dist_y >= par.max_dist_x ? (const void*)k_chain_twin<true> : (const void*)k_chain_twin<false>;
+		const void *fn = samegap ? (const void*)k_chain_twin<true, ONE_LUT> : (const void*)k_chain_twin<false, ONE_LUT>;
 		const hipError_t e = hipFuncGetAttributes(&fa, fn);
 		if (e != hipSuccess) return e;
 		if (fa.sharedSizeBytes != 0) return hipErrorInvalidConfiguration;
 	}
-	if (par.max_dist_y >= par.max_dist_x) hipLaunchKernelGGL(k_chain_twin<true>, dim3((unsigned)blocks), dim3(64), TW_LDS_BYTES, st, g);
-	else hipLaunchKernelGGL(k_chain_twin<false>, dim3((unsigned)blocks), dim3(64), TW_LDS_BYTES, st, g);
+	if (samegap) hipLaunchKernelGGL((k_chain_twin<true, ONE_LUT>), dim3((unsigned)blocks), dim3(64), TwLayout<ONE_LUT>::BYTES, st, g);
+	else hipLaunchKernelGGL((k_chain_twin<false, ONE_LUT>), dim3((unsigned)blocks), dim3(64), TwLayout<ONE_LUT>::BYTES, st, g);
 	if (g.stamp) {
 		std::vector<unsigned long long> hb((size_t)blocks * 12);
 		if (hipStreamSynchronize(st) == hipSuccess && hipMemcpy(hb.data(), d_stamp, hb.size() * 8, hipMemcpyDeviceToHost) == hipSuccess) {
@@ -644,8 +676,8 @@
 				const unsigned long long *o = &hb[(size_t)b * 12];
 				tot += o[0]; svc += o[1]; flush += o[2]; unit += o[3]; nsvc += o[4]; nfast += o[5]; nunit += o[6]; head += o[8]; take += o[9]; tail += o[10]; ++nb;
 			}
-			fprintf(stderr, "[twin stamp raw] sums over waves: head %.0f take %.0f tail %.0f unit %.0f n_unit %.0f (build 3: ticks until the record / the first tile / the rest of a unit switch; switches; first tiles requested ahead)\n", head, take, tail, unit, nunit);
-			fprintf(stderr, "[twin stamp] %.0f waves, %.0f ticks each: service %.1f%% (%.0f calls, %.0f ticks each: cold state and decisions %.0f, next tile %.0f, flush %.0f, "
+			if (nb > 0) fprintf(stderr, "[twin stamp raw] sums over waves: head %.0f take %.0f tail %.0f unit %.0f n_unit %.0f (build 3: ticks until the record / the first tile / the rest of a unit switch; switches; first tiles requested ahead)\n", head, take, tail, unit, nunit);
+			if (nb > 0) fprintf(stderr, "[twin stamp] %.0f waves, %.0f ticks each: service %.1f%% (%.0f calls, %.0f ticks each: cold state and decisions %.0f, next tile %.0f, flush %.0f, "
 			                "unit switch %.0f (%.0f switches, %.0f ticks each), first anchor and cold state back %.0f), passes %.0f (%.0f ticks each, everything else included)\n",
 			        nb, tot / nb, 100.0 * svc / tot, nsvc, svc / (nsvc > 0 ? nsvc : 1), head / (nsvc > 0 ? nsvc : 1), take / (nsvc > 0 ? nsvc : 1), flush / (nsvc > 0 ? nsvc : 1),
 			        unit / (nsvc > 0 ? nsvc : 1), nunit, unit / (nunit > 0 ? nunit : 1), tail / (nsvc > 0 ? nsvc : 1), nfast, (tot - svc) / (nfast > 0 ? nfast : 1));
@@ -654,4 +686,24 @@
 	return hipGetLastError();
 }
 
-}
+hipError_t launch_chain_twin(hipStream_t st, const Params &par, int64_t max_units, const int64_t *d_off, const void *d_a,
+                             const unsigned long long *d_sumq, const uint16_t *d_lut, int lut_stride, const Unit *d_units,
+                             const unsigned long long *d_counters, int32_t *d_f, int32_t *d_p, int32_t *d_v,
+                             int32_t *d_first_child, uint8_t *d_flags, Unit *d_left, unsigned int *d_left_cnt, int force_left, int64_t total,
+                             const UnitAux *d_unit_aux, const unsigned int *d_key_range, unsigned int *d_route, unsigned int *d_queue, int two_tables)
+{
+	if (max_units <= 0) return hipSuccess;
+	if (!d_unit_aux || !d_key_range || !d_route || !d_queue) return hipErrorInvalidValue;
+	int dev = 0, cus = 256;
+	if (hipGetDevice(&dev) == hipSuccess) (void)hipDeviceGetAttribute(&cus, hipDeviceAttributeMultiprocessorCount, dev);
+	TwinArgs g;
+	g.par = par; g.off = d_off; g.a = (const ulonglong2*)d_a; g.sumq = d_sumq; g.lut = d_lut; g.lut_stride = lut_stride;
+	g.units = d_units; g.aux = d_unit_aux; g.counters = d_counters; g.f = d_f; g.p = d_p; g.v = d_v; g.first_child = d_first_child; g.flags = d_flags;
+	g.left = d_left; g.left_cnt = d_left_cnt; g.queue = d_queue; g.key_range = d_key_range; g.route = d_route; g.two_tables = two_tables != 0;
+	g.force_left = force_left; g.total = total; g.stamp = nullptr;
+	hipError_t e = launch_twin_layout<true>(st, g, max_units, cus, d_queue);
+	if (e == hipSuccess) e = launch_twin_layout<false>(st, g, max_units, cus, d_queue);
+	return e;
+}
+
+}
```
